# xiyichen/morphablediffusion

Hardware: AMD Instinct MI355X
Metric: multi-view denoising steps/sec (N=16 views, 256x256, CFG 2.0, DDIM-50 step) (higher is better)
Workload: dtype f16; 1 GPU; synthetic sample (FaceScape-FLAME-sized mesh, 5023 vertices before voxel de-duplication): N=16 target views, 256x256 (latent 32x32), perspective cameras, full-width UNet (916.9M params, random init), CFG 2.0, one denoise_apply per step; views_per_gpu=16, batch_view_num=16, parallelism=single GPU

## Files before the change

### include/mvd.h

```cpp
#ifndef MVD_H
#define MVD_H
#include <stddef.h>
#include <stdint.h>

#ifdef __cplusplus
extern "C" {
#endif

typedef struct mvd_ctx mvd_ctx;

typedef struct {
  int image_size;
  int in_channels;
  int out_channels;
  int model_channels;
  int num_res_blocks;
  int channel_mult[4];
  int num_heads;
  int context_dim;
  int volume_dims[4];
  int attention_levels;
} mvd_unet_config;

typedef struct {
  int time_dim;
  int view_dim;
  int num_views;
  int input_image_size;
  int frustum_volume_depth;
  int spatial_volume_size;
  float spatial_volume_length;
  float frustum_volume_length;
  int projection;
  int frustum_dims[4];
  float voxel_size;
} mvd_volume_config;

int mvd_create(const mvd_unet_config* ucfg, const mvd_volume_config* vcfg, int device, size_t workspace_bytes,
               mvd_ctx** out);
void mvd_destroy(mvd_ctx* ctx);
const char* mvd_last_error(void);
const char* mvd_compute_dtype(void);

int mvd_upload_weight(mvd_ctx* ctx, const char* name, const float* data, const int64_t* shape, int ndim, int on_device);
int mvd_set_precision_level(mvd_ctx* ctx, int level);
int mvd_set_vae_precision(mvd_ctx* ctx, int exact);
int mvd_finalize_weights(mvd_ctx* ctx);

int mvd_unet_forward(mvd_ctx* ctx, const float* x, const int64_t* timesteps, const float* context, int Bv, int n_ctx,
                     const float* src0, const float* src1, const float* src2, const float* src3, int depth0, float* out,
                     void* stream);
int mvd_unet_block(mvd_ctx* ctx, const char* path, const float* x, int B, int C, int H, int W, const int64_t* timesteps,
                   const float* context, const float* volume, int D, float* out, int out_capacity, int* out_shape, void* stream);


int mvd_embed_time(mvd_ctx* ctx, const int64_t* t, int B, float* out, void* stream);

int mvd_set_mesh(mvd_ctx* ctx, const float* vertices, const int32_t* coord, const int32_t* out_sh, const float* bounds,
                 int Nv);
int mvd_select_sample(mvd_ctx* ctx, int slot);
int mvd_set_cameras(mvd_ctx* ctx, const float* K, const float* RT, int N);
int mvd_set_mesh_async(mvd_ctx* ctx, const float* vertices, const int32_t* coord, const int32_t* out_sh, const float* bounds,
                       int Nv, void* stream);
int mvd_set_cameras_async(mvd_ctx* ctx, const float* K, const float* RT, int N, void* stream);
int mvd_set_samples_async(mvd_ctx* ctx, int B, const int* slots, const float* const* vertices, const int32_t* const* coord,
                          const int32_t* const* out_sh, const float* const* bounds, const int* Nv, const float* const* K,
                          const float* const* RT, int N, void* stream);
int mvd_rulebook_build(const int32_t* coord, const int32_t* out_sh, int Nv, int force_hash, int32_t* n_sites, int64_t* lens);
int mvd_rulebook_table(int which, int32_t* out);

int mvd_vertex_features(mvd_ctx* ctx, const float* x_noisy, const float* t_embed, const float* v_embed,
                        const int32_t* view_idx, int n_local, int add_bias, float* fused_out, void* stream);
int mvd_vertex_view_features(mvd_ctx* ctx, const float* x_noisy, const float* t_embed, const float* v_embed,
                             const int32_t* view_idx, int n_local, float* vf_out, void* stream);
int mvd_fuse_vertex_features(mvd_ctx* ctx, const float* vf_all, int n_views, float* fused_out, void* stream);
int mvd_vertex_features_stream_safe(mvd_ctx* ctx);
int mvd_stage_target_encoder(mvd_ctx* ctx, const float* x_noisy, const float* t_embed, const float* v_embed, int n_local,
                             float* feats, void* stream);
int mvd_stage_sparse_dense(mvd_ctx* ctx, const float* fused, int train_mode, float* dense_out, int32_t* shape_out, void* stream);
typedef struct { char internal[128]; } mvd_rccl_id;
int mvd_comm_unique_id(mvd_rccl_id* id_out);
int mvd_comm_init(mvd_ctx* ctx, const mvd_rccl_id* id, int rank, int world);
int mvd_comm_destroy(mvd_ctx* ctx);
int mvd_exchange_view_features(mvd_ctx* ctx, const float* local, float* all, int n_local, void* stream);
int mvd_comm_all_reduce(mvd_ctx* ctx, float* buf, size_t count, void* stream);
int mvd_set_volume_ready_event(mvd_ctx* ctx, void* event);
int mvd_volume_from_fused(mvd_ctx* ctx, const float* fused, float* volume_out, void* stream);

int mvd_volume_from_fused_train(mvd_ctx* ctx, const float* fused, float* volume_out, void* stream);
int mvd_mse_loss(mvd_ctx* ctx, const float* a, const float* b, size_t n, float* out, void* stream);
int mvd_train_enable(mvd_ctx* ctx, int on);
int mvd_train_param_count(mvd_ctx* ctx);
int mvd_train_param_info(mvd_ctx* ctx, int index, char* name, size_t name_cap, int64_t* offset, int64_t* numel, int64_t* shape,
                         int* ndim);
int64_t mvd_train_arena_size(mvd_ctx* ctx);
int mvd_train_adopt_arena(mvd_ctx* ctx, int which, float* ptr, int64_t numel);
int mvd_train_zero_grad(mvd_ctx* ctx, void* stream);
int mvd_train_unet_step(mvd_ctx* ctx, const float* x, const int64_t* timesteps, const float* context, int B, const float* src0,
                        const float* src1, const float* src2, const float* src3, int depth0, const float* target, float loss_scale,
                        int recompute, float* pred_out, float* loss_out, float* dsrc0, float* dsrc1, float* dsrc2, float* dsrc3,
                        void* stream);
int mvd_train_conditioner_backward(mvd_ctx* ctx, const float* x_noisy, int64_t timestep, const float* v_embed, int n_views,
                                   int target_index, const float* dsrc0, const float* dsrc1, const float* dsrc2, const float* dsrc3,
                                   float* dbg_dvolume, float* dbg_dfused, float* dbg_dfeats, float* dbg_dtembed, void* stream);
int mvd_train_conditioner_backward_batch(mvd_ctx* ctx, int B, const int* slots, const float* x_noisy, const int64_t* timesteps,
                                         const float* v_embed, int n_views, const int* target_index, const float* dsrc0,
                                         const float* dsrc1, const float* dsrc2, const float* dsrc3, float* dbg_dvolume,
                                         float* dbg_dfused, float* dbg_dfeats, float* dbg_dtembed, void* stream);
int mvd_train_cond_backward(mvd_ctx* ctx, int cond_index, const float* x, const float* context, const float* d_out, int B, int H,
                            int W, int depth0, float* dx, float* dcontext, void* stream);
int mvd_train_get_grad(mvd_ctx* ctx, const char* name, float* out, size_t numel, void* stream);
int mvd_train_get_tensor(mvd_ctx* ctx, const char* name, float* out, size_t numel, void* stream);
int64_t mvd_train_bn_calls(mvd_ctx* ctx);
int mvd_train_adamw_step(mvd_ctx* ctx, float lr, float lr_aux, float beta1, float beta2, float eps, float weight_decay, int step,
                         float inv_scale, int finetune_unet, int* skipped_out, void* stream);
int mvd_train_repack(mvd_ctx* ctx);
int mvd_train_repack_async(mvd_ctx* ctx, void* stream);
int mvd_train_grad_bucket_count(mvd_ctx* ctx);
int mvd_train_grad_bucket(mvd_ctx* ctx, int k, int max_ranges, int64_t* offs, int64_t* lens, int* n_ranges);
int mvd_train_grad_bucket_wait(mvd_ctx* ctx, int k, void* stream);
int mvd_train_set_bucket_snapshot(mvd_ctx* ctx, float* arena);
int mvd_train_sync_gradients(mvd_ctx* ctx, int phase, void* comm_stream, void* stream);
int mvd_set_volume(mvd_ctx* ctx, const float* volume, void* stream);

int mvd_frustum_volumes(mvd_ctx* ctx, const float* t_embed, const float* v_embed, const int32_t* view_idx, int TN,
                        float* out0, float* out1, float* out2, float* out3, void* stream);
int mvd_frustum_volumes_batch(mvd_ctx* ctx, int B, const int* slots, const float* volumes, const float* t_embed, const float* v_rows,
                              const int32_t* view_idx, float* out0, float* out1, float* out2, float* out3, void* stream);

int mvd_denoise_views(mvd_ctx* ctx, const float* x_noisy, const float* x_input, const float* clip, int64_t timestep,
                      const float* t_embed, const float* v_embed, const int32_t* view_idx, int TN, float cfg_scale,
                      const float* noise, float sqrt_one_minus_at, float sqrt_at, float sqrt_aprev, float dir_coef,
                      float sigma, float* eps_out, float* x_prev, void* stream);
int mvd_denoise_views_batch(mvd_ctx* ctx, int B, const int* slots, const float* x_noisy, const float* x_input, const float* clip,
                            const int64_t* timesteps, const float* t_embed, const float* v_embed, const int32_t* view_idx, int TN,
                            float cfg_scale, const float* noise, float sqrt_one_minus_at, float sqrt_at, float sqrt_aprev,
                            float dir_coef, float sigma, float* eps_out, float* x_prev, void* stream);

int mvd_denoise_views_ms(mvd_ctx* ctx, int B, const int* slots, const float* x_noisy, const float* x_input, const float* clip,
                         const int64_t* timesteps, const float* t_embed, const float* v_embed, const int32_t* view_idx, int TN,
                         float cfg_scale, const float* noise, float s1m, float sqrt_at, float c_x, float c_d, float c_c, float c_n,
                         float* x0_hist, int first, float* eps_out, float* x_next, void* stream);

int mvd_op_cfg_ms(const float* eps_c, const float* eps_u, float scale, const float* x, const float* noise, float s1m, float sqrt_at,
                  float c_x, float c_d, float c_c, float c_n, float* x0_hist, int first, float* eps_out, float* x_next, size_t n,
                  void* stream);
int mvd_op_conv(mvd_ctx* ctx, const float* x_nchw, int B, int Cin, int H, int W, const float* w, const float* bias,
                int Cout, int ksize, int stride, int upsample, const float* resid_nchw, float* out_nchw, int force_splitk,
                void* stream);
int mvd_op_linear(mvd_ctx* ctx, const float* a, int M, int K, const float* w, const float* bias, int N, int geglu,
                  const float* resid, int a_half, int force_splitk, float* out, void* stream);
int mvd_op_group_norm(mvd_ctx* ctx, const float* x_nchw, int B, int C, int HW, int groups, const float* gamma,
                      const float* beta, float eps, int act, float* out_nchw, void* stream);
int mvd_op_layer_norm(mvd_ctx* ctx, const float* x, int rows, int C, const float* gamma, const float* beta, float* out,
                      void* stream);
int mvd_op_attention(mvd_ctx* ctx, const float* q, const float* k, const float* v, int B, int T, int heads, int d,
                     float* out, void* stream);
int mvd_op_conv3d(mvd_ctx* ctx, const float* x_ncdhw, int B, int Cin, int D, int H, int W, const float* w,
                  const float* bias, int Cout, int stride, int transposed, const float* resid, float* out, void* stream);
int mvd_op_attention_bwd(mvd_ctx* ctx, const float* q, const float* k, const float* v, const float* d_out, int B, int T, int heads,
                         int d, float* dq, float* dk, float* dv, void* stream);
int mvd_op_group_norm_bwd(mvd_ctx* ctx, const float* x, const float* dy, int B, int rows, int C, int groups, const float* gamma,
                          const float* beta, float eps, int act, float* dx, float* dgamma, float* dbeta, void* stream);
int mvd_op_layer_norm_bwd(mvd_ctx* ctx, const float* x, const float* dy, int rows, int C, const float* gamma, float* dx,
                          float* dgamma, float* dbeta, void* stream);
int mvd_op_conv_bwd(mvd_ctx* ctx, int kind, int ksize, int B, int Cin, int H, int W, int Cout, const float* x, int x_f16,
                    const float* w, const float* dy, int xp, int accum, int need_din, int poison, float* dx, float* dw, float* db,
                    void* stream);
int mvd_op_linear_bwd(mvd_ctx* ctx, int B, int rows, int K, int N, const float* x, int x_f16, const float* w, const float* bias,
                      const float* dy, int geglu, int dx_f16, int staged, int xp, int accum, int poison, float* dx, float* dw,
                      float* db, void* stream);
int mvd_op_conv3d_bwd(mvd_ctx* ctx, int kind, int B, int Cin, int D, int H, int W, int Cout, const float* x, int x_f16,
                      const float* w, const float* dy, int accum, int poison, float* dx, float* dw, float* db, void* stream);
int mvd_op_tgemm(mvd_ctx* ctx, int M, int N, int K, const float* a, int a_f16, int a_trans, long lda, const float* b, int b_f16,
                 int b_trans, long ldb, float* out, int ldc, int accum, int xp, int poison, void* stream);
int mvd_op_st_tail(mvd_ctx* ctx, int C, int rows, int T, const float* ao, const float* xin, const float* rowbias,
                   const float* w_ao, const float* b_ao, const float* ln_g, const float* ln_b, const float* w1, const float* b1,
                   const float* w2, const float* b2, const float* w_po, const float* b_po, const float* resid, float* out,
                   int flags, int iters, float* ms_out, void* stream);
int mvd_op_st_head(mvd_ctx* ctx, int rows, int xp, const float* n0, const float* w_pi, const float* b_pi, const float* ln_g,
                   const float* ln_b, const float* w_q, const float* w_k, const float* w_v, float* t0_out, float* qkv_out,
                   int iters, float* ms_out, void* stream);
int mvd_bench_conv(mvd_ctx* ctx, int B, int C, int H, int W, int Cout, int iters, float* ms_out, void* stream);
int mvd_vae_decode(mvd_ctx* ctx, const float* z, int B, int h, int w, float* out, void* stream);
int mvd_vae_encode(mvd_ctx* ctx, const float* x, int B, int H, int W, float* moments, void* stream);
int mvd_clip_encode(mvd_ctx* ctx, const float* x, int B, int H, int W, float* out, void* stream);
int mvd_clip_embed_dim(mvd_ctx* ctx);
int mvd_probe_config(mvd_ctx* ctx, int mode, const char* family, int stride);
int mvd_probe_report(mvd_ctx* ctx, char* buf, size_t cap);
int mvd_bench_linear(mvd_ctx* ctx, int M, int K, int N, int flags, int iters, float* ms_out, void* stream);
int mvd_bench_group_norm(mvd_ctx* ctx, int B, int C, int HW, int groups, int flags, int iters, float* ms_out, void* stream);

#ifdef __cplusplus
}
#endif
#endif
```

### morphablediffusion_amd/csrc/c_api.hip

```cpp
#include <array>
#include <dlfcn.h>
#include <stdlib.h>
#include <string.h>

#include <algorithm>
#include <string>
#include <utility>
#include <vector>

#include "engine.h"
#include "rowchain.h"

int engine_set_cameras(mvd_ctx* c, const float* K, const float* RT, int N, hipStream_t s);
int engine_set_mesh(mvd_ctx* c, const float* vertices, const int32_t* coord, const int32_t* out_sh, const float* bounds,
                    int Nv, hipStream_t s);
int engine_select_sample(mvd_ctx* c, int slot);
int engine_set_samples(mvd_ctx* c, int B, const int* slots, const float* const* vertices, const int32_t* const* coord,
                       const int32_t* const* out_sh, const float* const* bounds, const int* Nv, const float* const* K,
                       const float* const* RT, int N, hipStream_t s);
int engine_rulebook_build(const int32_t* coord, const int32_t* out_sh, int Nv, int force_hash, int32_t* n_sites, int64_t* lens);
int engine_rulebook_table(int which, int32_t* out);
void mesh_free(MeshTables& m);

static thread_local std::string g_err;
// ... 899 lines not shown
  if (c->comm) {
    a->comm_destroy(c->comm);
    c->comm = nullptr;
  }
  const int rc = a->comm_init_rank(&c->comm, world, *id, rank);
  if (rc) {
    c->comm = nullptr;
    return rccl_fail(a, "ncclCommInitRank", rc);
  }
  c->comm_rank = rank;
  c->comm_world = world;
  return 0;
}

int mvd_comm_destroy(mvd_ctx* c) {
  if (!c || !c->comm) return 0;
  RcclApi* a = rccl_api();
  if (a) a->comm_destroy(c->comm);
  c->comm = nullptr;
  c->comm_world = 1;
  c->comm_rank = 0;
  return 0;
}

int mvd_exchange_view_features(mvd_ctx* c, const float* local, float* all, int n_local, void* stream) {
  if (!c || !c->comm) return mvd_fail("mvd_exchange_view_features: no communicator (mvd_comm_init)");
  if (hipSetDevice(c->device) != hipSuccess) return mvd_fail("hipSetDevice failed");
  if (!local || !all || n_local <= 0 || c->mesh.Nv <= 0) return mvd_fail("mvd_exchange_view_features: bad arguments / no mesh is set");
  RcclApi* a = rccl_api();
  if (!a) return mvd_fail("mvd_exchange_view_features: librccl.so could not be opened");
  if (c->v.num_views > 0 && (long)c->comm_world * n_local != c->v.num_views)
    return mvd_fail("mvd_exchange_view_features: comm_world * n_local does not equal the configured view count");
  const size_t count = (size_t)n_local * c->mesh.Nv * 16;
  const int rc = a->all_gather(local, all, count,  7, c->comm, S(stream));
  return rc ? rccl_fail(a, "ncclAllGather", rc) : 0;
}

int mvd_comm_all_reduce(mvd_ctx* c, float* buf, size_t count, void* stream) {
  if (!c || !c->comm) return mvd_fail("mvd_comm_all_reduce: no communicator (mvd_comm_init)");
  if (hipSetDevice(c->device) != hipSuccess) return mvd_fail("hipSetDevice failed");
  if (!buf || count == 0) return mvd_fail("mvd_comm_all_reduce: bad arguments");
  RcclApi* a = rccl_api();
  if (!a) return mvd_fail("mvd_comm_all_reduce: librccl.so could not be opened");
  const int rc = a->all_reduce(buf, buf, count,  7,  0, c->comm, S(stream));
  return rc ? rccl_fail(a, "ncclAllReduce", rc) : 0;
}

int mvd_train_sync_gradients(mvd_ctx* c, int phase, void* comm_stream, void* stream) {
  if (!c || !c->comm) return mvd_fail("mvd_train_sync_gradients: no communicator (mvd_comm_init)");
  if (hipSetDevice(c->device) != hipSuccess) return mvd_fail("hipSetDevice failed");
  if (!c->arena_g || c->arena_n == 0) return mvd_fail("mvd_train_sync_gradients: no gradient arena (mvd_train_enable)");
  if (phase != 0 && phase != 1) return mvd_fail("mvd_train_sync_gradients: phase is 0 (start) or 1 (finish)");
  RcclApi* a = rccl_api();
  if (!a) return mvd_fail("mvd_train_sync_gradients: librccl.so could not be opened");
  hipStream_t cs = S(comm_stream), ms = S(stream);
  auto reduce = [&](size_t off, size_t n) -> int {
    const int rc = a->all_reduce(c->arena_g + off, c->arena_g + off, n, 7, 0, c->comm, cs);
    return rc ? rccl_fail(a, "ncclAllReduce", rc) : 0;
  };
  if (phase == 0) {
    for (int k = 0; k < c->n_buckets; ++k) {
      const mvd_ctx::GradBucket& b = c->buckets[k];
      if (b.ev) HIP_CHECK_RET(hipStreamWaitEvent(cs, b.ev, 0));
      for (size_t r = 0; r < b.off.size(); ++r) RET_IF(reduce(b.off[r], b.len[r]));
    }
    c->grad_sync_started = true;
    return 0;
  }
  if (!c->ev_grad_sync[0]) {
    HIP_CHECK_RET(hipEventCreateWithFlags(&c->ev_grad_sync[0], hipEventDisableTiming));
    HIP_CHECK_RET(hipEventCreateWithFlags(&c->ev_grad_sync[1], hipEventDisableTiming));
  }
  HIP_CHECK_RET(hipEventRecord(c->ev_grad_sync[0], ms));
  HIP_CHECK_RET(hipStreamWaitEvent(cs, c->ev_grad_sync[0], 0));
  std::vector<std::pair<size_t, size_t>> spans;
  if (c->grad_sync_started)
    for (int k = 0; k < c->n_buckets; ++k)
      for (size_t r = 0; r < c->buckets[k].off.size(); ++r) spans.push_back({c->buckets[k].off[r], c->buckets[k].off[r] + c->buckets[k].len[r]});
  std::sort(spans.begin(), spans.end());
  size_t pos = 0;
  for (auto& sp : spans) {
    if (sp.first < pos) return mvd_fail("mvd_train_sync_gradients: gradient buckets overlap");
    if (sp.first > pos) RET_IF(reduce(pos, sp.first - pos));
    pos = sp.second;
  }
  if (pos < c->arena_n) RET_IF(reduce(pos, c->arena_n - pos));
  c->grad_sync_started = false;
  HIP_CHECK_RET(hipEventRecord(c->ev_grad_sync[1], cs));
  HIP_CHECK_RET(hipStreamWaitEvent(ms, c->ev_grad_sync[1], 0));
  return launch_scale_copy(c->arena_g, c->arena_n, 1.0f / (float)c->comm_world, c->arena_g, ms);
}

int mvd_op_conv(mvd_ctx* c, const float* x_nchw, int B, int Cin, int H, int W, const float* w, const float* bias, int Cout,
                int ksize, int stride, int upsample, const float* resid_nchw, float* out_nchw, int force_splitk,
                void* stream) {
  if (c && hipSetDevice(c->device) != hipSuccess) return mvd_fail("hipSetDevice failed");
  hipStream_t s = S(stream);
  WsScope ws_scope(c);
  const int cpad = (Cin + 7) / 8 * 8, taps = ksize * ksize;
  const int Hv = H << upsample, Wv = W << upsample;
  const int Ho = (Hv - 1) / stride + 1, Wo = (Wv - 1) / stride + 1;
  float* xn = ws_alloc<float>(c, (size_t)B * H * W * cpad);
  half_t* wp = ws_alloc<half_t>(c, (size_t)taps * Cout * cpad);
  float* on = ws_alloc<float>(c, (size_t)B * Ho * Wo * Cout);
  float* rn = resid_nchw ? ws_alloc<float>(c, (size_t)B * Ho * Wo * Cout) : nullptr;
  WS_CHECK(xn && wp && on);
  RET_IF(launch_nchw_to_nhwc(x_nchw, B, Cin, H * W, xn, cpad, cpad, s));
  RET_IF(launch_pack_weight(w, Cout, cpad, taps, 0, 0, wp, s, Cin));
  if (rn) RET_IF(launch_nchw_to_nhwc(resid_nchw, B, Cout, Ho * Wo, rn, Cout, Cout, s));
  if (force_splitk == -3) {
    if (taps != 9 || stride != 1 || upsample || rn || cpad != Cin) return mvd_fail("op_conv: the fp32 output-head form is 3x3, stride 1, no residual");
    RET_IF(launch_out_conv_f32(xn, Cin, w, bias, Cout, B, H, W, on, Cout, s));
    RET_IF(launch_nhwc_to_nchw(on, Cout, B, Cout, Ho * Wo, out_nchw, s));
    return 0;
  }
  if (force_splitk == -2) {
    if (taps != 9 || stride != 1 || upsample || rn) return mvd_fail("op_conv: the fp32 first-layer form is 3x3, stride 1, no residual");
    RET_IF(launch_conv_in_f32(xn, cpad, w, Cin, bias, Cout, B, H, W, on, Cout, s));
    RET_IF(launch_nhwc_to_nchw(on, Cout, B, Cout, Ho * Wo, out_nchw, s));
    return 0;
  }
  ConvW cw;
  cw.w = wp; cw.bias = const_cast<float*>(bias); cw.N = Cout; cw.Cin = cpad; cw.taps = taps;
  GemmArgs g;
  g.a = xn; g.a_f32 = 1; g.lda = cpad; g.w = &cw; g.out = on; g.ldc = Cout; g.resid = rn; g.ldr = Cout;
  g.use_bias = bias != nullptr; g.force_splitk = force_splitk;
  if (cpad % 64 == 0) {
    half_t* xh = ws_alloc<half_t>(c, (size_t)B * H * W * cpad);
    WS_CHECK(xh);
    RET_IF(launch_f32_to_f16(xn, xh, (size_t)B * H * W * cpad, s));
    g.a = xh;
    g.a_f32 = 0;
    const int bnx = Cout % 160 == 0 ? 160 : (Cout % 128 == 0 ? 128 : 0);
    if (taps == 9 && bnx && mvd_env_call::conv3x()) {
      cw.wx = ws_alloc<half_t>(c, conv3x_stream_halfs(Cout, cpad, bnx));
      WS_CHECK(cw.wx);
      RET_IF(conv3x_pack(wp, Cout, cpad, bnx, cw.wx, s));
      cw.wx_bn = bnx;
    }
  }
  if (upsample && taps == 9 && stride == 1 && cpad == Cin && B * H * W >= 2048) {
    cw.w_up = ws_alloc<half_t>(c, (size_t)16 * Cout * Cin);
    WS_CHECK(cw.w_up);
    RET_IF(launch_pack_upconv_weight(w, Cout, Cin, cw.w_up, s));
    g.a = xn; g.a_f32 = 1;
    RET_IF(run_upconv2d(c, g, B, H, W, s));
  } else {
    RET_IF(run_conv2d(c, g, B, H, W, stride, upsample, s));
  }
  RET_IF(launch_nhwc_to_nchw(on, Cout, B, Cout, Ho * Wo, out_nchw, s));
  return 0;
}

int mvd_op_conv3d(mvd_ctx* c, const float* x, int B, int Cin, int D, int H, int W, const float* w, const float* bias,
                  int Cout, int stride, int transposed, const float* resid, float* out, void* stream) {
  if (c && hipSetDevice(c->device) != hipSuccess) return mvd_fail("hipSetDevice failed");
  hipStream_t s = S(stream);
  WsScope ws_scope(c);
  if (Cin % 8) return mvd_fail("op_conv3d: Cin must be a multiple of 8");
  const int Do = transposed ? 2 * D : (D - 1) / stride + 1, Ho = transposed ? 2 * H : (H - 1) / stride + 1,
            Wo = transposed ? 2 * W : (W - 1) / stride + 1;
  float* xn = ws_alloc<float>(c, (size_t)B * D * H * W * Cin);
  half_t* wp = ws_alloc<half_t>(c, (size_t)27 * Cout * Cin);
  float* on = ws_alloc<float>(c, (size_t)B * Do * Ho * Wo * Cout);
  WS_CHECK(xn && wp && on);
  RET_IF(launch_nchw_to_nhwc(x, B, Cin, D * H * W, xn, Cin, Cin, s));
  RET_IF(launch_pack_weight(w, Cout, Cin, 27, transposed, 0, wp, s, Cin));
  if (resid) RET_IF(launch_nchw_to_nhwc(resid, B, Cout, Do * Ho * Wo, on, Cout, Cout, s));
  ConvW cw;
  cw.w = wp; cw.bias = const_cast<float*>(bias); cw.N = Cout; cw.Cin = Cin; cw.taps = 27;
  GemmArgs g;
  g.a = xn; g.a_f32 = 1; g.lda = Cin; g.w = &cw; g.out = on; g.ldc = Cout; g.use_bias = bias != nullptr;
  if (resid) { g.resid = on; g.ldr = Cout; }
  if (Cin % 64 == 0) {
    half_t* xh = ws_alloc<half_t>(c, (size_t)B * D * H * W * Cin);
    WS_CHECK(xh);
    RET_IF(launch_f32_to_f16(xn, xh, (size_t)B * D * H * W * Cin, s));
    g.a = xh;
    g.a_f32 = 0;
  }
  if (transposed) RET_IF(run_convT3d(c, g, B, D, H, W, s));
  else RET_IF(run_conv3d(c, g, B, D, H, W, stride, s));
  RET_IF(launch_nhwc_to_nchw(on, Cout, B, Cout, Do * Ho * Wo, out, s));
  return 0;
}

int mvd_op_linear(mvd_ctx* c, const float* a, int M, int K, const float* w, const float* bias, int N, int geglu,
                  const float* resid, int a_half, int force_splitk, float* out, void* stream) {
  if (c && hipSetDevice(c->device) != hipSuccess) return mvd_fail("hipSetDevice failed");
  hipStream_t s = S(stream);
  WsScope ws_scope(c);
  if (K % 8) return mvd_fail("op_linear: K must be a multiple of 8");
  half_t* wp = ws_alloc<half_t>(c, (size_t)N * K);
  float* bp = ws_alloc<float>(c, (size_t)N);
  WS_CHECK(wp && bp);
  RET_IF(launch_pack_weight(w, N, K, 1, 0, geglu, wp, s, K));
  if (bias) {
    if (geglu) RET_IF(launch_permute_geglu_bias(bias, N, bp, s));
    else HIP_CHECK_RET(hipMemcpyAsync(bp, bias, (size_t)N * 4, hipMemcpyDeviceToDevice, s));
  }
  ConvW cw;
  cw.w = wp; cw.bias = bias ? bp : nullptr; cw.N = N; cw.Cin = K; cw.taps = 1;
  GemmArgs g;
  g.a = a; g.a_f32 = 1; g.lda = K; g.w = &cw; g.out = out; g.ldc = geglu ? N / 2 : N; g.geglu = geglu;
  g.use_bias = bias != nullptr;
  g.force_splitk = force_splitk;
  if (resid) {
    g.resid = resid; g.resid_f32 = 1; g.ldr = N;
  }
  if (a_half) {
    half_t* ah = ws_alloc<half_t>(c, (size_t)M * K);
    WS_CHECK(ah);
    RET_IF(launch_f32_to_f16(a, ah, (size_t)M * K, s));
    g.a = ah; g.a_f32 = 0;
  }
  RET_IF(run_linear(c, g, 1, M, s));
  return 0;
}

int mvd_op_group_norm(mvd_ctx* c, const float* x_nchw, int B, int C, int HW, int groups, const float* gamma,
                      const float* beta, float eps, int act, float* out_nchw, void* stream) {
  if (c && hipSetDevice(c->device) != hipSuccess) return mvd_fail("hipSetDevice failed");
  hipStream_t s = S(stream);
  WsScope ws_scope(c);
  float* xn = ws_alloc<float>(c, (size_t)B * HW * C);
  half_t* y = ws_alloc<half_t>(c, (size_t)B * HW * C);
  float* yf = ws_alloc<float>(c, (size_t)B * HW * C);
  WS_CHECK(xn && y && yf);
  RET_IF(launch_nchw_to_nhwc(x_nchw, B, C, HW, xn, C, C, s));
  NormW n;
  n.g = const_cast<float*>(gamma); n.b = const_cast<float*>(beta); n.C = C;
  RET_IF(run_group_norm(c, xn, C, B, HW, n, groups, eps, act, nullptr, y, C, s));
  hipLaunchKernelGGL(f16_to_f32_kernel, dim3(nblk((size_t)B * HW * C)), dim3(256), 0, s, y, yf, (size_t)B * HW * C);
  RET_IF(launch_nhwc_to_nchw(yf, C, B, C, HW, out_nchw, s));
  return 0;
}

int mvd_op_layer_norm(mvd_ctx* c, const float* x, int rows, int C, const float* gamma, const float* beta, float* out,
                      void* stream) {
  if (c && hipSetDevice(c->device) != hipSuccess) return mvd_fail("hipSetDevice failed");
  hipStream_t s = S(stream);
  WsScope ws_scope(c);
  half_t* y = ws_alloc<half_t>(c, (size_t)rows * C);
  WS_CHECK(y);
  RET_IF(launch_layernorm(x, rows, C, gamma, beta, 1e-5f, y, s));
  hipLaunchKernelGGL(f16_to_f32_kernel, dim3(nblk((size_t)rows * C)), dim3(256), 0, s, y, out, (size_t)rows * C);
  HIP_CHECK_RET(hipGetLastError());
  return 0;
}

int mvd_op_attention(mvd_ctx* c, const float* q, const float* k, const float* v, int B, int T, int heads, int d, float* out,
                     void* stream) {
  if (c && hipSetDevice(c->device) != hipSuccess) return mvd_fail("hipSetDevice failed");
  hipStream_t s = S(stream);
  WsScope ws_scope(c);
  const int C = heads * d, rows = B * T;
  half_t* qkv = ws_alloc<half_t>(c, (size_t)rows * 3 * C);
  half_t* o = ws_alloc<half_t>(c, (size_t)rows * C);
  WS_CHECK(qkv && o);
  hipLaunchKernelGGL(pack_qkv_rows_kernel, dim3(nblk((size_t)rows * C)), dim3(256), 0, s, q, k, v, rows, C, qkv);
  RET_IF(launch_attention(qkv, 3 * C, qkv + 2 * C, 3 * C, o, C, B, T, heads, d, s));
  hipLaunchKernelGGL(f16_to_f32_kernel, dim3(nblk((size_t)rows * C)), dim3(256), 0, s, o, out, (size_t)rows * C);
  HIP_CHECK_RET(hipGetLastError());
  return 0;
}

int mvd_op_attention_bwd(mvd_ctx* c, const float* q, const float* k, const float* v, const float* d_out, int B, int T, int heads, int d,
                         float* dq, float* dk, float* dv, void* stream) {
  if (c && hipSetDevice(c->device) != hipSuccess) return mvd_fail("hipSetDevice failed");
  if (!c) return mvd_fail("null context");
  hipStream_t s = S(stream);
  WsScope ws_scope(c);
  const int C = heads * d, rows = B * T;
  half_t* qkv = ws_alloc<half_t>(c, (size_t)rows * 3 * C);
  half_t* o = ws_alloc<half_t>(c, (size_t)rows * C);
  half_t* do16 = ws_alloc<half_t>(c, (size_t)rows * C);
  half_t* dqkv = ws_alloc<half_t>(c, (size_t)rows * 3 * C);
  float* lse = ws_alloc<float>(c, (size_t)B * heads * T);
  float* delta = ws_alloc<float>(c, (size_t)B * heads * T);
  float* tmp = ws_alloc<float>(c, (size_t)rows * 3 * C);
  WS_CHECK(qkv && o && do16 && dqkv && lse && delta && tmp);
  hipLaunchKernelGGL(pack_qkv_rows_kernel, dim3(nblk((size_t)rows * C)), dim3(256), 0, s, q, k, v, rows, C, qkv);
  RET_IF(launch_attention(qkv, 3 * C, qkv + 2 * C, 3 * C, o, C, B, T, heads, d, s));
  RET_IF(bwd_cast_rows(d_out, C, rows, C, C, do16, s));
  RET_IF(bwd_attention(qkv, 3 * C, o, do16, C, dqkv, 3 * C, lse, delta, B, T, heads, d, s));
  hipLaunchKernelGGL(f16_to_f32_kernel, dim3(nblk((size_t)rows * 3 * C)), dim3(256), 0, s, dqkv, tmp, (size_t)rows * 3 * C);
  HIP_CHECK_RET(hipGetLastError());
  float* outs[3] = {dq, dk, dv};
  for (int i = 0; i < 3; ++i)
    HIP_CHECK_RET(hipMemcpy2DAsync(outs[i], (size_t)C * 4, tmp + (size_t)i * C, (size_t)3 * C * 4, (size_t)C * 4, rows, hipMemcpyDeviceToDevice, s));
  return 0;
}

int mvd_op_group_norm_bwd(mvd_ctx* c, const float* x, const float* dy, int B, int rows, int C, int groups, const float* gamma,
                          const float* beta, float eps, int act, float* dx, float* dgamma, float* dbeta, void* stream) {
  if (c && hipSetDevice(c->device) != hipSuccess) return mvd_fail("hipSetDevice failed");
  if (!c) return mvd_fail("null context");
  hipStream_t s = S(stream);
  WsScope ws_scope(c);
  const bool one_block = mvd_env().gn_bwd_one_block;
  const int S = one_block ? 1 : bwd_gn_slabs(B, groups, rows);
  float* dg = ws_alloc<float>(c, (size_t)B * S * C);
  float* db = ws_alloc<float>(c, (size_t)B * S * C);
  float* part = ws_alloc<float>(c, (size_t)B * groups * S * 4);
  WS_CHECK(dg && db && part);
  if (one_block)
    RET_IF(bwd_group_norm(x, C, nullptr, 0, dy, C, B, rows, C, groups, gamma, beta, eps, act, dx, C, 0, dg, db, nullptr, s));
  else
    RET_IF(bwd_group_norm_slab(x, C, nullptr, 0, dy, C, B, rows, C, groups, gamma, beta, eps, act, dx, C, 0, part,
                               part + (size_t)B * groups * S * 2, dg, db, nullptr, S, s));
  RET_IF(bwd_sum_rows_add(dg, B * S, C, C, dgamma, 0, s));
  return bwd_sum_rows_add(db, B * S, C, C, dbeta, 0, s);
}

int mvd_op_layer_norm_bwd(mvd_ctx* c, const float* x, const float* dy, int rows, int C, const float* gamma, float* dx, float* dgamma,
                          float* dbeta, void* stream) {
  if (c && hipSetDevice(c->device) != hipSuccess) return mvd_fail("hipSetDevice failed");
  if (!c) return mvd_fail("null context");
  hipStream_t s = S(stream);
  WsScope ws_scope(c);
  float* part = ws_alloc<float>(c, (size_t)bwd_ln_max_blocks() * 2 * C);
  WS_CHECK(part);
  int nb = 0;
  RET_IF(bwd_layer_norm(x, C, dy, C, rows, C, gamma, 1e-5f, dx, C, 0, part, &nb, s));
  RET_IF(bwd_sum_rows_add(part, nb, C, 2 * C, dgamma, 0, s));
  return bwd_sum_rows_add(part + C, nb, C, 2 * C, dbeta, 0, s);
}

int mvd_bench_conv(mvd_ctx* c, int B, int C, int H, int W, int Cout, int iters, float* ms_out, void* stream) {
  if (c && hipSetDevice(c->device) != hipSuccess) return mvd_fail("hipSetDevice failed");
  hipStream_t s = S(stream);
  WsScope ws_scope(c);
  const size_t na = (size_t)B * H * W * C, nw = (size_t)9 * Cout * C;
  half_t* a = ws_alloc<half_t>(c, na);
  half_t* w = ws_alloc<half_t>(c, nw);
  float* o = ws_alloc<float>(c, (size_t)B * H * W * Cout);
  WS_CHECK(a && w && o);
// ... 324 lines not shown
```

### morphablediffusion_amd/csrc/common.h

```cpp
#pragma once
#include <hip/hip_runtime.h>
#include <hip/hip_fp16.h>
#include <stdint.h>

#include "env.h"

#ifdef MVD_BF16
typedef __bf16 half_t;
#define MVD_MFMA_32x32x16 __builtin_amdgcn_mfma_f32_32x32x16_bf16
#define MVD_MFMA_16x16x32 __builtin_amdgcn_mfma_f32_16x16x32_bf16
#define MVD_DTYPE_NAME "bf16"
#else
typedef _Float16 half_t;
#define MVD_MFMA_32x32x16 __builtin_amdgcn_mfma_f32_32x32x16_f16
#define MVD_MFMA_16x16x32 __builtin_amdgcn_mfma_f32_16x16x32_f16
#define MVD_DTYPE_NAME "f16"
#endif
typedef half_t h8 __attribute__((ext_vector_type(8)));
typedef half_t h4 __attribute__((ext_vector_type(4)));
typedef half_t h2 __attribute__((ext_vector_type(2)));
typedef float f32x16 __attribute__((ext_vector_type(16)));
typedef float f32x4 __attribute__((ext_vector_type(4)));

#define MVD_MAX_TAPS 27

enum { ACT_NONE = 0, ACT_SILU = 1, ACT_RELU = 2 };

inline bool xcd_prefers_cols(int tiles_m, int groups_n, double a_bytes, double w_bytes) {
  const int nwg = tiles_m * groups_n, q = (nwg + 7) / 8;
  if (nwg < 16) return false;
  auto span = [](int q_, int inner, int outer) {
    const double n = q_ % inner == 0 ? q_ / inner : (q_ - 1) / (double)inner + 1.0;
    return n < outer ? n : (double)outer;
  };
  const double at = a_bytes / tiles_m, wt = w_bytes / groups_n;
  const double row = at * span(q, groups_n, tiles_m) + wt * (q < groups_n ? q : groups_n);
  const double col = wt * span(q, tiles_m, groups_n) + at * (q < tiles_m ? q : tiles_m);
  return col < 0.8 * row;
}

struct IGemm {
  const void* a;
  int a_f32;
  int lda;
  int Cin;
  int cin_alg;
  int B, Z, Y, X;
  int IZ, IY, IX;
  int sz, sy, sx;
  int ups;
  int PZ, PY, PX;
  int ntaps;
  int tap[MVD_MAX_TAPS];
  const half_t* w;
  int N;
  void* out;
  int out_f32;
  int ldc;
  int out_linear;
  int OZ, OY, OX, ozm, ozo, oym, oyo, oxm, oxo;
  const float* bias;
  const float* rowbias;
  int rb_ld;
  const float* rowscale;
  int rs_ld;
  float* gn_partial;
  int gn_cpg;
  const void* resid;
  int resid_f32;
  int ldr;
  int out_split;
  int geglu;
  float alpha;
  int act;
  int nch;
  int xcd_cols;
  int npar;
  int par_ntaps[8];
  int par_tap[8][8];
  int par_oz[8], par_oy[8], par_ox[8];
  int par_walk;
  const half_t* wx;
  int wx_bn;
  int bn;
  int bm;
  int splitk;
  float* partial;
};

struct MvdStream {
  hipStream_t s;
};

#define HIP_CHECK_RET(expr)                                        \
  do {                                                             \
    hipError_t _e = (expr);                                        \
    if (_e != hipSuccess) return mvd_fail(hipGetErrorString(_e));  \
  } while (0)

int mvd_fail(const char* msg);
const char* mvd_error_text();

#define MVD_MAX_DEVICES 64
static inline int mvd_current_device() {
  int d = 0;
  if (hipGetDevice(&d) != hipSuccess || d < 0 || d >= MVD_MAX_DEVICES) d = 0;
  return d;
}
static inline int cdiv(int a, int b) { return (a + b - 1) / b; }
static inline int igemm_tap(int dz, int dy, int dx, int slab) { return (dz + 1) | ((dy + 1) << 2) | ((dx + 1) << 4) | (slab << 8); }

int launch_igemm(const IGemm& g, hipStream_t s);
int igemm_pick_bn(int N, int geglu);
int launch_splitk_reduce(const IGemm& g, hipStream_t s);
bool conv3_halo_eligible(const IGemm& g);
int conv3_halo_tiles(const IGemm& g, int bn);
int launch_conv3_halo(const IGemm& g, hipStream_t s);
int igemm_pick_splitk(int M, int N, int ksteps, int bn);
bool conv3x_eligible(const IGemm& g, int bn);
size_t conv3x_stream_halfs(int N, int Cin, int bn);
int conv3x_pack(const half_t* w, int N, int Cin, int bn, half_t* stream, hipStream_t s);
int launch_conv3x(const IGemm& g, const half_t* stream, int bn, hipStream_t s);
bool gemm_dma_eligible(const IGemm& g);
bool gemm_dma_is_plain(const IGemm& g);
void gemm_dma_plan(int M, int N, int ksteps, int bn, int geglu, int* nch_out, int* splitk_out);
int launch_target_encoder(const float* x, const float* pre, int n_views, const half_t* const* w, const float* const* bias,
                          const int* cin, const float* const* gamma, const float* const* beta, float* feats, hipStream_t s);
void gemm_dma_plan_us(int M, int N, int ksteps, int geglu, int out_b, int res_b, int* bn_io, int* nch_out, int* splitk_out,
                      int* bm_out = nullptr);
int launch_gemm_dma(const IGemm& g, hipStream_t s);

int launch_gn_stats(const float* x, int ld, int B, int rows_per_sample, int C, int G, const float* preadd, int pld,
                    float* partial, int* nslabs_out, hipStream_t s);
int launch_gn_apply(const float* x, int ld, int B, int rows_per_sample, int C, int G, const float* preadd, int pld,
                    const float* partial, int nslabs, const float* gamma, const float* beta, float eps, int act,
                    half_t* out, int ldo, hipStream_t s, int split = 0);
int gn_max_slabs();
int launch_gn_finalize(const float* partial, int B, int nslabs, int rows_per_sample, int C, int G, const float* gamma,
                       const float* beta, float eps, float* scale, float* shift, int ld, hipStream_t s);
bool gn_group_eligible(int ld, int rows, int C, int G, int pld, int ldo);
int launch_gn_group(const float* x, int ld, int B, int rows, int C, int G, const float* preadd, int pld, const float* gamma,
                    const float* beta, float eps, int act, half_t* out, int ldo, hipStream_t s, int split = 0,
                    int nslab = 1, size_t slab_stride = 0, const float* bias2 = nullptr, const float* resid = nullptr, int ldr = 0,
                    float* mat = nullptr, int ldm = 0);
int launch_layernorm(const float* x, int rows, int C, const float* gamma, const float* beta, float eps,
                     half_t* out, hipStream_t s, half_t* raw = nullptr, int ld_raw = 0);
bool layernorm_slabs_takes(int C);
int launch_layernorm_slabs(const float* slabs, int nslab, size_t slab_stride, int rows, int C, const float* bias, const float* rowbias,
                           int rb_ld, int T, const float* resid, int ldr, float* mat, const float* gamma, const float* beta, float eps,
                           half_t* out, hipStream_t s, half_t* raw = nullptr, int ld_raw = 0);
int launch_layernorm_f32(const float* x, long ldx, int rows, int C, const float* gamma, const float* beta, float eps,
                         float* out, hipStream_t s);
int launch_attention(const half_t* qk, int ldqk, const half_t* v, int ldv, half_t* out, int ldo, int B, int T, int heads,
                     int d, hipStream_t s, int Tstride = 0);
int launch_clip_patches(const float* img, int B, int H, int W, int S, int P, int Kp, half_t* out, hipStream_t s);
int launch_clip_tokens(const float* pe, const float* cls, const float* pos, int B, int T, int Tp, int C, float* x,
                       hipStream_t s);
int launch_scale_copy(const float* src, size_t n, float k, float* dst, hipStream_t s);
int launch_softmax_rows(const float* s, long rows, int cols, half_t* p, hipStream_t st);
int launch_depth_attn(const float* qk, const half_t* ctxn, half_t* z, int n_cond, int HW, int D, int Cc, int heads,
                      hipStream_t s, int split = 0, int nfill = 0, const half_t* fill_row = nullptr, int ldx = 0);
int launch_small_linear(const float* a, int lda, int rows, int K, const half_t* w, const float* bias, int N,
                        int act_in, float* out, int ldo, int accumulate, hipStream_t s);
int launch_timestep_embedding(const int64_t* t, int B, int dim, float* out, hipStream_t s);
int launch_nchw_to_nhwc(const float* in, int B, int C, int HW, float* out, int ldo, int cpad, hipStream_t s);
int launch_nhwc_to_nchw(const float* in, int ld, int B, int C, int HW, float* out, hipStream_t s);
int launch_pack_weight(const float* src, int N, int Cin, int taps, int transposed, int geglu, half_t* dst,
                       hipStream_t s, int cin_src = -1, int xp = 0);
int launch_rows_f32_to_f16_split(const float* in, int lda, long rows, int C, half_t* out, hipStream_t s);
int launch_permute_geglu_bias(const float* src, int N, float* dst, hipStream_t s);
int launch_f32_to_f16(const float* in, half_t* out, size_t n, hipStream_t s);
int launch_rows_f32_to_f16(const float* in, int lda, long rows, int C, half_t* out, hipStream_t s);
int launch_pack_upconv_weight(const float* src, int N, int Cin, half_t* dst, hipStream_t s);
int launch_fill_rows_f16(half_t* out, int ld, int rows, const half_t* vec, int n, hipStream_t s);
int launch_fold_qk(const float* wq, const float* wk, int heads, int hd, int Cc, int I, float scale, half_t* out,
                   hipStream_t s, float* out32 = nullptr);
int launch_fold_ov(const float* wo, const float* wv, int heads, int hd, int Cc, int I, half_t* out, hipStream_t s,
                   float* out32 = nullptr);
int launch_fold_mm(const float* a, int lda, const float* b, int ldb, int M, int N, int K, half_t* out16, int ldc, float* out32,
                   hipStream_t s);
int launch_relu_beta_tile(const float* beta, int Cc, int heads, half_t* out, hipStream_t s, int split = 0);
int launch_cfg_ddim(const float* eps_c, const float* eps_u, float scale, const float* x, const float* noise,
                    float sqrt_one_minus_at, float sqrt_at, float sqrt_aprev, float dir_coef, float sigma,
                    float* eps_out, float* x_prev, size_t n, hipStream_t s);
struct DpmCoef {
  float s1m, sqrt_at, c_x, c_d, c_c, c_n;
};
int launch_cfg_dpm(const float* eps_c, const float* eps_u, float scale, const float* x, const float* noise, DpmCoef k,
                   float* x0_hist, int use_hist, float* eps_out, float* x_next, size_t n, hipStream_t s);
struct ViewCam {
  float P[12];
  float Pinv[12];
  float Kinv[9];
  float near_, far_;
};
int launch_vertex_gather(const float* feats, const ViewCam* cams, const int* view_idx, int n_views, const float* verts, int Nv, int V,
                         float vol_len, int fsize, int persp, float* out, hipStream_t s);
int launch_fuse_views(const float* vf, int n_views, int Nv, int total_views, const float* w, const float* b,
                      float* out, int accumulate, hipStream_t s);
int launch_sparse_conv(const float* in, const int* nbr, int n_out, int Cin, int Cout, const float* w, const float* wp,
                       const float* scale, const float* shift, float* out, hipStream_t s, int mask_nonrep = 0);
bool sparse_mfma_takes(int Cin, int Cout);
int launch_sparse_w_frag(const float* w, int Cl_in, int Cl_out, int transposed, int flip, float* dst, hipStream_t s);
int launch_sparse_w_pack(const float* src, int Cin, int Cout, int layout, float* dst, hipStream_t s);
int launch_bn_fold(const float* gamma, const float* beta, const float* mean, const float* var, float eps, int C, float* scale,
                   float* shift, hipStream_t s);
int launch_bn_rows_relu(const float* x, float* y, int n, int C, const float* gamma, const float* beta, float eps, float* stats_out,
                        hipStream_t s, float* rmean = nullptr, float* rvar = nullptr, float momentum = 0.f);
int launch_mse(const float* a, const float* b, size_t n, float* out, hipStream_t s);
int launch_latent_gather(const float* feats, const int* grid, int gd, int gh, int gw, const float* min_xyz,
                         const int* out_sh, float voxel, int V, float vol_len, float* out, hipStream_t s);
int launch_sparse_densify(const float* feats, const int* grid, long nvox, int C, float* out, hipStream_t s);
int launch_frustum_gather(const float* vol, const ViewCam* cams, const int* view_idx, int TN, int D, int S, int V,
                          float vol_len, int persp, half_t* out, hipStream_t s);
int launch_bits_checksum(const void* p, size_t bytes, unsigned long long* out, hipStream_t s);
int launch_add_rows(float* dst, const float* a, const float* b, size_t n, hipStream_t s);
int launch_add_image_rows(const float* in, int ldi, const float* img, int C, int nb, int HW, float* out, int ldo, hipStream_t s);
int launch_upsample2_f16(const float* in, int ldi, int B, int H, int W, int C, half_t* out, hipStream_t s);
int launch_conv_in_f32(const float* x, int ldx, const float* w, int cin_src, const float* bias, int N, int B, int H, int W, float* out,
                       int ldo, hipStream_t s);
int launch_out_conv_f32(const float* a, int C, const float* w, const float* bias, int N, int B, int H, int W, float* out, int ldo,
                        hipStream_t s);
int launch_probe_null(hipStream_t s);
```

### morphablediffusion_amd/csrc/engine.h

```cpp
#pragma once
#include <functional>
#include <map>
#include <string>
#include <vector>

#include "../../include/mvd.h"
#include "common.h"
#include "rowchain.h"

struct RawTensor {
  float* d = nullptr;
  std::vector<int64_t> shape;
  size_t numel = 0;
};

struct ConvW {
  int xp = 0;
  int cin_l = 0;
  half_t* w = nullptr;
  half_t* wx = nullptr;
  int wx_bn = 0;
  half_t* w_up = nullptr;
  int res_out = 0;
  float* w32 = nullptr;
  int cin_src = 0;
  float* bias = nullptr;
  int N = 0, Cin = 0, taps = 1;
  half_t* wT = nullptr;
  int Np = 0;
  std::string key;
  std::string bkey;
};
struct NormW {
  float* g = nullptr;
  float* b = nullptr;
  int C = 0;
  std::string key;
};
struct LinW {
  std::string key;
  half_t* w = nullptr;
  float* bias = nullptr;
  int N = 0, K = 0;
};

struct ResW {
  NormW n1, n2;
  ConvW c1, c2, skip;
  bool has_skip = false;
  int cin = 0, cout = 0, emb_off = 0;
  int res = 0;
  std::string key;
};
struct STW {
  NormW norm, ln1, ln3;
  ConvW proj_in, qkv, attn_out, ff1, ff2, proj_out;
  int C = 0, heads = 8, a2_off = 0;
  std::string key;
  half_t* rc_stream = nullptr;
  half_t* rh_stream = nullptr;
  int rc_po = 1, rh_xp = 0;
  ConvW ffp;
};
struct CondW {
  ConvW proj_in, proj_ctx, wqk, wov, conv1, conv2;
  NormW gn_in, gn_ctx, gn_o1, gn_o2;
  half_t* relu_beta = nullptr;
  int dim = 0, Cc = 0, I = 0;
  int res = 0;
  std::string key;
};
struct VaeResW {
  NormW n1, n2;
  ConvW c1, c2, skip;
  bool has_skip = false;
  int cin = 0, cout = 0;
};
struct VaeAttnW {
  NormW norm;
  ConvW q, k, v, proj;
};
struct VaeW {
  bool present = false;
  int ch = 0, out_ch = 0, zc = 0, embed = 0, block_in = 0, nlev = 0;
  ConvW post_quant;
  ConvW conv_in, conv_out;
  NormW norm_out;
  VaeResW mid1, mid2;
  VaeAttnW attn;
  std::vector<std::vector<VaeResW>> up;
  std::vector<ConvW> up_conv;
};
struct VaeEncW {
  bool present = false;
  int in_ch = 0, nlev = 0, mom = 0;
  ConvW conv_in, conv_out, quant;
  NormW norm_out;
  VaeResW mid1, mid2;
  VaeAttnW attn;
  std::vector<std::vector<VaeResW>> down;
  std::vector<ConvW> down_conv;
};

struct ClipLayerW {
  NormW ln1, ln2;
  ConvW qkv;
  ConvW out;
  ConvW fc;
  ConvW proj;
};
struct ClipW {
  bool present = false;
  int width = 0, layers = 0, heads = 0, patch = 0, image = 0, embed = 0;
  int T = 0, Tp = 0, Kp = 0;
  ConvW conv1;
  float* cls = nullptr;
  float* pos = nullptr;
  NormW ln_pre, ln_post;
  LinW proj;
  std::vector<ClipLayerW> blk;
};

struct UOp {
  int kind = 0;
  int idx = 0;
  int cin = 0, cout = 0;
};
enum { OP_CONV_IN = 0, OP_RES = 1, OP_ST = 2, OP_DOWN = 3, OP_UP = 4 };

struct FrustumBlockW {
  LinW t_conv, v_conv;
  NormW gn;
  ConvW conv;
  int cin = 0, cout = 0, stride = 1;
};
struct SparseLayerW {
  std::string wkey, bnkey;
  int layout = 0;
  float* w = nullptr;
  float* wp = nullptr;
  float* wd = nullptr;
  float* scale = nullptr;
  float* shift = nullptr;
  float* gamma = nullptr;
  float* beta = nullptr;
  float* rmean = nullptr;
  float* rvar = nullptr;
  int cin = 0, cout = 0;
  bool strided = false;
};
struct EncBlockW {
  LinW t, v;
  NormW n1, n2;
  ConvW c1, c2;
};

struct Workspace {
  char* base = nullptr;
  size_t size = 0, off = 0, peak = 0;
  int hold = 0;
  void* alloc(size_t bytes) {
    size_t o = (off + 255) & ~(size_t)255;
    if (o + bytes > size) return nullptr;
    off = o + bytes;
    if (off > peak) peak = off;
    return base + o;
  }
};

struct MeshTables {
  int Nv = 0;
  float* verts = nullptr;
  int n_sites[3] = {0, 0, 0};
  int shape[3][3];
// ... 415 lines not shown
```

### morphablediffusion_amd/csrc/engine_unet.hip

```cpp
#include <string.h>

#include <algorithm>

#include "engine.h"

namespace {

void igemm_init(IGemm& g) {
  memset(&g, 0, sizeof(g));
  g.alpha = 1.0f;
  g.sz = g.sy = g.sx = 1;
  g.out_linear = 1;
  g.Z = g.Y = g.X = g.B = 1;
  g.IZ = g.IY = g.IX = 1;
  g.PZ = g.PY = g.PX = 1;
  for (int i = 0; i < MVD_MAX_TAPS; ++i) g.tap[i] = igemm_tap(0, 0, 0, i);
}

void igemm_fill(IGemm& g, const GemmArgs& ga) {
  g.a = ga.a;
  g.a_f32 = ga.a_f32;
  g.lda = ga.lda;
  g.Cin = ga.w->Cin;
  g.cin_alg = ga.w->xp ? ga.w->cin_l : ga.w->Cin;
// ... 26 lines not shown
  for (int s2 = 1; s2 <= 8 && s2 <= ncc; ++s2) {
    const int rounds = cdiv(tiles * s2, 256), steps = cdiv(ncc, s2) * 9;
    double t = rounds * (steps * step_us + 8.0);
    if (s2 > 1) t += 3.0 + (s2 + 1) * (double)M * N * 4.0 / 3.5e6;
    if (t < *us) {
      *us = t;
      sk = s2;
    }
  }
  return sk;
}

bool place_partials(mvd_ctx* c, IGemm& g, int M, int sk, const GemmArgs* defer, bool form_ok) {
  g.splitk = sk;
  g.partial = nullptr;
  bool deferred = false;
  if (sk > 1) {
    if (defer && defer->slabs && defer->sk_used && sk <= mvd_env().defer_max && (size_t)sk * M * g.N <= defer->slabs_cap &&
        (!g.resid || (defer->defer_epilogue && g.resid_f32)) && form_ok) {
      g.partial = defer->slabs;
      deferred = true;
    } else {
      g.partial = ws_alloc<float>(c, (size_t)sk * M * g.N);
      if (!g.partial) g.splitk = 1;
    }
  }
  if (defer && defer->sk_used) *defer->sk_used = deferred ? sk : 1;
  return deferred;
}

int reduce_partials(mvd_ctx* c, IGemm& g, int M, hipStream_t s) {
  ProbeScope ps(c, s, "splitk_reduce_kernel", 0.0, (double)M * g.N * 4.0 * (g.splitk + 1));
  return launch_splitk_reduce(g, s);
}

int go_conv3x(mvd_ctx* c, IGemm& g, int M, int force_splitk, hipStream_t s, const GemmArgs* defer) {
  const int ncc = g.Cin / 64;
  const int tiles = (g.X == 8 ? cdiv(g.B, 4) : g.B * (g.Y / 16) * (g.X / 16)) * (g.N / g.wx_bn);
  double us;
  int sk = pick_chunk_split(tiles, ncc, g.wx_bn == 160 ? 0.75 : 0.62, M, g.N, &us);
  if (force_splitk > 0) sk = force_splitk < ncc ? force_splitk : ncc;
  if (sk > 1) sk = cdiv(ncc, cdiv(ncc, sk));
  g.bn = g.wx_bn;
  WsScope ws_scope(c, WS_TEMP);
  const bool deferred = place_partials(c, g, M, sk, defer, true);
  const double kalg = (double)(g.cin_alg ? g.cin_alg : g.Cin);
  const double flops = 2.0 * M * g.N * kalg * 9.0;
  double bytes = (double)M * kalg * 2 + 9.0 * g.N * kalg * 2 + (g.splitk > 1 ? 0.0 : (double)M * g.N * 4);
  if (g.resid && g.splitk <= 1) bytes += (double)M * g.N * 4;
  int r;
  {
    ProbeScope ps(c, s, g.wx_bn == 160 ? "conv3x_kernel<5>" : "conv3x_kernel<4>", flops, bytes);
    r = launch_conv3x(g, g.wx, g.wx_bn, s);
  }
  if (!r && g.splitk > 1 && !deferred) r = reduce_partials(c, g, M, s);
  return r;
}

int go_parity_batch(mvd_ctx* c, IGemm& g, int M, hipStream_t s) {
  if (!gemm_dma_eligible(g)) return mvd_fail("igemm_go: parity batch needs the LDS-DMA kernel");
  int kmax = 0;
  for (int p = 0; p < g.npar; ++p) kmax = g.par_ntaps[p] > kmax ? g.par_ntaps[p] : kmax;
  int nch = 1, sk2 = 1;
  gemm_dma_plan(M * g.npar, g.N, kmax * cdiv(g.Cin, 64), g.bn, 1, &nch, &sk2);
  g.nch = nch;
  g.splitk = 1;
  g.partial = nullptr;
  const int pwalk_min = mvd_env().par_walk_min;
  if (pwalk_min > 0 && cdiv(M, 256) * cdiv(g.N, g.bn) >= pwalk_min) {
    g.par_walk = 1;
    g.nch = 1;
  }
  double fl = 0.0;
  for (int p = 0; p < g.npar; ++p) fl += 2.0 * M * g.N * (double)(g.cin_alg ? g.cin_alg : g.Cin) * g.par_ntaps[p];
  const double by = (double)g.B * g.PZ * g.PY * g.PX * g.Cin * 2 + (double)g.npar * kmax * g.N * g.Cin * 2 +
                    (double)M * g.npar * g.N * (g.out_f32 ? 4 : 2) + (g.resid ? (double)M * g.npar * g.N * (g.resid_f32 ? 4 : 2) : 0.0);
  char fam[64];
  snprintf(fam, sizeof fam, "gemm_dma_kernel<%d,0>", g.bn);
  ProbeScope ps(c, s, fam, fl, by);
  return launch_gemm_dma(g, s);
}

int plan_halo(IGemm& g, int M, int force_splitk) {
  const MvdEnv& env = mvd_env();
  const int ncc = g.Cin / 64;
  double best = 1e30;
  int best_bn = 128, best_sk = 1;
  for (int bn = 128; bn <= 160; bn += 32) {
    double us;
    const int s2 = pick_chunk_split(conv3_halo_tiles(g, bn), ncc, bn == 160 ? 1.3 : 1.0, M, g.N, &us);
    if (us < best) {
      best = us;
      best_bn = bn;
      best_sk = s2;
    }
  }
  g.bn = best_bn;
  int sk = force_splitk > 0 ? (force_splitk < ncc ? force_splitk : ncc) : best_sk;
  if (env.halo_bn) g.bn = env.halo_bn;
  if (env.halo_sk) sk = env.halo_sk;
  if (sk > ncc) sk = ncc;
  if (sk > 1) sk = cdiv(ncc, cdiv(ncc, sk));
  return sk;
}

int plan_dense(IGemm& g, int M, int force_splitk) {
  const MvdEnv& env = mvd_env();
  int nch = 1, sk2 = 1;
  const int ksteps = g.ntaps * cdiv(g.Cin, 64);
  const bool plain_gemm = !g.gn_partial && !g.rowscale && g.ntaps == 1;
  if (plain_gemm && !env.old_plan) {
    int bn = 0, bm = 256;
    gemm_dma_plan_us(M, g.N, ksteps, g.geglu, g.out_f32 ? 4 : (g.out_split ? 6 : 2), g.resid ? (g.resid_f32 ? 4 : 2) : 0, &bn,
                     &nch, &sk2, gemm_dma_is_plain(g) ? &bm : nullptr);
    g.bn = bn;
    g.bm = bm;
  } else {
    gemm_dma_plan(M, g.N, ksteps, g.bn, g.geglu, &nch, &sk2);
  }
  if (g.gn_partial || g.rowscale) {
    if (g.bn == 160) g.bn = 128;
    const int tiles = cdiv(M, 256) * cdiv(g.N, g.bn);
    nch = cdiv(tiles, 256);
    if (nch > 64) nch = 64;
    force_splitk = 1;
  }
  int sk = g.geglu ? 1 : (force_splitk > 0 ? force_splitk : sk2);
  if (env.dense_bn && !g.geglu && !g.gn_partial && !g.rowscale) {
    g.bn = env.dense_bn;
    g.bm = (env.dense_bm == 128 && gemm_dma_is_plain(g)) ? 128 : 256;
    gemm_dma_plan(M, g.N, ksteps, g.bn, g.geglu, &nch, &sk2);
    if (g.bm == 128) {
      nch = 1;
      sk2 = 1;
    }
    if (force_splitk <= 0) sk = sk2;
  }
  if (env.dense_sk && !g.geglu && force_splitk <= 0) sk = env.dense_sk;
  if (sk > ksteps) sk = ksteps;
  if (sk > 1) sk = cdiv(ksteps, cdiv(ksteps, sk));
  g.nch = sk > 1 ? 1 : nch;
  if (env.plan_debug) fprintf(stderr, "[plan] M=%d N=%d ksteps=%d -> bm=%d bn=%d nch=%d sk=%d\n", M, g.N, ksteps, g.bm ? g.bm : 256, g.bn, g.nch, sk);
  return sk;
}

int plan_gather(IGemm& g, int M, int force_splitk) {
  const int ksteps = g.ntaps * cdiv(g.Cin, 64);
  int sk = force_splitk > 0 ? force_splitk : igemm_pick_splitk(M, g.N, ksteps, g.bn);
  if (sk > ksteps) sk = ksteps;
  if (sk > 1) sk = cdiv(ksteps, cdiv(ksteps, sk));
  return sk;
}

enum IGemmKernel { K_GATHER = 0, K_HALO = 1, K_DENSE = 2 };

int launch_planned(mvd_ctx* c, IGemm& g, int M, int sk, IGemmKernel kernel, hipStream_t s, const GemmArgs* defer) {
  WsScope ws_scope(c, WS_TEMP);
  const bool deferred =
      place_partials(c, g, M, sk, defer, !g.geglu && g.act == 0 && g.alpha == 1.0f && g.out_linear && g.out_f32 && !g.out_split);
  const bool timing = mvd_env().layer_timing;
  static hipEvent_t ev0 = nullptr, ev1 = nullptr;
  if (timing) {
    if (!ev0) {
      hipEventCreate(&ev0);
      hipEventCreate(&ev1);
    }
    hipEventRecord(ev0, s);
  }
  int r;
  const double flops = 2.0 * M * g.N * (double)(g.cin_alg ? g.cin_alg : g.Cin) * g.ntaps;
  const double in_rows = (double)g.B * g.PZ * g.PY * g.PX;
  const double out_cols = g.geglu ? g.N / 2 : g.N;
  const double kalg = (double)(g.cin_alg ? g.cin_alg : g.Cin);
  double bytes = in_rows * kalg * (g.a_f32 ? 4 : 2) + (double)g.ntaps * g.N * kalg * 2 +
                 (g.gn_partial ? 0.0 : (double)M * out_cols * (g.out_f32 ? 4 : 2));
  if (g.resid) bytes += (double)M * g.N * (g.resid_f32 ? 4 : 2);
  char fam[64];
  if (kernel == K_HALO) {
    snprintf(fam, sizeof fam, "conv3_dma_kernel<%d,%d,%d>", g.bn == 160 ? 160 : 128, g.X % 16 == 0 ? 16 : 8, g.X % 16 == 0 ? 16 : 8);
    ProbeScope ps(c, s, fam, flops, g.splitk > 1 ? bytes - (double)M * out_cols * (g.out_f32 ? 4 : 2) : bytes);
    r = launch_conv3_halo(g, s);
  } else if (kernel == K_DENSE) {
    if (g.bm == 128) snprintf(fam, sizeof fam, "gemm_dma_kernel<128x%d>", g.bn);
    else snprintf(fam, sizeof fam, "gemm_dma_kernel<%d,%d>", g.bn, g.gn_partial ? 1 : (g.rowscale ? 2 : 0));
    ProbeScope ps(c, s, fam, flops, bytes);
    r = launch_gemm_dma(g, s);
  } else {
    const int bn = g.bn ? g.bn : igemm_pick_bn(g.N, g.geglu);
    snprintf(fam, sizeof fam, "igemm_kernel<%d,%d>", g.a_f32, bn);
    ProbeScope ps(c, s, fam, flops, bytes);
    r = launch_igemm(g, s);
  }
  if (!r && g.splitk > 1 && !deferred) r = reduce_partials(c, g, M, s);
  if (timing) {
    hipEventRecord(ev1, s);
    hipEventSynchronize(ev1);
    float ms = 0.f;
    hipEventElapsedTime(&ms, ev0, ev1);
    const double fl = 2.0 * M * g.N * g.Cin * g.ntaps;
    fprintf(stderr, "[gemm] M=%d N=%d Cin=%d taps=%d f32=%d halo=%d bn=%d sk=%d geglu=%d  %.1f us  %.0f TF\n", M, g.N, g.Cin,
            g.ntaps, g.a_f32, (int)kernel, g.bn, g.splitk, g.geglu, ms * 1e3, fl / (ms * 1e-3) * 1e-12);
  }
  return r;
}

int igemm_go(mvd_ctx* c, IGemm& g, int force_splitk, hipStream_t s, const GemmArgs* defer = nullptr) {
  const MvdEnv& env = mvd_env();
  const int M = g.B * g.Z * g.Y * g.X;
  g.bn = igemm_pick_bn(g.N, g.geglu);
  if (g.a_f32 && g.bn == 160 && env.igemm_f32_bn128) g.bn = 128;
  if (env.conv3x && c->use_halo && g.wx && conv3x_eligible(g, g.wx_bn)) return go_conv3x(c, g, M, force_splitk, s, defer);
  if (g.npar > 0) return go_parity_batch(c, g, M, s);
  const bool halo = c->use_halo && conv3_halo_eligible(g);
  const bool dense = env.gemm_dma && !halo && M >= env.dense_min_m && (g.ntaps == 1 || M <= 16384) && gemm_dma_eligible(g);
  if (g.gn_partial && !dense) return mvd_fail("igemm_go: the statistics-only pass needs the LDS-DMA kernel");
  if (halo) return launch_planned(c, g, M, plan_halo(g, M, force_splitk), K_HALO, s, defer);
  if (dense) return launch_planned(c, g, M, plan_dense(g, M, force_splitk), K_DENSE, s, defer);
  return launch_planned(c, g, M, plan_gather(g, M, force_splitk), K_GATHER, s, defer);
}

}

int run_linear(mvd_ctx* c, const GemmArgs& ga, int B, int rows, hipStream_t s) {
  IGemm g;
  igemm_init(g);
  igemm_fill(g, ga);
  g.B = B;
  g.X = rows / B;
  g.IX = g.X;
  g.PX = g.X;
  g.ntaps = 1;
  return igemm_go(c, g, ga.force_splitk, s, &ga);
}

int run_conv2d(mvd_ctx* c, const GemmArgs& ga, int B, int H, int W, int stride, int ups, hipStream_t s) {
  IGemm g;
  igemm_init(g);
  igemm_fill(g, ga);
  g.B = B;
  g.PY = H;
  g.PX = W;
  g.ups = ups;
  g.IY = H << ups;
  g.IX = W << ups;
  g.sy = g.sx = stride;
  g.Y = (g.IY - 1) / stride + 1;
  g.X = (g.IX - 1) / stride + 1;
  if (ga.w->taps == 9) {
    g.ntaps = 9;
    for (int t = 0; t < 9; ++t) g.tap[t] = igemm_tap(0, t / 3 - 1 + ga.tap_shift, t % 3 - 1 + ga.tap_shift, t);
  } else if (ga.w->taps == 1) {
    g.ntaps = 1;
  } else {
    return mvd_fail("run_conv2d: kernel must be 1x1 or 3x3");
  }
  return igemm_go(c, g, ga.force_splitk, s, &ga);
}

int run_upconv2d(mvd_ctx* c, const GemmArgs& ga_in, int B, int H, int W, hipStream_t s) {
  if (!ga_in.w->w_up) return mvd_fail("run_upconv2d: weights were not folded");
  WsScope ws_scope(c, WS_TEMP);
  GemmArgs ga = ga_in;
  ConvW cw = *ga_in.w;
  cw.w = cw.w_up;
  cw.taps = 16;
  ga.w = &cw;
  if (ga.a_f32) {
    half_t* ah = ws_alloc<half_t>(c, (size_t)B * H * W * cw.Cin);
    WS_CHECK(ah);
    RET_IF(launch_rows_f32_to_f16((const float*)ga.a, ga.lda, (long)B * H * W, cw.Cin, ah, s));
    ga.a = ah;
    ga.a_f32 = 0;
    ga.lda = cw.Cin;
  }
  IGemm gb;
  igemm_init(gb);
  igemm_fill(gb, ga);
  gb.B = B;
  gb.Y = gb.PY = gb.IY = H;
  gb.X = gb.PX = gb.IX = W;
  gb.out_linear = 0;
  gb.OZ = 1;
  gb.OY = 2 * H;
  gb.OX = 2 * W;
  gb.ozm = 1;
  gb.oym = gb.oxm = 2;
  const bool batched = mvd_env().parity_batch && ga.force_splitk <= 1 && gemm_dma_eligible(gb);
  for (int par = 0; par < 4; ++par) {
    const int py = par >> 1, px = par & 1;
    int taps[4];
    for (int a = 0; a < 2; ++a)
      for (int b = 0; b < 2; ++b)
        taps[a * 2 + b] = igemm_tap(0, py == 0 ? a - 1 : a, px == 0 ? b - 1 : b, par * 4 + a * 2 + b);
    if (batched) {
      gb.par_ntaps[par] = 4;
      for (int i = 0; i < 4; ++i) gb.par_tap[par][i] = taps[i];
      gb.par_oz[par] = 0;
      gb.par_oy[par] = py;
      gb.par_ox[par] = px;
      continue;
    }
    IGemm g = gb;
    g.ntaps = 4;
    for (int i = 0; i < 4; ++i) g.tap[i] = taps[i];
    g.oyo = py;
    g.oxo = px;
    RET_IF(igemm_go(c, g, ga.force_splitk, s));
  }
  if (batched) {
    gb.npar = 4;
    gb.ntaps = 4;
    gb.bn = igemm_pick_bn(gb.N, 0);
    RET_IF(igemm_go(c, gb, 0, s));
  }
  return 0;
}

int run_conv3d(mvd_ctx* c, const GemmArgs& ga, int B, int D, int H, int W, int stride, hipStream_t s) {
  IGemm g;
  igemm_init(g);
  igemm_fill(g, ga);
  g.B = B;
  g.PZ = g.IZ = D;
  g.PY = g.IY = H;
  g.PX = g.IX = W;
  g.sz = g.sy = g.sx = stride;
  g.Z = (D - 1) / stride + 1;
  g.Y = (H - 1) / stride + 1;
  g.X = (W - 1) / stride + 1;
  if (ga.w->taps == 27) {
    g.ntaps = 27;
    for (int t = 0; t < 27; ++t) g.tap[t] = igemm_tap(t / 9 - 1, (t / 3) % 3 - 1, t % 3 - 1, t);
  } else if (ga.w->taps == 1) {
    g.ntaps = 1;
  } else {
    return mvd_fail("run_conv3d: kernel must be 1 or 27 taps");
  }
  return igemm_go(c, g, ga.force_splitk, s);
}

int run_convT3d(mvd_ctx* c, const GemmArgs& ga, int B, int D, int H, int W, hipStream_t s) {
  if (ga.w->taps != 27) return mvd_fail("run_convT3d: expects a 3x3x3 kernel");
  IGemm gb;
  igemm_init(gb);
  igemm_fill(gb, ga);
  gb.B = B;
  gb.Z = gb.PZ = gb.IZ = D;
  gb.Y = gb.PY = gb.IY = H;
  gb.X = gb.PX = gb.IX = W;
  gb.out_linear = 0;
  gb.OZ = 2 * D;
  gb.OY = 2 * H;
  gb.OX = 2 * W;
  gb.ozm = gb.oym = gb.oxm = 2;
  const bool batched = mvd_env().parity_batch && !ga.a_f32 && ga.force_splitk <= 1 && B * D * H * W >= 512 && gemm_dma_eligible(gb);
  for (int par = 0; par < 8; ++par) {
    const int pz = par >> 2, py = (par >> 1) & 1, px = par & 1;
    const int kz[2] = {pz ? 0 : 1, 2}, dzv[2] = {pz ? 1 : 0, 0}, nz = pz ? 2 : 1;
    const int ky[2] = {py ? 0 : 1, 2}, dyv[2] = {py ? 1 : 0, 0}, ny = py ? 2 : 1;
    const int kx[2] = {px ? 0 : 1, 2}, dxv[2] = {px ? 1 : 0, 0}, nx = px ? 2 : 1;
    int taps[8], t = 0;
    for (int a = 0; a < nz; ++a)
      for (int b = 0; b < ny; ++b)
        for (int e = 0; e < nx; ++e) taps[t++] = igemm_tap(dzv[a], dyv[b], dxv[e], (kz[a] * 3 + ky[b]) * 3 + kx[e]);
    if (batched) {
      gb.par_ntaps[par] = t;
      for (int i = 0; i < t; ++i) gb.par_tap[par][i] = taps[i];
      gb.par_oz[par] = pz;
      gb.par_oy[par] = py;
      gb.par_ox[par] = px;
      continue;
    }
    IGemm g = gb;
    for (int i = 0; i < t; ++i) g.tap[i] = taps[i];
    g.ntaps = t;
    g.ozo = pz;
    g.oyo = py;
    g.oxo = px;
    RET_IF(igemm_go(c, g, ga.force_splitk, s));
  }
  if (batched) {
    gb.npar = 8;
    gb.ntaps = 8;
    gb.bn = igemm_pick_bn(gb.N, 0);
    RET_IF(igemm_go(c, gb, 0, s));
  }
  return 0;
}

int run_group_norm(mvd_ctx* c, const float* x, int ld, int B, int rows_per_sample, const NormW& n, int groups, float eps,
                   int act, const float* preadd, half_t* out, int ldo, hipStream_t s, int preadd_ld, int split, int nslab,
                   size_t slab_stride, const float* bias2, const float* resid, int ldr, float* mat, int ldm) {
  ProbeScope ps(c, s, "group_norm", 0.0, (double)B * rows_per_sample * n.C * 6.0);
  if (!mvd_env().gn_two_pass && gn_group_eligible(ld, rows_per_sample, n.C, groups, preadd ? (preadd_ld ? preadd_ld : n.C) : 0, ldo))
    return launch_gn_group(x, ld, B, rows_per_sample, n.C, groups, preadd, preadd_ld ? preadd_ld : n.C, n.g, n.b, eps, act, out,
                           ldo, s, split, nslab, slab_stride, bias2, resid, ldr, mat, ldm);
  if (nslab > 1 || resid || mat) return mvd_fail("run_group_norm: slab input needs the single-pass form");
  WsScope ws_scope(c, WS_TEMP);
  float* partial = ws_alloc<float>(c, (size_t)B * gn_max_slabs() * groups * 2);
  WS_CHECK(partial);
  int nslabs = 0;
  RET_IF(launch_gn_stats(x, ld, B, rows_per_sample, n.C, groups, preadd, preadd_ld, partial, &nslabs, s));
  RET_IF(launch_gn_apply(x, ld, B, rows_per_sample, n.C, groups, preadd, preadd_ld, partial, nslabs, n.g, n.b, eps, act, out,
                         ldo, s, split));
  return 0;
}

namespace {

}

int unet_do_res(Fwd& f, const ResW& r, View in, View out, int H, int W, ResSaved* sv, Carry* in_carry, Carry* out_carry) {
  mvd_ctx* c = f.c;
  WsScope ws_scope(c, WS_BLOCK);
  const int rows = f.Bv * H * W;
  const int w1 = r.c1.xp ? 3 : 1, w2 = r.c2.xp ? 3 : 1;
  half_t* a1 = ws_alloc<half_t>(c, (size_t)rows * r.cin * w1);
  float* h1 = ws_alloc<float>(c, (size_t)rows * r.cout);
  half_t* a2 = ws_alloc<half_t>(c, (size_t)rows * r.cout * w2);
  WS_CHECK(a1 && h1 && a2);
  const bool skip_side = r.has_skip && mvd_env().skip_side && !f.train && !sv;
  const bool sk_in_carry = r.has_skip && out_carry && out_carry->aux && out_carry->aux_cap >= (size_t)rows * r.cout;
  float* skbuf = nullptr;
  auto launch_skip = [&](hipStream_t ss, bool no_split) -> int {
    GemmArgs gs;
    gs.a = in.p; gs.a_f32 = 1; gs.lda = in.ld; gs.w = &r.skip; gs.out = skbuf; gs.ldc = r.cout;
    if (no_split) gs.force_splitk = 1;
    if (r.skip.xp) {
      half_t* as = ws_alloc<half_t>(c, (size_t)rows * 3 * r.cin);
      WS_CHECK(as);
      RET_IF(launch_rows_f32_to_f16_split(in.p, in.ld, rows, r.cin, as, ss));
      gs.a = as; gs.a_f32 = 0; gs.lda = 3 * r.cin;
    }
    return run_linear(c, gs, f.Bv, rows, ss);
  };
  auto fork_skip = [&]() -> int {
    if (!c->side2) {
      HIP_CHECK_RET(hipStreamCreateWithFlags(&c->side2, hipStreamNonBlocking));
      HIP_CHECK_RET(hipEventCreateWithFlags(&c->ev_s2_fork, hipEventDisableTiming));
      HIP_CHECK_RET(hipEventCreateWithFlags(&c->ev_s2_join, hipEventDisableTiming));
    }
    HIP_CHECK_RET(hipEventRecord(c->ev_s2_fork, f.s));
    HIP_CHECK_RET(hipStreamWaitEvent(c->side2, c->ev_s2_fork, 0));
    RET_IF(launch_skip(c->side2, true));
    HIP_CHECK_RET(hipEventRecord(c->ev_s2_join, c->side2));
    return 0;
  };
  if (r.has_skip) {
    skbuf = sk_in_carry ? out_carry->aux : ws_alloc<float>(c, (size_t)rows * r.cout);
    WS_CHECK(skbuf);
  }
  const bool in_slabs = in_carry && in_carry->sk > 1;
  if (skip_side && !in_slabs) RET_IF(fork_skip());
  if (in_slabs)
    RET_IF(run_group_norm(c, in_carry->slabs, r.cin, f.Bv, H * W, r.n1, 32, 1e-5f, ACT_SILU, nullptr, a1, r.cin * w1, f.s, 0, r.c1.xp,
                          in_carry->sk, in_carry->stride, in_carry->bias, in_carry->resid, in_carry->ldr, in.p, in.ld));
  else
    RET_IF(run_group_norm(c, in.p, in.ld, f.Bv, H * W, r.n1, 32, 1e-5f, ACT_SILU, nullptr, a1, r.cin * w1, f.s, 0, r.c1.xp));
  if (skip_side && in_slabs) RET_IF(fork_skip());
  GemmArgs g1;
  g1.a = a1; g1.lda = r.cin * w1; g1.w = &r.c1; g1.out = h1; g1.ldc = r.cout;
  g1.rowbias = f.emb_all + r.emb_off; g1.rb_ld = c->emb_total;
  int sk1 = 1;
  const size_t slab_elems = (size_t)rows * r.cout;
  if (mvd_env().defer_reduce && !f.train && gn_group_eligible(r.cout, H * W, r.cout, 32, c->emb_total, r.cout * w2)) {
    const size_t nsl = rows > 8192 ? 4 : 16;
    g1.slabs = ws_alloc<float>(c, nsl * slab_elems);
    g1.slabs_cap = g1.slabs ? nsl * slab_elems : 0;
    g1.sk_used = &sk1;
  }
  RET_IF(run_conv2d(c, g1, f.Bv, H, W, 1, 0, f.s));
  if (sk1 > 1)
    RET_IF(run_group_norm(c, g1.slabs, r.cout, f.Bv, H * W, r.n2, 32, 1e-5f, ACT_SILU, g1.rowbias, a2, r.cout * w2, f.s, g1.rb_ld,
                          r.c2.xp, sk1, slab_elems, r.c1.bias));
  else
    RET_IF(run_group_norm(c, h1, r.cout, f.Bv, H * W, r.n2, 32, 1e-5f, ACT_SILU, nullptr, a2, r.cout * w2, f.s, 0, r.c2.xp));
  const float* resid = in.p;
  int ldr = in.ld;
  bool skip_outlives_scope = true;
  if (r.has_skip) {
    skip_outlives_scope = sk_in_carry;
    if (skip_side) HIP_CHECK_RET(hipStreamWaitEvent(f.s, c->ev_s2_join, 0));
    else RET_IF(launch_skip(f.s, false));
    resid = skbuf;
    ldr = r.cout;
  }
  GemmArgs g2;
  g2.a = a2; g2.lda = r.cout * w2; g2.w = &r.c2; g2.out = out.p; g2.ldc = out.ld; g2.resid = resid; g2.ldr = ldr;
  int sk2 = 1;
  if (out_carry && out_carry->slabs && skip_outlives_scope) {
    g2.slabs = out_carry->slabs; g2.slabs_cap = out_carry->cap; g2.sk_used = &sk2; g2.defer_epilogue = true;
  }
  RET_IF(run_conv2d(c, g2, f.Bv, H, W, 1, 0, f.s));
  if (out_carry) {
    out_carry->sk = sk2;
    out_carry->stride = (size_t)rows * r.cout;
    out_carry->bias = r.c2.bias;
    out_carry->resid = resid;
    out_carry->ldr = ldr;
  }
  if (sv) {
    sv->a1 = a1; sv->ld1 = r.cin * w1; sv->h1 = h1; sv->a2 = a2; sv->ld2 = r.cout * w2;
  }
  return 0;
}

int unet_do_st(Fwd& f, const STW& t, View in, View out, int H, int W, STSaved* sv, Carry* in_carry, Carry* out_carry) {
// ... 829 lines not shown
```

### morphablediffusion_amd/csrc/engine_weights.hip

```cpp
#include <algorithm>
#include <math.h>
#include <string.h>

#include "engine.h"

int engine_dmalloc(mvd_ctx* c, void** p, size_t bytes) {
  if (bytes == 0) bytes = 16;
  if (c->repacking) {
    if (c->repack_cursor >= c->sec_end || c->owned_bytes[c->repack_cursor] != bytes)
      return mvd_fail("engine_repack: allocation sequence differs from the first build");
    *p = c->owned[c->repack_cursor++];
    return 0;
  }
  HIP_CHECK_RET(hipMalloc(p, bytes));
  c->owned.push_back(*p);
  c->owned_bytes.push_back(bytes);
  return 0;
}

void engine_build_rotate(mvd_ctx* c) {
  if (c->bs_multi) c->bs = c->bstreams[(c->bs_rr++) & 3];
}
int engine_build_join(mvd_ctx* c) {
  if (!c->bs_multi) return 0;
// ... 374 lines not shown
  RET_IF(pack_conv(c, V + "quant_conv.weight", V + "quant_conv.bias", false, false, &v.quant, 0, c->vae_exact));
  v.present = true;
  return 0;
}

int build_vae(mvd_ctx* c) {
  const std::string V = "first_stage_model.", D = V + "decoder.";
  VaeW& v = c->vae;
  RawTensor *co, *ci, *pq;
  RET_IF(get_raw(c, D + "conv_out.weight", &co));
  RET_IF(get_raw(c, D + "conv_in.weight", &ci));
  RET_IF(get_raw(c, V + "post_quant_conv.weight", &pq));
  v.out_ch = (int)co->shape[0];
  v.ch = (int)co->shape[1];
  v.block_in = (int)ci->shape[0];
  v.zc = (int)ci->shape[1];
  v.embed = (int)pq->shape[1];
  if (v.out_ch > 4 || v.zc > 8 || (v.zc & 3) || v.embed > 8)
    return mvd_fail("VAE decoder: out_ch <= 4, z_channels in {4, 8} and embed_dim <= 8 expected");
  RET_IF(pack_conv(c, V + "post_quant_conv.weight", V + "post_quant_conv.bias", false, false, &v.post_quant, 8, c->vae_exact));
  RET_IF(pack_conv(c, D + "conv_in.weight", D + "conv_in.bias", false, false, &v.conv_in, 8, c->vae_exact));
  RET_IF(build_vae_res(c, D + "mid.block_1", &v.mid1));
  RET_IF(build_vae_res(c, D + "mid.block_2", &v.mid2));
  RET_IF(build_vae_attn(c, D + "mid.attn_1", &v.attn));
  v.nlev = 0;
  while (c->raw.count(D + "up." + std::to_string(v.nlev) + ".block.0.conv1.weight")) ++v.nlev;
  if (v.nlev < 1) return mvd_fail("VAE decoder: no up blocks uploaded");
  v.up.assign(v.nlev, {});
  v.up_conv.assign(v.nlev, ConvW());
  for (int l = 0; l < v.nlev; ++l) {
    const std::string L = D + "up." + std::to_string(l);
    for (int i = 0; c->raw.count(L + ".block." + std::to_string(i) + ".conv1.weight"); ++i) {
      VaeResW r;
      RET_IF(build_vae_res(c, L + ".block." + std::to_string(i), &r));
      v.up[l].push_back(r);
    }
    if (l > 0) {
      ConvW& uc = v.up_conv[l];
      RET_IF(pack_conv(c, L + ".upsample.conv.weight", L + ".upsample.conv.bias", false, false, &uc, 0, c->vae_exact));
      RawTensor* r;
      RET_IF(get_raw(c, L + ".upsample.conv.weight", &r));
      if (!c->vae_exact) {
        RET_IF(dmalloc(c, (void**)&uc.w_up, (size_t)16 * uc.N * uc.Cin * sizeof(half_t)));
        RET_IF(launch_pack_upconv_weight(r->d, uc.N, uc.Cin, uc.w_up, c->bs));
      }
    }
  }
  RET_IF(load_norm(c, D + "norm_out", &v.norm_out));
  {
    RawTensor pad, padb, *b;
    RET_IF(get_raw(c, D + "conv_out.bias", &b));
    const size_t per = co->numel / co->shape[0];
    pad.shape = {4, co->shape[1], co->shape[2], co->shape[3]};
    pad.numel = 4 * per;
    HIP_CHECK_RET(hipMalloc((void**)&pad.d, pad.numel * sizeof(float)));
    HIP_CHECK_RET(hipMemset(pad.d, 0, pad.numel * sizeof(float)));
    HIP_CHECK_RET(hipMemcpyAsync(pad.d, co->d, co->numel * sizeof(float), hipMemcpyDeviceToDevice, 0));
    padb.shape = {4};
    padb.numel = 4;
    HIP_CHECK_RET(hipMalloc((void**)&padb.d, 4 * sizeof(float)));
    HIP_CHECK_RET(hipMemset(padb.d, 0, 4 * sizeof(float)));
    HIP_CHECK_RET(hipMemcpyAsync(padb.d, b->d, b->numel * sizeof(float), hipMemcpyDeviceToDevice, 0));
    c->raw[D + "conv_out.weight.pad4"] = pad;
    c->raw[D + "conv_out.bias.pad4"] = padb;
    RET_IF(pack_conv(c, D + "conv_out.weight.pad4", D + "conv_out.bias.pad4", false, false, &v.conv_out, 0, c->vae_exact));
  }
  v.present = true;
  return 0;
}

int repack_xp(mvd_ctx* c, const std::string& wkey, ConvW* o, int cin_pad = 0) {
  if (o->xp) return 0;
  ConvW n;
  RET_IF(pack_conv(c, wkey, "", false, false, &n, cin_pad, true));
  n.bias = o->bias;
  n.bkey = o->bkey;
  n.w_up = nullptr;
  *o = n;
  return 0;
}

int xp_cond(mvd_ctx* c, CondW& d) {
  if (d.wqk.xp) return 0;
  const int heads = 4, hd = d.Cc / 2;
  RET_IF(repack_xp(c, d.key + ".proj_out.2.weight", &d.conv1));
  RET_IF(repack_xp(c, d.key + ".proj_out.5.weight", &d.conv2));
  RawTensor *wq, *wk, *wv, *wo;
  RET_IF(get_raw(c, d.key + ".depth_attn.to_q.weight", &wq));
  RET_IF(get_raw(c, d.key + ".depth_attn.to_k.weight", &wk));
  RET_IF(get_raw(c, d.key + ".depth_attn.to_v.weight", &wv));
  RET_IF(get_raw(c, d.key + ".depth_attn.to_out.weight", &wo));
  const size_t nf = (size_t)heads * d.Cc * d.I;
  float* tmp = nullptr;
  RET_IF(dmalloc(c, (void**)&tmp, nf * sizeof(float)));
  auto fold = [&](ConvW& w, int N, int Cl, bool qk) -> int {
    if (qk) RET_IF(launch_fold_qk(wq->d, wk->d, heads, hd, d.Cc, d.I, 1.0f / sqrtf((float)hd), nullptr, c->bs, tmp));
    else RET_IF(launch_fold_ov(wo->d, wv->d, heads, hd, d.Cc, d.I, nullptr, c->bs, tmp));
    w.N = N;
    w.cin_l = Cl;
    w.Cin = 3 * Cl;
    w.xp = 1;
    w.taps = 1;
    RET_IF(dmalloc(c, (void**)&w.w, (size_t)N * 3 * Cl * sizeof(half_t)));
    return launch_pack_weight(tmp, N, 3 * Cl, 1, 0, 0, w.w, c->bs, Cl, 1);
  };
  RET_IF(fold(d.wqk, heads * d.Cc, d.I, true));
  RET_IF(fold(d.wov, d.I, heads * d.Cc, false));
  RET_IF(dmalloc(c, (void**)&d.relu_beta, (size_t)3 * heads * d.Cc * sizeof(half_t)));
  return launch_relu_beta_tile(d.gn_ctx.b, d.Cc, heads, d.relu_beta, c->bs, 1);
}

int xp_ops(mvd_ctx* c, const std::vector<UOp>& ops, bool convs3) {
  for (const UOp& op : ops) {
    if (op.kind == OP_RES) {
      ResW& r = c->res[op.idx];
      if (r.has_skip) RET_IF(repack_xp(c, r.key + ".skip_connection.weight", &r.skip));
      if (convs3) {
        RET_IF(repack_xp(c, r.key + ".in_layers.2.weight", &r.c1));
        RET_IF(repack_xp(c, r.key + ".out_layers.3.weight", &r.c2));
      }
    } else if (op.kind == OP_ST) {
      STW& t = c->st[op.idx];
      RET_IF(repack_xp(c, t.key + ".proj_in.weight", &t.proj_in));
      RET_IF(repack_xp(c, t.key + ".proj_out.weight", &t.proj_out));
    }
  }
  return 0;
}

int build_conv3x_streams(mvd_ctx* c) {
  if (!mvd_env().conv3x || !c->has_unet) return 0;
  auto takes = [](int res) { return (res % 16 == 0 && res >= 16) || res == 8; };
  std::vector<ConvW*> cs;
  for (ResW& r : c->res) {
    if (!takes(r.res)) continue;
    cs.push_back(&r.c1);
    cs.push_back(&r.c2);
  }
  for (CondW& d : c->conds) {
    if (!takes(d.res)) continue;
    cs.push_back(&d.conv1);
    cs.push_back(&d.conv2);
  }
  for (ConvW& w : c->convs)
    if (w.res_out == 8 && !w.xp) cs.push_back(&w);
  for (ConvW* w : cs) {
    if (w->taps != 9 || w->Cin % 64) continue;
    const int bn = w->N % 160 == 0 ? 160 : (w->N % 128 == 0 ? 128 : 0);
    if (!bn) continue;
    engine_build_rotate(c);
    RET_IF(dmalloc(c, (void**)&w->wx, conv3x_stream_halfs(w->N, w->Cin, bn) * sizeof(half_t)));
    RET_IF(conv3x_pack(w->w, w->N, w->Cin, bn, w->wx, c->bs));
    w->wx_bn = bn;
  }
  return engine_build_join(c);
}

int build_rowchain_streams(mvd_ctx* c) {
  if (!c->has_unet || c->train_mode) return 0;
  for (STW& st : c->st) {
    const int C = st.C;
    if (!rc_supported_c(C)) continue;
    const std::string& p = st.key;
    const std::string t = p + ".transformer_blocks.0";
    engine_build_rotate(c);
    RawTensor *wao, *g3, *b3, *w1, *b1, *w2, *b2, *wpo;
    RET_IF(get_raw(c, t + ".attn1.to_out.0.weight", &wao));
    RET_IF(get_raw(c, t + ".norm3.weight", &g3));
    RET_IF(get_raw(c, t + ".norm3.bias", &b3));
    RET_IF(get_raw(c, t + ".ff.net.0.proj.weight", &w1));
    RET_IF(get_raw(c, t + ".ff.net.0.proj.bias", &b1));
    RET_IF(get_raw(c, t + ".ff.net.2.weight", &w2));
    RET_IF(get_raw(c, t + ".ff.net.2.bias", &b2));
    RET_IF(get_raw(c, p + ".proj_out.weight", &wpo));
    if (wao->numel != (size_t)C * C || w1->numel != (size_t)8 * C * C || w2->numel != (size_t)4 * C * C || wpo->numel != (size_t)C * C)
      return mvd_fail("build_rowchain_streams: transformer block weights do not have the row-chain kernel's shapes");
    st.rc_po = st.proj_out.xp ? 2 : 1;
    if (!rowchain_form_instantiated(C, 1, st.rc_po)) st.rc_po = 0;
    float* tmp = nullptr;
    RET_IF(dmalloc(c, (void**)&tmp, (size_t)8 * C * sizeof(float)));
    RET_IF(dmalloc(c, (void**)&st.rc_stream, rowchain_stream_halfs(C, 1, st.rc_po) * sizeof(half_t)));
    RcWeights rw;
    rw.w_ao = wao->d; rw.ln_g = g3->d; rw.ln_b = b3->d; rw.w1 = w1->d; rw.b1 = b1->d; rw.w2 = w2->d; rw.b2 = b2->d; rw.w_po = wpo->d;
    RET_IF(rowchain_pack(rw, C, 1, st.rc_po, tmp, st.rc_stream, c->bs));
    if (C == RH_C) {
      RawTensor *wpi, *g1, *b1n, *q, *k, *v;
      RET_IF(get_raw(c, p + ".proj_in.weight", &wpi));
      RET_IF(get_raw(c, t + ".norm1.weight", &g1));
      RET_IF(get_raw(c, t + ".norm1.bias", &b1n));
      RET_IF(get_raw(c, t + ".attn1.to_q.weight", &q));
      RET_IF(get_raw(c, t + ".attn1.to_k.weight", &k));
      RET_IF(get_raw(c, t + ".attn1.to_v.weight", &v));
      if (wpi->numel != (size_t)C * C || q->numel != (size_t)C * C) return mvd_fail("build_rowchain_streams: unexpected proj_in / to_q shape");
      st.rh_xp = st.proj_in.xp ? 1 : 0;
      RET_IF(dmalloc(c, (void**)&st.rh_stream, rowhead_stream_halfs(st.rh_xp) * sizeof(half_t)));
      RhWeights hw;
      hw.w_pi = wpi->d; hw.ln_g = g1->d; hw.ln_b = b1n->d; hw.w_q = q->d; hw.w_k = k->d; hw.w_v = v->d;
      RET_IF(rowhead_pack(hw, st.rh_xp, tmp, st.rh_stream, c->bs));
    }
  }
  return engine_build_join(c);
}

int build_ffp(mvd_ctx* c) {
  if (!mvd_env().ffp || !c->has_unet || c->train_mode) return 0;
  for (STW& st : c->st) {
    if (st.proj_out.xp || (st.C & 7)) continue;
    const int C = st.C;
    const std::string t = st.key + ".transformer_blocks.0";
    RawTensor *w2, *b2, *wpo, *bpo;
    RET_IF(get_raw(c, t + ".ff.net.2.weight", &w2));
    RET_IF(get_raw(c, t + ".ff.net.2.bias", &b2));
    RET_IF(get_raw(c, st.key + ".proj_out.weight", &wpo));
    RET_IF(get_raw(c, st.key + ".proj_out.bias", &bpo));
    if (w2->numel != (size_t)4 * C * C || wpo->numel != (size_t)C * C || b2->numel != (size_t)C || bpo->numel != (size_t)C) continue;
    engine_build_rotate(c);
    ConvW& f = st.ffp;
    f.N = C; f.Cin = 5 * C; f.cin_l = 5 * C; f.taps = 1;
    half_t* tmp16 = nullptr;
    float* tmp32 = nullptr;
    RET_IF(dmalloc(c, (void**)&f.w, (size_t)C * 5 * C * sizeof(half_t)));
    RET_IF(dmalloc(c, (void**)&f.bias, (size_t)C * sizeof(float)));
    RET_IF(dmalloc(c, (void**)&tmp16, (size_t)C * C * sizeof(half_t)));
    RET_IF(dmalloc(c, (void**)&tmp32, (size_t)C * sizeof(float)));
    RET_IF(launch_fold_mm(wpo->d, C, w2->d, 4 * C, C, 4 * C, C, f.w, 5 * C, nullptr, c->bs));
    RET_IF(launch_f32_to_f16(wpo->d, tmp16, (size_t)C * C, c->bs));
    HIP_CHECK_RET(hipMemcpy2DAsync(f.w + 4 * C, (size_t)5 * C * sizeof(half_t), tmp16, (size_t)C * sizeof(half_t), (size_t)C * sizeof(half_t), C,
                                   hipMemcpyDeviceToDevice, c->bs));
    RET_IF(launch_fold_mm(wpo->d, C, b2->d, 1, C, 1, C, nullptr, 1, tmp32, c->bs));
    RET_IF(launch_add_rows(f.bias, tmp32, bpo->d, (size_t)C, c->bs));
  }
  return engine_build_join(c);
}

int apply_xp_policy(mvd_ctx* c) {
  const int lvl = mvd_env_call::xp(c->precision_level);
  if (lvl <= 0 || !c->has_unet) return 0;
  const std::string U = "model.diffusion_model.";
  RET_IF(repack_xp(c, U + "out.2.weight", &c->out_conv));
  RET_IF(repack_xp(c, U + "input_blocks.0.0.weight", &c->convs[c->in_blocks[0][0].idx], 8));
  if (lvl < 2) return 0;
  const int nb = (int)c->out_blocks.size();
  const int nblk = lvl >= 5 ? 3 : (lvl >= 3 ? 2 : 1);
  for (int k = 0; k < nblk && k < nb; ++k) {
    const int bi = nb - 1 - k;
    RET_IF(xp_ops(c, c->out_blocks[bi], lvl >= 5 || (lvl >= 4 && k == 0)));
    if (bi >= 3 && 1 + (bi - 3) < (int)c->conds.size()) RET_IF(xp_cond(c, c->conds[1 + (bi - 3)]));
  }
  if (lvl >= 6)
    for (int j = 1; j <= 2 && j < (int)c->in_blocks.size(); ++j) RET_IF(xp_ops(c, c->in_blocks[j], true));
  return 0;
}

namespace {

int build_unet_section(mvd_ctx* c) {
  const std::string U = "model.diffusion_model.";
  const mvd_unet_config& u = c->u;
  const int mc = u.model_channels;
  const int temb = 4 * mc;
  c->res.clear();
  c->st.clear();
  c->convs.clear();
  c->conds.clear();
  c->in_blocks.clear();
  c->out_blocks.clear();
  c->mid_block.clear();
  c->emb_total = 0;
  c->a2_total = 0;
  RET_IF(pack_lin(c, U + "time_embed.0.weight", U + "time_embed.0.bias", &c->te0));
  RET_IF(pack_lin(c, U + "time_embed.2.weight", U + "time_embed.2.bias", &c->te2));
  struct EmbPiece {
    std::string key;
    int cout;
  };
  std::vector<EmbPiece> emb_pieces;
  auto add_res = [&](const std::string& name, int cin, int cout, std::vector<UOp>& ops) -> int {
    ResW r;
    RET_IF(build_res(c, U + name, cin, cout, &r));
    r.emb_off = c->emb_total;
    c->emb_total += cout;
    emb_pieces.push_back({U + name + ".emb_layers.1", cout});
    c->res.push_back(r);
    ops.push_back({OP_RES, (int)c->res.size() - 1, cin, cout});
    return 0;
  };
  std::vector<std::string> a2v_keys;
  auto add_st = [&](const std::string& name, int C, std::vector<UOp>& ops) -> int {
    STW s;
    RET_IF(build_st(c, U + name, C, &s));
    s.a2_off = c->a2_total;
    c->a2_total += C;
    a2v_keys.push_back(U + name + ".transformer_blocks.0.attn2");
    c->st.push_back(s);
    ops.push_back({OP_ST, (int)c->st.size() - 1, C, C});
    return 0;
  };
  auto add_conv = [&](const std::string& wkey, int kind, int cin, int cout, std::vector<UOp>& ops) -> int {
    ConvW w;
    RET_IF(pack_conv(c, U + wkey + ".weight", U + wkey + ".bias", false, false, &w));
    if (kind == OP_UP && w.taps == 9) {
      RawTensor* r;
      RET_IF(get_raw(c, U + wkey + ".weight", &r));
      RET_IF(dmalloc(c, (void**)&w.w_up, (size_t)16 * w.N * w.Cin * sizeof(half_t)));
      RET_IF(launch_pack_upconv_weight(r->d, w.N, w.Cin, w.w_up, c->bs));
    }
// ... 86 lines not shown
    }
  }
  c->a2_all.N = c->a2_total;
  c->a2_all.Cin = u.context_dim;
  c->a2_all.taps = 1;
  RET_IF(dmalloc(c, (void**)&c->a2_all.w, (size_t)c->a2_total * u.context_dim * sizeof(half_t)));
  RET_IF(dmalloc(c, (void**)&c->a2_all.bias, (size_t)c->a2_total * sizeof(float)));
  {
    size_t off = 0;
    for (auto& k : a2v_keys) {
      RawTensor *wv, *wo, *bo;
      RET_IF(get_raw(c, k + ".to_v.weight", &wv));
      RET_IF(get_raw(c, k + ".to_out.0.weight", &wo));
      RET_IF(get_raw(c, k + ".to_out.0.bias", &bo));
      const int C = (int)bo->numel;
      RET_IF(launch_fold_ov(wo->d, wv->d, 1, C, u.context_dim, C, c->a2_all.w + off * u.context_dim, c->bs));
      HIP_CHECK_RET(hipMemcpyAsync(c->a2_all.bias + off, bo->d, C * sizeof(float), hipMemcpyDeviceToDevice, c->bs));
      off += C;
    }
  }
  {
    const int c2 = mc * u.channel_mult[2], c1 = mc * u.channel_mult[1], c0 = mc * u.channel_mult[0];
    const int* d = u.volume_dims;
    const int dims[10] = {c2, c2, c2, c2, c1, c1, c1, c0, c0, c0};
    const int ccs[10] = {d[3], d[2], d[2], d[1], d[1], d[1], d[0], d[0], d[0], d[0]};
    const int lvl[10] = {3, 2, 2, 1, 1, 1, 0, 0, 0, 0};
    c->conds.resize(10);
    RET_IF(build_cond(c, U + "middle_conditions", dims[0], ccs[0], &c->conds[0]));
    for (int k = 0; k < 9; ++k)
      RET_IF(build_cond(c, U + "output_conditions." + std::to_string(k), dims[k + 1], ccs[k + 1], &c->conds[k + 1]));
    for (int k = 0; k < 10; ++k) c->conds[k].res = u.image_size >> lvl[k];
    c->ctx_groups.clear();
    for (int L = 0; L < 4; ++L) {
      mvd_ctx::CtxGroup gp;
      gp.level = L;
      for (int k = 0; k < 10; ++k)
        if (lvl[k] == L && gp.nblk < 4 && !c->conds[k].proj_ctx.xp && (gp.nblk == 0 || c->conds[k].Cc == gp.Cc)) {
          gp.Cc = c->conds[k].Cc;
          gp.cond[gp.nblk++] = k;
        }
      if (gp.nblk < 2) continue;
      const int Cc = gp.Cc, N = gp.nblk * Cc;
      gp.w.N = N; gp.w.Cin = Cc; gp.w.taps = 1;
      gp.gn.C = N;
      RET_IF(dmalloc(c, (void**)&gp.w.w, (size_t)N * Cc * sizeof(half_t)));
      RET_IF(dmalloc(c, (void**)&gp.gn.g, (size_t)N * sizeof(float)));
      RET_IF(dmalloc(c, (void**)&gp.gn.b, (size_t)N * sizeof(float)));
      for (int j = 0; j < gp.nblk; ++j) {
        const CondW& d = c->conds[gp.cond[j]];
        if (d.proj_ctx.N != Cc || d.proj_ctx.Cin != Cc) return mvd_fail("build_unet_section: unexpected proj_context shape");
        HIP_CHECK_RET(hipMemcpyAsync(gp.w.w + (size_t)j * Cc * Cc, d.proj_ctx.w, (size_t)Cc * Cc * sizeof(half_t), hipMemcpyDeviceToDevice, c->bs));
        HIP_CHECK_RET(hipMemcpyAsync(gp.gn.g + (size_t)j * Cc, d.gn_ctx.g, (size_t)Cc * sizeof(float), hipMemcpyDeviceToDevice, c->bs));
        HIP_CHECK_RET(hipMemcpyAsync(gp.gn.b + (size_t)j * Cc, d.gn_ctx.b, (size_t)Cc * sizeof(float), hipMemcpyDeviceToDevice, c->bs));
      }
      c->ctx_groups.push_back(gp);
    }
  }
  return 0;
}

int build_step_section(mvd_ctx* c) {
  RET_IF(pack_lin(c, "time_embed.0.weight", "time_embed.0.bias", &c->step_te0));
  RET_IF(pack_lin(c, "time_embed.2.weight", "time_embed.2.bias", &c->step_te2));
  return 0;
}

int build_condnet_section(mvd_ctx* c) {
  const std::string S = "spatial_volume.";
  RET_IF(pack_conv(c, S + "target_encoder.init_conv.weight", S + "target_encoder.init_conv.bias", false, false,
                   &c->enc_init, 8));
  for (int i = 0; i < 3; ++i) {
    const std::string p = S + "target_encoder.out_conv" + std::to_string(i) + ".";
    EncBlockW& e = c->enc_blocks[i];
    RET_IF(pack_lin(c, p + "time_embed.weight", p + "time_embed.bias", &e.t));
    RET_IF(pack_lin(c, p + "view_embed.weight", p + "view_embed.bias", &e.v));
    RET_IF(load_norm(c, p + "conv.0", &e.n1));
    RET_IF(pack_conv(c, p + "conv.2.weight", p + "conv.2.bias", false, false, &e.c1));
    RET_IF(load_norm(c, p + "conv.3", &e.n2));
    RET_IF(pack_conv(c, p + "conv.5.weight", p + "conv.5.bias", false, false, &e.c2));
  }
  RET_IF(load_norm(c, S + "target_encoder.final_out.0", &c->enc_final_norm));
  RET_IF(pack_conv(c, S + "target_encoder.final_out.2.weight", S + "target_encoder.final_out.2.bias", false, false,
                   &c->enc_final));
  RET_IF(copy_f32(c, S + "smpl_feature_extractor.conv0.weight", &c->fuse_w));
  RET_IF(copy_f32(c, S + "smpl_feature_extractor.conv0.bias", &c->fuse_b));
  {
    const char* blk[9] = {"conv0", "conv0", "down0", "conv1", "conv1", "down1", "conv2", "conv2", "conv2"};
    const int slot[9] = {0, 3, 0, 0, 3, 0, 0, 3, 6};
    for (int i = 0; i < 9; ++i)
      RET_IF(build_sparse_layer(c, S + "xyzc_net.", blk[i], slot[i], blk[i][0] == 'd', &c->sparse[i]));
  }
  const std::string F = S + "frustum_volume_feats.";
  RET_IF(pack_conv(c, F + "conv0.weight", F + "conv0.bias", false, false, &c->fr_conv0));
  for (int i = 0; i < 6; ++i)
    RET_IF(build_frustum_block(c, F + "conv" + std::to_string(i + 1) + ".", "bn", false, (i % 2 == 0) ? 2 : 1,
                               &c->fr_blocks[i]));
  for (int i = 0; i < 3; ++i)
    RET_IF(build_frustum_block(c, F + "up" + std::to_string(i) + ".", "norm", true, 2, &c->fr_up[i]));
  {
    auto stack = [&](const std::vector<std::string>& prefixes, const char* wn, LinW* out, int K) -> int {
      int total = 0;
      std::vector<RawTensor*> ws, bs;
      for (auto& p : prefixes) {
        RawTensor *wt, *bt;
        RET_IF(get_raw(c, p + wn + ".weight", &wt));
        RET_IF(get_raw(c, p + wn + ".bias", &bt));
        ws.push_back(wt);
        bs.push_back(bt);
        total += (int)wt->shape[0];
      }
      out->N = total;
      out->K = K;
      RET_IF(dmalloc(c, (void**)&out->w, (size_t)total * K * sizeof(half_t)));
      RET_IF(dmalloc(c, (void**)&out->bias, (size_t)total * sizeof(float)));
      size_t off = 0;
      for (size_t i = 0; i < ws.size(); ++i) {
        RET_IF(launch_f32_to_f16(ws[i]->d, out->w + off * K, ws[i]->numel, c->bs));
        HIP_CHECK_RET(hipMemcpyAsync(out->bias + off, bs[i]->d, bs[i]->numel * sizeof(float), hipMemcpyDeviceToDevice, c->bs));
        off += ws[i]->shape[0];
      }
      return 0;
    };
    std::vector<std::string> fp, ep;
    int off = 0;
    for (int i = 0; i < 9; ++i) {
      fp.push_back(i < 6 ? F + "conv" + std::to_string(i + 1) + "." : F + "up" + std::to_string(i - 6) + ".");
      c->film_off[i] = off;
      off += i < 6 ? c->fr_blocks[i].cin : c->fr_up[i - 6].cin;
    }
    c->film_total = off;
    RET_IF(stack(fp, "t_conv", &c->film_t, c->v.time_dim));
    RET_IF(stack(fp, "v_conv", &c->film_v, c->v.view_dim));
    for (int i = 0; i < 3; ++i) ep.push_back(S + "target_encoder.out_conv" + std::to_string(i) + ".");
    RET_IF(stack(ep, "time_embed", &c->enc_t, c->v.time_dim));
    RET_IF(stack(ep, "view_embed", &c->enc_v, c->v.view_dim));
  }
  return 0;
}

int build_hot_sections(mvd_ctx* c) {
  if (c->has_unet) {
    RET_IF(build_unet_section(c));
    RET_IF(apply_xp_policy(c));
    RET_IF(engine_build_join(c));
    RET_IF(build_conv3x_streams(c));
    RET_IF(build_rowchain_streams(c));
    RET_IF(build_ffp(c));
    if (c->train_mode) RET_IF(engine_build_dgrad(c));
  }
  if (c->has_step) RET_IF(build_step_section(c));
  if (c->has_cond) {
    RET_IF(build_condnet_section(c));
    RET_IF(engine_build_join(c));
    if (c->train_mode) RET_IF(engine_build_dgrad_cond(c));
  }
  return 0;
}

}

int engine_finalize(mvd_ctx* c) {
  const std::string U = "model.diffusion_model.";
  HIP_CHECK_RET(hipSetDevice(c->device));
  const bool has_unet = c->raw.count(U + "time_embed.0.weight") > 0;
  const bool has_cond = c->raw.count("spatial_volume.target_encoder.init_conv.weight") > 0;
  const bool has_step = c->raw.count("time_embed.0.weight") > 0;
  const bool has_vae = c->raw.count("first_stage_model.decoder.conv_in.weight") > 0;
  const bool has_vae_enc = c->raw.count("first_stage_model.encoder.conv_in.weight") > 0;
  const bool has_clip = c->raw.count("clip_image_encoder.model.visual.conv1.weight") > 0;
  if (!has_unet && !has_cond && !has_vae && !has_vae_enc && !has_clip)
    return mvd_fail("finalize: no UNet, spatial_volume, first-stage or CLIP weights were uploaded");
  if (has_clip) RET_IF(build_clip(c));
  if (has_vae) RET_IF(build_vae(c));
  if (has_vae_enc) RET_IF(build_vae_encoder(c));
  c->has_unet = has_unet;
  c->has_step = has_step;
  c->has_cond = has_cond;
  if (c->train_mode) RET_IF(engine_train_setup(c));
  for (auto& cc : c->cond_const) cc.valid = false;
  c->sec_begin = c->owned.size();
  RET_IF(build_hot_sections(c));
  c->sec_end = c->owned.size();
  HIP_CHECK_RET(hipDeviceSynchronize());
  for (auto it = c->raw.begin(); it != c->raw.end();) {
    if (c->train_mode && engine_hot_key(it->first)) {
      ++it;
      continue;
    }
    hipFree(it->second.d);
    it = c->raw.erase(it);
  }
  if (c->has_unet) RET_IF(engine_side_init(c));
  c->finalized = true;
  return 0;
}

int engine_repack(mvd_ctx* c, hipStream_t after, bool have_stream) {
  if (!c->finalized || !c->train_mode) return mvd_fail("engine_repack: the context was not finalized in training mode");
  HIP_CHECK_RET(hipSetDevice(c->device));
  const bool one_stream = mvd_env().repack_one_stream;
  if (!c->bstreams[0])
    for (int i = 0; i < 4; ++i) {
      HIP_CHECK_RET(hipStreamCreateWithFlags(&c->bstreams[i], hipStreamNonBlocking));
      HIP_CHECK_RET(hipEventCreateWithFlags(&c->bevents[i], hipEventDisableTiming));
    }
  if (!c->bev_after) HIP_CHECK_RET(hipEventCreateWithFlags(&c->bev_after, hipEventDisableTiming));
  if (have_stream) {
    HIP_CHECK_RET(hipEventRecord(c->bev_after, after));
    for (int i = 0; i < 4; ++i) HIP_CHECK_RET(hipStreamWaitEvent(c->bstreams[i], c->bev_after, 0));
  } else {
    HIP_CHECK_RET(hipDeviceSynchronize());
  }
  c->bs_multi = !one_stream;
  c->bs_rr = 0;
  c->bs = c->bstreams[0];
  c->repacking = true;
  c->repack_cursor = c->sec_begin;
  const int r = build_hot_sections(c);
  const bool complete = c->repack_cursor == c->sec_end;
  c->repacking = false;
  c->bs_multi = false;
  c->bs = 0;
  if (have_stream) {
    for (int i = 0; i < 4; ++i) {
      hipEventRecord(c->bevents[i], c->bstreams[i]);
      hipStreamWaitEvent(after, c->bevents[i], 0);
    }
  } else {
    hipDeviceSynchronize();
  }
  RET_IF(r);
  if (!complete) return mvd_fail("engine_repack: allocation sequence shorter than the first build");
  return 0;
}
```

### morphablediffusion_amd/csrc/env.h

```cpp
#pragma once

#define MVD_ENV_TABLE(PROCESS, ENGINE, CALL, PROCESS_CALL) \
   \
  ENGINE(off, halo, "MVD_NO_HALO", true, "3x3 convs on the gather kernel instead of the LDS-halo / conv3x kernels") \
  PROCESS_CALL(off, conv3x, "MVD_NO_CONV3X", true, "no conv3x fragment streams: 3x3 ResBlock convs on the LDS-halo kernel") \
  PROCESS(off, up_conv3x, "MVD_NO_UP_CONV3X", true, "the 4x4 -> 8x8 upsample conv as the 9-tap GEMM on the fp32 source, not upsample + conv3x") \
  PROCESS(off, gemm_dma, "MVD_NO_GEMM_DMA", true, "GEMMs / 1x1 convs on the older register-staged igemm kernel, not the LDS-DMA kernel") \
  PROCESS(num, dense_min_m, "MVD_DENSE_MIN_M", 64, "fewest rows routed to the LDS-DMA kernel (2 views per rank: 7.08 ms at 512, 6.97 ms at 64)") \
  PROCESS(off, plain, "MVD_NO_PLAIN", true, "general row mapping for plain GEMMs instead of the PLAIN instantiations") \
  PROCESS(on, old_plan, "MVD_OLD_PLAN", false, "k-step cost model (gemm_dma_plan) instead of gemm_dma_plan_us for plain GEMMs") \
  PROCESS(on, igemm_f32_bn128, "MVD_IGEMM_F32_BN128", false, "fp32 sources on 128-column tiles where 160 is picked (32768 x 960 x 320: 48 vs 37 us)") \
  PROCESS(on, bm128, "MVD_BM128", false, "offer the planner the four-wave 128-row tiles: measured, lost (profiles/r06_b_bm_sweep.txt)") \
  PROCESS(on, bm128_off, "MVD_NO_BM128", false, "overrides MVD_BM128: the 128-row tiles stay off") \
  PROCESS(num, dense_bn, "MVD_DENSE_BN", 0, "sweep (tools/gemm_plan_sweep.py): column-tile width of the dense launches, 0 = planner's") \
  PROCESS(num, dense_sk, "MVD_DENSE_SK", 0, "sweep: split-K of the dense launches, 0 = planner's") \
  PROCESS(num, dense_bm, "MVD_DENSE_BM", 0, "sweep: 128 = four-wave row tiles with MVD_DENSE_BN, else 256") \
  PROCESS(num, halo_bn, "MVD_HALO_BN", 0, "sweep (tools/conv_bench3.py): column width of the LDS-halo kernel, 0 = planner's") \
  PROCESS(num, halo_sk, "MVD_HALO_SK", 0, "sweep: split over 64-channel chunks of the LDS-halo kernel, 0 = planner's") \
  PROCESS(off, parity_batch, "MVD_NO_PARITY_BATCH", true, "one launch per output-parity class of the transposed / upsample convs, not one for all") \
  PROCESS(num, par_walk_min, "MVD_PAR_WALK_MIN", 0, "tiles from which a workgroup walks the parity classes, 0 = never (profiles/r06_y_ab_pwalk.txt: nothing)") \
  PROCESS(off, xcd_cols, "MVD_NO_XCD_COLS", true, "row-tile-major XCD walk always, never the column-major one (common.h: xcd_prefers_cols)") \
  PROCESS(off, attn_xcd, "MVD_ATTN_NO_XCD", true, "attention with the pre-remap workgroup order") \
   \
  PROCESS(num, defer_max, "MVD_DEFER_MAX", 16, "largest split a consumer takes as slabs (4 = the round-3 limit)") \
  PROCESS(off, defer_reduce, "MVD_NO_DEFER_REDUCE", true, "ResBlock conv1 with its own reduce pass; also turns off ln_defer and cond_defer") \
  PROCESS(off, cond_defer, "MVD_NO_COND_DEFER", true, "the DepthTransformer's GEMMs in front of a GroupNorm with their reduce passes") \
  PROCESS(on, ln_defer, "MVD_LN_DEFER", false, "LayerNorm sums the split-K slabs of proj_in / to_out (profiles/r06_g_ab_ln_defer.txt: no time gained)") \
  PROCESS(off, carry, "MVD_NO_CARRY", true, "a block's last GEMM reduces its own slabs instead of leaving them to the next block's GroupNorm") \
   \
  PROCESS(on, gn_two_pass, "MVD_GN_TWO_PASS", false, "two-pass GroupNorm everywhere; also turns off defer_reduce, cond_defer and out_conv_f32") \
  PROCESS(on, skip_side, "MVD_SKIP_SIDE", false, "the ResBlock's 1x1 skip conv on a helper stream (profiles/r06_z_ab_skip_side.txt: nothing)") \
  PROCESS(off, rowchain, "MVD_NO_ROWCHAIN", true, "the transformer block behind the attention as layered GEMMs, not the row-chain kernel") \
  PROCESS(num, rowchain_min_rows, "MVD_ROWCHAIN_MIN_ROWS", 16384, "fewest rows that take the row-chain kernel") \
  PROCESS(off, rowhead, "MVD_NO_ROWHEAD", true, "proj_in, LayerNorm1 and q | k | v as separate launches, not the row-head kernel") \
  PROCESS(off, xp_fuse, "MVD_NO_XP_FUSE", true, "extended-precision proj_in / proj_out as separate GEMMs beside the row kernels") \
  PROCESS(off, ffp, "MVD_NO_FFP", true, "FF2 and proj_out as two GEMMs, not one over [gg | t2]") \
  PROCESS(on, ln_scalar, "MVD_LN_SCALAR", false, "element-per-thread LayerNorm (also keeps FF2 and proj_out apart)") \
  PROCESS(off, ctx_fold, "MVD_NO_CTX_FOLD", true, "GroupNorm(proj_context(volume)) materialised, not folded into two GEMM passes") \
  PROCESS(off, ctx_group, "MVD_NO_CTX_GROUP", true, "context fold block by block, not once per level") \
  PROCESS(off, cond_const, "MVD_NO_COND_CONST", true, "DepthTransformer over all samples, context-free ones included (profiles/r06_i_ab_cond_const.txt)") \
  PROCESS(off, conv_in_f32, "MVD_NO_CONV_IN_F32", true, "the input conv on the MFMA forms, not in exact fp32 on the vector ALU") \
  PROCESS(off, out_conv_f32, "MVD_NO_OUT_CONV_F32", true, "the output head on the MFMA forms, not GroupNorm + conv in exact fp32") \
  PROCESS(off, side_stream, "MVD_NO_SIDE_STREAM", true, "context volumes and folds on the caller's stream") \
  PROCESS(off, side_emb, "MVD_NO_SIDE_EMB", true, "the timestep-embedding GEMMs on the caller's stream") \
  PROCESS(on, one_way_fork, "MVD_ONE_WAY_FORK", false, "side-stream fork without the acknowledgement: the round-1 race on demand (DESIGN.md section 4, tools/det_fork.sh)") \
   \
  PROCESS(off, fused_enc, "MVD_NO_FUSED_ENC", true, "the 2-D target encoder layer by layer, not as one launch") \
  CALL(one, bn_loop, "MVD_BN_LOOP", false, "the looped BatchNorm + ReLU kernel; tests/test_gpu_train.py flips it for its bit-identity check") \
  CALL(one, sparse_valu, "MVD_SPARSE_VALU", false, "read when sparse-conv weights are built: one-site-per-workgroup kernels and the scatter-form data gradient") \
  CALL(num, xp, "MVD_XP", precision_level, "overrides the engine's extended-precision level when the policy is applied") \
  PROCESS(on, stage_scalar, "MVD_STAGE_SCALAR", false, "element-per-thread staging kernels of the backward pass (profiles/r04_m_*)") \
  PROCESS(on, gn_bwd_one_block, "MVD_GN_BWD_ONE_BLOCK", false, "mvd_op_group_norm_bwd: one workgroup per (sample, group), not the slabbed form") \
  PROCESS(one, repack_one_stream, "MVD_REPACK_STREAMS", false, "=1: the training re-pack on one stream, not four") \
   \
  PROCESS(on, plan_debug, "MVD_PLAN_DEBUG", false, "print every dense plan as a [plan] line") \
  PROCESS(on, layer_timing, "MVD_LAYER_TIMING", false, "per-GEMM event time (tools/layer_step.py); synchronises every launch") \
  PROCESS(on, debug_sum, "MVD_DEBUG_SUM", false, "bit checksums of the step's buffers: which differ between repeats?") \
  PROCESS(on, mesh_timing, "MVD_MESH_TIMING", false, "host phases of set_mesh / set_samples") \
  PROCESS(on, cond_bwd_timing, "MVD_COND_BWD_TIMING", false, "host-side enqueue time of each conditioner-backward phase")

#include <stdlib.h>

inline bool mvd_env_on(const char* name, bool) { return getenv(name) != nullptr; }
inline bool mvd_env_off(const char* name, bool) { return getenv(name) == nullptr; }
inline bool mvd_env_one(const char* name, bool) { const char* v = getenv(name); return v && v[0] == '1'; }
inline int mvd_env_num(const char* name, int unset) { const char* v = getenv(name); return v ? atoi(v) : unset; }

#define MVD_ENV_SKIP(...)
#define MVD_ENV_FIELD(kind, field, name, def, doc) decltype(mvd_env_##kind(name, 0)) field = def;
#define MVD_ENV_PARSE(kind, field, name, def, doc) e.field = mvd_env_##kind(name, def);

struct MvdEnv {
  MVD_ENV_TABLE(MVD_ENV_FIELD, MVD_ENV_SKIP, MVD_ENV_SKIP, MVD_ENV_FIELD)
};
inline const MvdEnv& mvd_env() {
  static const MvdEnv env = [] {
    MvdEnv e;
    MVD_ENV_TABLE(MVD_ENV_PARSE, MVD_ENV_SKIP, MVD_ENV_SKIP, MVD_ENV_PARSE)
    e.ln_defer = e.ln_defer && e.defer_reduce;
    e.defer_reduce = e.defer_reduce && !e.gn_two_pass;
    e.cond_defer = e.cond_defer && e.defer_reduce;
    e.out_conv_f32 = e.out_conv_f32 && !e.gn_two_pass;
    e.bm128 = e.bm128 && !e.bm128_off;
    return e;
  }();
  return env;
}

struct MvdEnvEngine {
  MVD_ENV_TABLE(MVD_ENV_SKIP, MVD_ENV_FIELD, MVD_ENV_SKIP, MVD_ENV_SKIP)
};
inline MvdEnvEngine mvd_env_engine() {
  MvdEnvEngine e;
  MVD_ENV_TABLE(MVD_ENV_SKIP, MVD_ENV_PARSE, MVD_ENV_SKIP, MVD_ENV_SKIP)
  return e;
}

namespace mvd_env_call {
#define MVD_ENV_CALL_BOOL(kind, field, name, def) inline bool field() { return mvd_env_##kind(name, def); }
#define MVD_ENV_CALL_on MVD_ENV_CALL_BOOL
#define MVD_ENV_CALL_off MVD_ENV_CALL_BOOL
#define MVD_ENV_CALL_one MVD_ENV_CALL_BOOL
#define MVD_ENV_CALL_num(kind, field, name, def) inline int field(int unset) { return mvd_env_num(name, unset); }
#define MVD_ENV_CALL_FN(kind, field, name, def, doc) MVD_ENV_CALL_##kind(kind, field, name, def)
MVD_ENV_TABLE(MVD_ENV_SKIP, MVD_ENV_SKIP, MVD_ENV_CALL_FN, MVD_ENV_CALL_FN)
}
```

### morphablediffusion_amd/csrc/k_misc.hip

```cpp
#include "common.h"

namespace {

__global__ __launch_bounds__(256) void small_linear_kernel(const float* __restrict__ a, int lda, int rows, int K,
                                                           const half_t* __restrict__ w, const float* __restrict__ bias,
                                                           int N, int act_in, float* __restrict__ out, int ldo,
                                                           int accumulate) {
  const int lane = threadIdx.x & 63;
  const int n = blockIdx.x * 4 + (threadIdx.x >> 6);
  if (n >= N) return;
  const half_t* wr = w + (long)n * K;
  const int out_rows = rows < 0 ? -rows : rows;
  const int in_rows = rows < 0 ? 1 : rows;
  for (int r0 = 0; r0 < in_rows; r0 += 8) {
    float acc[8];
#pragma unroll
    for (int j = 0; j < 8; ++j) acc[j] = 0.f;
    if ((K & 7) == 0 && (lda & 3) == 0) {
      for (int k = lane * 8; k < K; k += 512) {
        const h8 wv = *(const h8*)(wr + k);
#pragma unroll
        for (int j = 0; j < 8; ++j) {
          if (r0 + j < in_rows) {
            const float4 a0 = *(const float4*)(a + (long)(r0 + j) * lda + k);
// ... 69 lines not shown
                                    int cpad) {
  const long total = (long)B * HW * cpad;
  for (long idx = (long)blockIdx.x * blockDim.x + threadIdx.x; idx < total; idx += (long)gridDim.x * blockDim.x) {
    const int c = (int)(idx % cpad);
    const long bp = idx / cpad;
    const int p = (int)(bp % HW), b = (int)(bp / HW);
    out[bp * ldo + c] = c < C ? in[((long)b * C + c) * HW + p] : 0.f;
  }
}

__global__ void nhwc_to_nchw_kernel(const float* __restrict__ in, int ld, int B, int C, int HW, float* __restrict__ out) {
  const long total = (long)B * C * HW;
  for (long idx = (long)blockIdx.x * blockDim.x + threadIdx.x; idx < total; idx += (long)gridDim.x * blockDim.x) {
    const int p = (int)(idx % HW);
    const long bc = idx / HW;
    const int c = (int)(bc % C), b = (int)(bc / C);
    out[idx] = in[((long)b * HW + p) * ld + c];
  }
}

__global__ __launch_bounds__(256) void nchw_to_nhwc_tiled_kernel(const float* __restrict__ in, int C, int HW, float* __restrict__ out, int ldo,
                                                                 int cpad) {
  __shared__ float tile[32][33];
  const int b = blockIdx.z, p0 = blockIdx.x * 32, c0 = blockIdx.y * 32, tx = threadIdx.x & 31, ty = threadIdx.x >> 5;
#pragma unroll
  for (int i = 0; i < 4; ++i) {
    const int c = c0 + ty + 8 * i, p = p0 + tx;
    tile[ty + 8 * i][tx] = (c < C && p < HW) ? in[((long)b * C + c) * HW + p] : 0.f;
  }
  __syncthreads();
#pragma unroll
  for (int i = 0; i < 4; ++i) {
    const int p = p0 + ty + 8 * i, c = c0 + tx;
    if (p < HW && c < cpad) out[((long)b * HW + p) * ldo + c] = tile[tx][ty + 8 * i];
  }
}
__global__ __launch_bounds__(256) void nhwc_to_nchw_tiled_kernel(const float* __restrict__ in, int ld, int C, int HW, float* __restrict__ out) {
  __shared__ float tile[32][33];
  const int b = blockIdx.z, p0 = blockIdx.x * 32, c0 = blockIdx.y * 32, tx = threadIdx.x & 31, ty = threadIdx.x >> 5;
#pragma unroll
  for (int i = 0; i < 4; ++i) {
    const int p = p0 + ty + 8 * i, c = c0 + tx;
    tile[ty + 8 * i][tx] = (p < HW && c < C) ? in[((long)b * HW + p) * ld + c] : 0.f;
  }
  __syncthreads();
#pragma unroll
  for (int i = 0; i < 4; ++i) {
    const int c = c0 + ty + 8 * i, p = p0 + tx;
    if (c < C && p < HW) out[((long)b * C + c) * HW + p] = tile[tx][ty + 8 * i];
  }
}

__global__ void pack_weight_kernel(const float* __restrict__ src, int N, int Cin, int taps, int transposed, int geglu,
                                   int cin_src, half_t* __restrict__ dst, int xp) {
  const long total = (long)taps * N * Cin;
  const int Cl = xp ? Cin / 3 : Cin;
  for (long idx = (long)blockIdx.x * blockDim.x + threadIdx.x; idx < total; idx += (long)gridDim.x * blockDim.x) {
    const int cp = (int)(idx % Cin), seg = cp / Cl, c = cp - seg * Cl;
    const long tn = idx / Cin;
    const int nd = (int)(tn % N), t = (int)(tn / N);
    int n = nd;
    if (geglu) {
      const int j = nd >> 6, wi = nd & 63;
      n = wi < 32 ? 32 * j + wi : N / 2 + 32 * j + (wi - 32);
    }
    if (c >= cin_src) {
      dst[idx] = (half_t)0;
      continue;
    }
    const long s = transposed ? ((long)c * N + n) * taps + t : ((long)n * cin_src + c) * taps + t;
    const float w = src[s];
    const half_t hi = (half_t)w;
    dst[idx] = seg < 2 ? hi : (half_t)(w - (float)hi);
  }
}

__global__ __launch_bounds__(256) void pack_weight_taps_kernel(const float* __restrict__ src, int N, int Cin, int taps, int geglu, int cin_src,
                                                               half_t* __restrict__ dst, int xp) {
  __shared__ float sw[64 * 27];
  const int Cl = xp ? Cin / 3 : Cin;
  const int nd = blockIdx.y, c0 = blockIdx.x * 64;
  int n = nd;
  if (geglu) {
    const int j = nd >> 6, wi = nd & 63;
    n = wi < 32 ? 32 * j + wi : N / 2 + 32 * j + (wi - 32);
  }
  const int nc = min(64, cin_src - c0);
  const float* p = src + ((long)n * cin_src + c0) * taps;
  for (int i = threadIdx.x; i < nc * taps; i += 256) sw[i] = p[i];
  __syncthreads();
  for (int i = threadIdx.x; i < 64 * taps; i += 256) {
    const int t = i >> 6, cl = i & 63, c = c0 + cl;
    if (c >= Cl) continue;
    const float w = cl < nc ? sw[cl * taps + t] : 0.f;
    const half_t hi = (half_t)w;
    half_t* d = dst + ((long)t * N + nd) * Cin + c;
    d[0] = hi;
    if (xp) {
      d[Cl] = hi;
      d[2 * Cl] = (half_t)(w - (float)hi);
    }
  }
}

__global__ __launch_bounds__(256) void pack_weight_taps_vec_kernel(const float* __restrict__ src, int N, int Cin, int taps, int geglu,
                                                                   int cin_src, half_t* __restrict__ dst, int xp) {
  __shared__ float sw[4][64 * 27];
  const int Cl = xp ? Cin / 3 : Cin;
  const int nd0 = blockIdx.y * 4, c0 = blockIdx.x * 64;
  const int nc = min(64, cin_src - c0);
#pragma unroll
  for (int rw = 0; rw < 4; ++rw) {
    const int nd = nd0 + rw;
    if (nd >= N) break;
    int n = nd;
    if (geglu) {
      const int j = nd >> 6, wi = nd & 63;
      n = wi < 32 ? 32 * j + wi : N / 2 + 32 * j + (wi - 32);
    }
    const float* p = src + ((long)n * cin_src + c0) * taps;
    for (int i = threadIdx.x; i < nc * taps; i += 256) sw[rw][i] = p[i];
  }
  __syncthreads();
  const int per_row = taps * 8;
  for (int i = threadIdx.x; i < 4 * per_row; i += 256) {
    const int rw = i / per_row, rem = i - rw * per_row, t = rem >> 3, cl = (rem & 7) * 8, c = c0 + cl, nd = nd0 + rw;
    if (nd >= N || c >= Cl) continue;
    h8 hi, lo;
#pragma unroll
    for (int k = 0; k < 8; ++k) {
      const float w = cl + k < nc ? sw[rw][(cl + k) * taps + t] : 0.f;
      hi[k] = (half_t)w;
      lo[k] = (half_t)(w - (float)hi[k]);
    }
    half_t* d = dst + ((long)t * N + nd) * Cin + c;
    *(h8*)d = hi;
    if (xp) {
      *(h8*)(d + Cl) = hi;
      *(h8*)(d + 2 * Cl) = lo;
    }
  }
}

__global__ void permute_geglu_bias_kernel(const float* __restrict__ src, int N, float* __restrict__ dst) {
  const int nd = blockIdx.x * blockDim.x + threadIdx.x;
  if (nd >= N) return;
  const int j = nd >> 6, wi = nd & 63;
  dst[nd] = src[wi < 32 ? 32 * j + wi : N / 2 + 32 * j + (wi - 32)];
}

__global__ void f32_to_f16_kernel(const float* __restrict__ in, half_t* __restrict__ out, size_t n) {
  for (size_t i = (size_t)blockIdx.x * blockDim.x + threadIdx.x; i < n; i += (size_t)gridDim.x * blockDim.x)
    out[i] = (half_t)in[i];
}

__global__ void rows_f32_to_f16_split_kernel(const float* __restrict__ in, int lda, long rows, int C, half_t* __restrict__ out) {
  const int q = C >> 2;
  const long total = rows * q;
  for (long i = (long)blockIdx.x * blockDim.x + threadIdx.x; i < total; i += (long)gridDim.x * blockDim.x) {
    const long r = i / q;
    const int c = (int)(i - r * q) * 4;
    const float4 v = *(const float4*)(in + r * lda + c);
    h4 hi, lo;
    hi[0] = (half_t)v.x; hi[1] = (half_t)v.y; hi[2] = (half_t)v.z; hi[3] = (half_t)v.w;
    lo[0] = (half_t)(v.x - (float)hi[0]); lo[1] = (half_t)(v.y - (float)hi[1]);
    lo[2] = (half_t)(v.z - (float)hi[2]); lo[3] = (half_t)(v.w - (float)hi[3]);
    half_t* o = out + r * 3 * C + c;
    *(h4*)o = hi;
    *(h4*)(o + C) = lo;
    *(h4*)(o + 2 * C) = hi;
  }
}

__global__ void rows_f32_to_f16_kernel(const float* __restrict__ in, int lda, long rows, int C, half_t* __restrict__ out) {
  const int q = C >> 2;
  const long total = rows * q;
  for (long i = (long)blockIdx.x * blockDim.x + threadIdx.x; i < total; i += (long)gridDim.x * blockDim.x) {
    const long r = i / q;
    const int c = (int)(i - r * q) * 4;
    const float4 v = *(const float4*)(in + r * lda + c);
    h4 o;
    o[0] = (half_t)v.x; o[1] = (half_t)v.y; o[2] = (half_t)v.z; o[3] = (half_t)v.w;
    *(h4*)(out + r * C + c) = o;
  }
}

__global__ void pack_upconv_weight_kernel(const float* __restrict__ src, int N, int Cin, half_t* __restrict__ dst) {
  const long total = (long)16 * N * Cin;
  for (long idx = (long)blockIdx.x * blockDim.x + threadIdx.x; idx < total; idx += (long)gridDim.x * blockDim.x) {
    const int c = (int)(idx % Cin);
    const int n = (int)((idx / Cin) % N);
    const int slab = (int)(idx / ((long)Cin * N));
    const int b = slab & 1, a = (slab >> 1) & 1, px = (slab >> 2) & 1, py = slab >> 3;
    const int ky0 = py == 0 ? (a == 0 ? 0 : 1) : (a == 0 ? 0 : 2), ky1 = py == 0 ? (a == 0 ? 0 : 2) : (a == 0 ? 1 : 2);
    const int kx0 = px == 0 ? (b == 0 ? 0 : 1) : (b == 0 ? 0 : 2), kx1 = px == 0 ? (b == 0 ? 0 : 2) : (b == 0 ? 1 : 2);
    const float* w = src + ((long)n * Cin + c) * 9;
    float acc = 0.f;
    for (int ky = ky0; ky <= ky1; ++ky)
      for (int kx = kx0; kx <= kx1; ++kx) acc += w[ky * 3 + kx];
    dst[idx] = (half_t)acc;
  }
}

__global__ void fill_rows_f16_kernel(half_t* __restrict__ out, int ld, int rows, const half_t* __restrict__ vec, int n) {
  const long total = (long)rows * n;
  for (long idx = (long)blockIdx.x * blockDim.x + threadIdx.x; idx < total; idx += (long)gridDim.x * blockDim.x) {
    const int c = (int)(idx % n);
    out[(idx / n) * ld + c] = vec[c];
  }
}

__global__ __launch_bounds__(256) void fold_gemm_kernel(const float* __restrict__ a, long a_zs, long a_rs, long a_cs,
                                                        const float* __restrict__ b, long b_zs, long b_rs, long b_cs, int M, int N, int K,
                                                        float scale, long c_zs, long c_rs, long c_cs, half_t* __restrict__ out,
                                                        float* __restrict__ out32) {
  __shared__ float sA[16][68], sB[16][68];
  const int tx = threadIdx.x & 15, ty = threadIdx.x >> 4, z = blockIdx.z;
  const int m0 = blockIdx.y * 64, n0 = blockIdx.x * 64;
  const float* az = a + z * a_zs;
  const float* bz = b + z * b_zs;
  double acc[4][4];
#pragma unroll
  for (int i = 0; i < 4; ++i)
#pragma unroll
    for (int j = 0; j < 4; ++j) acc[i][j] = 0.0;
  for (int k0 = 0; k0 < K; k0 += 16) {
#pragma unroll
    for (int e = 0; e < 4; ++e) {
      const int ml = ty + 16 * e, ka = k0 + tx;
      sA[tx][ml] = (m0 + ml < M && ka < K) ? az[(long)(m0 + ml) * a_rs + (long)ka * a_cs] : 0.f;
      const int nl = tx + 16 * e, kb = k0 + ty;
      sB[ty][nl] = (kb < K && n0 + nl < N) ? bz[(long)kb * b_rs + (long)(n0 + nl) * b_cs] : 0.f;
    }
    __syncthreads();
#pragma unroll
    for (int kk = 0; kk < 16; ++kk) {
      double av[4], bv[4];
#pragma unroll
      for (int i = 0; i < 4; ++i) av[i] = (double)sA[kk][ty + 16 * i];
#pragma unroll
      for (int j = 0; j < 4; ++j) bv[j] = (double)sB[kk][tx + 16 * j];
#pragma unroll
      for (int i = 0; i < 4; ++i)
#pragma unroll
        for (int j = 0; j < 4; ++j) acc[i][j] += av[i] * bv[j];
    }
    __syncthreads();
  }
#pragma unroll
  for (int i = 0; i < 4; ++i)
#pragma unroll
    for (int j = 0; j < 4; ++j) {
      const int m = m0 + ty + 16 * i, n = n0 + tx + 16 * j;
      if (m < M && n < N) {
        const long o = z * c_zs + (long)m * c_rs + (long)n * c_cs;
        const float v = (float)(acc[i][j] * (double)scale);
        if (out32) out32[o] = v;
        else out[o] = (half_t)v;
      }
    }
}

__global__ void relu_beta_tile_kernel(const float* __restrict__ beta, int Cc, int heads, half_t* __restrict__ out, int split) {
  const int idx = blockIdx.x * blockDim.x + threadIdx.x;
  const int W4 = heads * Cc;
  if (idx >= W4) return;
  const float v = fmaxf(beta[idx % Cc], 0.f);
  const half_t hi = (half_t)v;
  out[idx] = hi;
  if (split) {
    out[W4 + idx] = (half_t)(v - (float)hi);
    out[2 * W4 + idx] = hi;
  }
}

__global__ void cfg_ddim_kernel(const float* __restrict__ ec, const float* __restrict__ eu, float scale,
                                const float* __restrict__ x, const float* __restrict__ noise, float s1m, float sqrt_at,
                                float sqrt_aprev, float dir_coef, float sigma, float* __restrict__ eps_out,
                                float* __restrict__ x_prev, size_t n) {
  for (size_t i = (size_t)blockIdx.x * blockDim.x + threadIdx.x; i < n; i += (size_t)gridDim.x * blockDim.x) {
    float e = ec[i];
    if (eu) e = eu[i] + scale * (e - eu[i]);
    if (eps_out) eps_out[i] = e;
    if (x_prev) {
      const float pred_x0 = (x[i] - s1m * e) / sqrt_at;
      float xp = sqrt_aprev * pred_x0 + dir_coef * e;
      if (noise) xp += sigma * noise[i];
      x_prev[i] = xp;
    }
  }
}

__device__ __forceinline__ void dpm_elem(float ec, const float eu, bool has_eu, float scale, float x, float z, bool has_z, float h,
                                         bool use_hist, const DpmCoef& k, float& e, float& pred_x0, float& xn) {
  e = ec;
  if (has_eu) e = eu + scale * (e - eu);
  pred_x0 = (x - k.s1m * e) / k.sqrt_at;
  xn = k.c_x * x + k.c_d * pred_x0;
  if (use_hist) xn += k.c_c * (pred_x0 - h);
  if (has_z) xn += k.c_n * z;
}

__global__ void cfg_dpm_kernel(const float* __restrict__ ec, const float* __restrict__ eu, float scale, const float* __restrict__ x,
                               const float* __restrict__ noise, DpmCoef k, float* x0_hist, int use_hist,
                               float* __restrict__ eps_out, float* __restrict__ x_next, size_t n, int vec) {
  const size_t stride = (size_t)gridDim.x * blockDim.x, tid = (size_t)blockIdx.x * blockDim.x + threadIdx.x;
  const size_t n4 = vec ? n / 4 : 0;
  const float4 zero4 = make_float4(0.f, 0.f, 0.f, 0.f);
  for (size_t q = tid; q < n4; q += stride) {
    const float4 c4 = reinterpret_cast<const float4*>(ec)[q];
    const float4 u4 = eu ? reinterpret_cast<const float4*>(eu)[q] : zero4;
    const float4 x4 = reinterpret_cast<const float4*>(x)[q];
    const float4 z4 = noise ? reinterpret_cast<const float4*>(noise)[q] : zero4;
    const float4 h4 = use_hist ? reinterpret_cast<const float4*>(x0_hist)[q] : zero4;
    float4 e4, p4, n4v;
    dpm_elem(c4.x, u4.x, eu, scale, x4.x, z4.x, noise, h4.x, use_hist, k, e4.x, p4.x, n4v.x);
    dpm_elem(c4.y, u4.y, eu, scale, x4.y, z4.y, noise, h4.y, use_hist, k, e4.y, p4.y, n4v.y);
    dpm_elem(c4.z, u4.z, eu, scale, x4.z, z4.z, noise, h4.z, use_hist, k, e4.z, p4.z, n4v.z);
    dpm_elem(c4.w, u4.w, eu, scale, x4.w, z4.w, noise, h4.w, use_hist, k, e4.w, p4.w, n4v.w);
    if (eps_out) reinterpret_cast<float4*>(eps_out)[q] = e4;
    reinterpret_cast<float4*>(x0_hist)[q] = p4;
    reinterpret_cast<float4*>(x_next)[q] = n4v;
  }
  for (size_t i = n4 * 4 + tid; i < n; i += stride) {
    float e, p, xn;
    dpm_elem(ec[i], eu ? eu[i] : 0.f, eu, scale, x[i], noise ? noise[i] : 0.f, noise, use_hist ? x0_hist[i] : 0.f, use_hist, k, e, p,
             xn);
    if (eps_out) eps_out[i] = e;
    x0_hist[i] = p;
    x_next[i] = xn;
  }
}

__global__ void add_rows_kernel(float* __restrict__ dst, const float* __restrict__ a, const float* __restrict__ b, size_t n) {
  for (size_t i = (size_t)blockIdx.x * blockDim.x + threadIdx.x; i < n; i += (size_t)gridDim.x * blockDim.x)
    dst[i] = a[i] + (b ? b[i] : 0.f);
}

inline int grid_for(size_t n, int block = 256, int cap = 4096) {
  size_t g = (n + block - 1) / block;
  if (g > (size_t)cap) g = cap;
  if (g < 1) g = 1;
  return (int)g;
}

}

int launch_small_linear(const float* a, int lda, int rows, int K, const half_t* w, const float* bias, int N,
                        int act_in, float* out, int ldo, int accumulate, hipStream_t s) {
  hipLaunchKernelGGL(small_linear_kernel, dim3(cdiv(N, 4)), dim3(256), 0, s, a, lda, rows, K, w, bias, N, act_in, out,
                     ldo, accumulate);
  HIP_CHECK_RET(hipGetLastError());
  return 0;
}

int launch_timestep_embedding(const int64_t* t, int B, int dim, float* out, hipStream_t s) {
  hipLaunchKernelGGL(timestep_embedding_kernel, dim3(cdiv(B * dim, 256)), dim3(256), 0, s, t, B, dim, out);
  HIP_CHECK_RET(hipGetLastError());
  return 0;
}

int launch_nchw_to_nhwc(const float* in, int B, int C, int HW, float* out, int ldo, int cpad, hipStream_t s) {
  if (C >= 16 && HW >= 32 && B <= 65535 && cdiv(cpad, 32) <= 65535)
    hipLaunchKernelGGL(nchw_to_nhwc_tiled_kernel, dim3(cdiv(HW, 32), cdiv(cpad, 32), B), dim3(256), 0, s, in, C, HW, out, ldo, cpad);
  else
    hipLaunchKernelGGL(nchw_to_nhwc_kernel, dim3(grid_for((size_t)B * HW * cpad)), dim3(256), 0, s, in, B, C, HW, out,
                       ldo, cpad);
  HIP_CHECK_RET(hipGetLastError());
  return 0;
}

int launch_nhwc_to_nchw(const float* in, int ld, int B, int C, int HW, float* out, hipStream_t s) {
  if (C >= 16 && HW >= 32 && B <= 65535 && cdiv(C, 32) <= 65535)
    hipLaunchKernelGGL(nhwc_to_nchw_tiled_kernel, dim3(cdiv(HW, 32), cdiv(C, 32), B), dim3(256), 0, s, in, ld, C, HW, out);
  else
    hipLaunchKernelGGL(nhwc_to_nchw_kernel, dim3(grid_for((size_t)B * HW * C)), dim3(256), 0, s, in, ld, B, C, HW, out);
  HIP_CHECK_RET(hipGetLastError());
  return 0;
}

int launch_pack_weight(const float* src, int N, int Cin, int taps, int transposed, int geglu, half_t* dst,
                       hipStream_t s, int cin_src, int xp) {
  if (xp && Cin % 3) return mvd_fail("pack_weight: the extended-precision layout needs Cin = 3 * Cl");
  if (cin_src <= 0) cin_src = xp ? Cin / 3 : Cin;
  if (taps > 1 && taps <= 27 && !transposed && N <= 65535) {
    const int Cl = xp ? Cin / 3 : Cin;
    if (!(Cl & 7) && !((uintptr_t)dst & 15))
      hipLaunchKernelGGL(pack_weight_taps_vec_kernel, dim3(cdiv(Cl, 64), cdiv(N, 4)), dim3(256), 0, s, src, N, Cin, taps, geglu, cin_src,
                         dst, xp);
    else
      hipLaunchKernelGGL(pack_weight_taps_kernel, dim3(cdiv(Cl, 64), N), dim3(256), 0, s, src, N, Cin, taps, geglu, cin_src, dst, xp);
    HIP_CHECK_RET(hipGetLastError());
    return 0;
  }
  hipLaunchKernelGGL(pack_weight_kernel, dim3(grid_for((size_t)N * Cin * taps)), dim3(256), 0, s, src, N, Cin, taps,
                     transposed, geglu, cin_src, dst, xp);
  HIP_CHECK_RET(hipGetLastError());
  return 0;
}

int launch_permute_geglu_bias(const float* src, int N, float* dst, hipStream_t s) {
  hipLaunchKernelGGL(permute_geglu_bias_kernel, dim3(cdiv(N, 256)), dim3(256), 0, s, src, N, dst);
  HIP_CHECK_RET(hipGetLastError());
  return 0;
}

int launch_f32_to_f16(const float* in, half_t* out, size_t n, hipStream_t s) {
  hipLaunchKernelGGL(f32_to_f16_kernel, dim3(grid_for(n)), dim3(256), 0, s, in, out, n);
  HIP_CHECK_RET(hipGetLastError());
  return 0;
}

int launch_rows_f32_to_f16(const float* in, int lda, long rows, int C, half_t* out, hipStream_t s) {
  if ((C & 3) || (lda & 3)) return mvd_fail("rows_f32_to_f16: C and lda must be multiples of 4");
  hipLaunchKernelGGL(rows_f32_to_f16_kernel, dim3(grid_for((size_t)rows * C / 4)), dim3(256), 0, s, in, lda, rows, C, out);
  HIP_CHECK_RET(hipGetLastError());
  return 0;
}

int launch_rows_f32_to_f16_split(const float* in, int lda, long rows, int C, half_t* out, hipStream_t s) {
  if ((C & 3) || (lda & 3)) return mvd_fail("rows_f32_to_f16_split: C and lda must be multiples of 4");
  hipLaunchKernelGGL(rows_f32_to_f16_split_kernel, dim3(grid_for((size_t)rows * C / 4)), dim3(256), 0, s, in, lda, rows, C, out);
  HIP_CHECK_RET(hipGetLastError());
  return 0;
}

int launch_pack_upconv_weight(const float* src, int N, int Cin, half_t* dst, hipStream_t s) {
  hipLaunchKernelGGL(pack_upconv_weight_kernel, dim3(grid_for((size_t)16 * N * Cin)), dim3(256), 0, s, src, N, Cin, dst);
  HIP_CHECK_RET(hipGetLastError());
  return 0;
}

int launch_fill_rows_f16(half_t* out, int ld, int rows, const half_t* vec, int n, hipStream_t s) {
  hipLaunchKernelGGL(fill_rows_f16_kernel, dim3(grid_for((size_t)rows * n)), dim3(256), 0, s, out, ld, rows, vec, n);
  HIP_CHECK_RET(hipGetLastError());
  return 0;
}

int launch_fold_qk(const float* wq, const float* wk, int heads, int hd, int Cc, int I, float scale, half_t* out,
                   hipStream_t s, float* out32) {
  hipLaunchKernelGGL(fold_gemm_kernel, dim3(cdiv(I, 64), cdiv(Cc, 64), heads), dim3(256), 0, s, wk, (long)hd * Cc, 1L, (long)Cc, wq,
                     (long)hd * I, (long)I, 1L, Cc, I, hd, scale, (long)Cc * I, (long)I, 1L, out, out32);
  HIP_CHECK_RET(hipGetLastError());
  return 0;
}

int launch_fold_ov(const float* wo, const float* wv, int heads, int hd, int Cc, int I, half_t* out, hipStream_t s,
                   float* out32) {
  hipLaunchKernelGGL(fold_gemm_kernel, dim3(cdiv(Cc, 64), cdiv(I, 64), heads), dim3(256), 0, s, wo, (long)hd, (long)I, 1L, wv,
                     (long)hd * Cc, (long)Cc, 1L, I, Cc, hd, 1.0f, (long)Cc, (long)heads * Cc, 1L, out, out32);
  HIP_CHECK_RET(hipGetLastError());
  return 0;
}

int launch_fold_mm(const float* a, int lda, const float* b, int ldb, int M, int N, int K, half_t* out16, int ldc, float* out32,
                   hipStream_t s) {
  hipLaunchKernelGGL(fold_gemm_kernel, dim3(cdiv(N, 64), cdiv(M, 64), 1), dim3(256), 0, s, a, 0L, (long)lda, 1L, b, 0L, (long)ldb, 1L, M, N, K,
                     1.0f, 0L, (long)ldc, 1L, out16, out32);
  HIP_CHECK_RET(hipGetLastError());
  return 0;
}

int launch_relu_beta_tile(const float* beta, int Cc, int heads, half_t* out, hipStream_t s, int split) {
  hipLaunchKernelGGL(relu_beta_tile_kernel, dim3(cdiv(heads * Cc, 256)), dim3(256), 0, s, beta, Cc, heads, out, split);
  HIP_CHECK_RET(hipGetLastError());
  return 0;
}

int launch_cfg_ddim(const float* eps_c, const float* eps_u, float scale, const float* x, const float* noise,
                    float sqrt_one_minus_at, float sqrt_at, float sqrt_aprev, float dir_coef, float sigma,
                    float* eps_out, float* x_prev, size_t n, hipStream_t s) {
  hipLaunchKernelGGL(cfg_ddim_kernel, dim3(grid_for(n)), dim3(256), 0, s, eps_c, eps_u, scale, x, noise,
                     sqrt_one_minus_at, sqrt_at, sqrt_aprev, dir_coef, sigma, eps_out, x_prev, n);
  HIP_CHECK_RET(hipGetLastError());
  return 0;
}

int launch_cfg_dpm(const float* eps_c, const float* eps_u, float scale, const float* x, const float* noise, DpmCoef k,
                   float* x0_hist, int use_hist, float* eps_out, float* x_next, size_t n, hipStream_t s) {
  if (n == 0) return 0;
  if (!eps_c || !x || !x0_hist || !x_next) return mvd_fail("launch_cfg_dpm: null argument");
  const auto al = [](const void* p) { return ((uintptr_t)p & 15) == 0; };
  const int vec = al(eps_c) && al(eps_u) && al(x) && al(noise) && al(x0_hist) && al(eps_out) && al(x_next);
  const size_t work = vec ? n / 4 + (n & 3) : n;
  hipLaunchKernelGGL(cfg_dpm_kernel, dim3(grid_for(work)), dim3(256), 0, s, eps_c, eps_u, scale, x, noise, k, x0_hist, use_hist ? 1 : 0,
                     eps_out, x_next, n, vec);
  HIP_CHECK_RET(hipGetLastError());
  return 0;
}

__global__ void bits_checksum_kernel(const unsigned* __restrict__ p, size_t nwords, unsigned long long* __restrict__ out) {
  unsigned long long a = 0;
  for (size_t i = (size_t)blockIdx.x * blockDim.x + threadIdx.x; i < nwords; i += (size_t)gridDim.x * blockDim.x)
    a += (unsigned long long)p[i] * 0x9E3779B97F4A7C15ull + (i & 0xFFFF);
  atomicAdd(out, a);
}
int launch_bits_checksum(const void* p, size_t bytes, unsigned long long* out, hipStream_t s) {
  hipMemsetAsync(out, 0, 8, s);
  hipLaunchKernelGGL(bits_checksum_kernel, dim3(512), dim3(256), 0, s, (const unsigned*)p, bytes / 4, out);
  HIP_CHECK_RET(hipGetLastError());
  return 0;
}

int launch_add_rows(float* dst, const float* a, const float* b, size_t n, hipStream_t s) {
  hipLaunchKernelGGL(add_rows_kernel, dim3(grid_for(n)), dim3(256), 0, s, dst, a, b, n);
  HIP_CHECK_RET(hipGetLastError());
  return 0;
}

namespace {
__global__ void probe_null_kernel() {}
}
int launch_probe_null(hipStream_t s) {
  hipLaunchKernelGGL(probe_null_kernel, dim3(1), dim3(64), 0, s);
  return hipGetLastError() == hipSuccess ? 0 : mvd_fail("probe_null launch failed");
}

namespace {
__global__ __launch_bounds__(256) void add_image_rows_kernel(const float* __restrict__ in, int ldi, const float* __restrict__ img, int C4,
                                                             long total4, int HW, float* __restrict__ out, int ldo) {
  for (long i = (long)blockIdx.x * blockDim.x + threadIdx.x; i < total4; i += (long)gridDim.x * blockDim.x) {
    const long row = i / C4;
    const int q = (int)(i - row * C4), p = (int)(row % HW);
    const float4 a = *(const float4*)(in + row * ldi + q * 4), k = *(const float4*)(img + ((long)p * C4 + q) * 4);
    *(float4*)(out + row * ldo + q * 4) = make_float4(a.x + k.x, a.y + k.y, a.z + k.z, a.w + k.w);
  }
}
}
int launch_add_image_rows(const float* in, int ldi, const float* img, int C, int nb, int HW, float* out, int ldo, hipStream_t s) {
  if ((C & 3) || (ldi & 3) || (ldo & 3) || (((uintptr_t)in | (uintptr_t)img | (uintptr_t)out) & 15))
    return mvd_fail("add_image_rows: 16-byte aligned rows");
  const long total4 = (long)nb * HW * (C / 4);
  if (total4 <= 0) return 0;
  long blocks = (total4 + 255) / 256;
  if (blocks > 4096) blocks = 4096;
  hipLaunchKernelGGL(add_image_rows_kernel, dim3((unsigned)blocks), dim3(256), 0, s, in, ldi, img, C / 4, total4, HW, out, ldo);
  HIP_CHECK_RET(hipGetLastError());
  return 0;
}

namespace {
__global__ __launch_bounds__(256) void upsample2_f16_kernel(const float* __restrict__ in, int ldi, int B, int H, int W, int C4,
                                                            half_t* __restrict__ out) {
  const long total = (long)B * 4 * H * W * C4;
  for (long i = (long)blockIdx.x * blockDim.x + threadIdx.x; i < total; i += (long)gridDim.x * blockDim.x) {
    const int q = (int)(i % C4);
    long p = i / C4;
    const int x = (int)(p % (2 * W));
    p /= 2 * W;
    const int y = (int)(p % (2 * H)), b = (int)(p / (2 * H));
    const float4 v = *(const float4*)(in + (((long)b * H + (y >> 1)) * W + (x >> 1)) * ldi + q * 4);
    h4 o;
    o[0] = (half_t)v.x; o[1] = (half_t)v.y; o[2] = (half_t)v.z; o[3] = (half_t)v.w;
    *(h4*)(out + i * 4) = o;
  }
}
}
int launch_upsample2_f16(const float* in, int ldi, int B, int H, int W, int C, half_t* out, hipStream_t s) {
  if ((C & 3) || (ldi & 3) || (((uintptr_t)in | (uintptr_t)out) & 15)) return mvd_fail("upsample2_f16: 16-byte aligned rows");
  const long total = (long)B * 4 * H * W * (C / 4);
  if (total <= 0) return 0;
  long blocks = (total + 255) / 256;
  if (blocks > 4096) blocks = 4096;
  hipLaunchKernelGGL(upsample2_f16_kernel, dim3((unsigned)blocks), dim3(256), 0, s, in, ldi, B, H, W, C / 4, out);
  HIP_CHECK_RET(hipGetLastError());
// ... 155 lines not shown
```

### morphablediffusion_amd/engine.py

```python
import collections
import ctypes as C
import os
from typing import Dict, Optional

import torch

from . import lib as L
from .spec import UNetConfig, VolumeConfig


def _stream():
    return C.c_void_p(torch.cuda.current_stream().cuda_stream)


def _f32(t, device):
    return t.detach().to(device=device, dtype=torch.float32).contiguous()


IncompatibleKeys = collections.namedtuple("IncompatibleKeys", ["missing_keys", "unexpected_keys"])
MAX_SAMPLE_SLOTS = 64


def _level_dims(d, s):
    out = []
# ... 433 lines not shown
        v = _f32(volume, self.device)
        L.check(self.lib.mvd_set_volume(self._ctx, L.ptr(v), _stream()))

    def mse_loss(self, a, b):
        a, b = _f32(a, self.device), _f32(b, self.device)
        out = torch.empty(1, device=self.device, dtype=torch.float32)
        L.check(self.lib.mvd_mse_loss(self._ctx, L.ptr(a), L.ptr(b), C.c_size_t(a.numel()), L.ptr(out), _stream()))
        return out[0]

    def frustum_volumes_batch(self, slots, volumes, t_embed, v_rows, view_idx):
        dev = self.device
        vol, te, vr = _f32(volumes, dev), _f32(t_embed, dev), _f32(v_rows, dev)
        vi = view_idx.to(device=dev, dtype=torch.int32).contiguous()
        B = vol.shape[0]
        outs, ptrs = {}, []
        for lvl, (Dl, Sl) in enumerate(_level_dims(self.vcfg.frustum_volume_depth, self.vcfg.frustum_volume_size)):
            o = torch.empty(B, self.vcfg.frustum_dims[lvl], Dl, Sl, Sl, device=dev, dtype=torch.float32)
            outs[Sl] = o
            ptrs.append(L.ptr(o))
        L.check(self.lib.mvd_frustum_volumes_batch(self._ctx, B, (C.c_int * B)(*[int(v) for v in slots]), L.ptr(vol), L.ptr(te), L.ptr(vr),
                                                   L.ptr(vi), *ptrs, _stream()))
        return outs

    def frustum_volumes(self, t_embed, v_embed, view_idx):
        dev = self.device
        vi = view_idx.to(device=dev, dtype=torch.int32).contiguous()
        TN = vi.shape[0]
        outs = {}
        ptrs = []
        for lvl, (Dl, Sl) in enumerate(_level_dims(self.vcfg.frustum_volume_depth, self.vcfg.frustum_volume_size)):
            o = torch.empty(TN, self.vcfg.frustum_dims[lvl], Dl, Sl, Sl, device=dev, dtype=torch.float32)
            outs[Sl] = o
            ptrs.append(L.ptr(o))
        te, ve = _f32(t_embed, dev), _f32(v_embed, dev)
        L.check(self.lib.mvd_frustum_volumes(self._ctx, L.ptr(te), L.ptr(ve), L.ptr(vi), TN, *ptrs, _stream()))
        return outs

    def denoise_views(self, x_noisy, x_input, clip, timestep, t_embed, v_embed, view_idx, cfg_scale, noise, coef,
                      want_eps=False, out=None, eps_out=None):
        dev = self.device
        x = _f32(x_noisy, dev)
        vi = view_idx.to(device=dev, dtype=torch.int32).contiguous()
        TN = vi.shape[0]

        def direct(t):
            return t is not None and t.is_contiguous() and t.dtype == torch.float32 and t.device == x.device and t.shape == x.shape

        x_prev = out if direct(out) else torch.empty_like(x)
        eps = (eps_out if direct(eps_out) else torch.empty_like(x)) if want_eps else None
        nz = None if noise is None else _f32(noise, dev)
        xi, cl, te, ve = _f32(x_input, dev), _f32(clip, dev), _f32(t_embed, dev), _f32(v_embed, dev)
        L.check(self.lib.mvd_denoise_views(
            self._ctx, L.ptr(x), L.ptr(xi), L.ptr(cl), C.c_int64(int(timestep)),
            L.ptr(te), L.ptr(ve), L.ptr(vi), TN, C.c_float(cfg_scale), L.ptr(nz),
            C.c_float(coef[0]), C.c_float(coef[1]), C.c_float(coef[2]), C.c_float(coef[3]), C.c_float(coef[4]),
            L.ptr(eps), L.ptr(x_prev), _stream()))
        if out is not None and x_prev is not out:
            out.copy_(x_prev)
        if want_eps and eps_out is not None and eps is not eps_out:
            eps_out.copy_(eps)
        return (x_prev, eps) if want_eps else x_prev

    def denoise_views_batch(self, slots, x_noisy, x_input, clip, timesteps, t_embed, v_embed, view_idx, cfg_scale, noise, coef,
                            want_eps=False):
        dev = self.device
        x = _f32(x_noisy, dev)
        B, TN = x.shape[:2]
        vi = view_idx.to(device=dev, dtype=torch.int32).contiguous()
        assert vi.shape[0] == TN and len(slots) == B and len(timesteps) == B
        x_prev = torch.empty_like(x)
        eps = torch.empty_like(x) if want_eps else None
        nz = None if noise is None else _f32(noise, dev)
        xi, cl, te, ve = _f32(x_input, dev), _f32(clip, dev), _f32(t_embed, dev), _f32(v_embed, dev)
        sl = (C.c_int * B)(*[int(v) for v in slots])
        ts = (C.c_int64 * B)(*[int(v) for v in timesteps])
        L.check(self.lib.mvd_denoise_views_batch(
            self._ctx, B, sl, L.ptr(x), L.ptr(xi), L.ptr(cl), ts, L.ptr(te), L.ptr(ve), L.ptr(vi), TN, C.c_float(cfg_scale),
            L.ptr(nz), C.c_float(coef[0]), C.c_float(coef[1]), C.c_float(coef[2]), C.c_float(coef[3]), C.c_float(coef[4]),
            L.ptr(eps), L.ptr(x_prev), _stream()))
        return (x_prev, eps) if want_eps else x_prev

    def denoise_views_ms(self, slots, x_noisy, x_input, clip, timesteps, t_embed, v_embed, view_idx, cfg_scale, noise, coef,
                         x0_hist, first, want_eps=False, out=None, eps_out=None):
        dev = self.device
        x = _f32(x_noisy, dev)
        single = slots is None
        B, TN = (1, x.shape[0]) if single else x.shape[:2]
        vi = view_idx.to(device=dev, dtype=torch.int32).contiguous()
        steps = [timesteps] if single else list(timesteps)
        assert vi.shape[0] == TN and len(steps) == B and (single or len(slots) == B)
        if not (x0_hist.is_contiguous() and x0_hist.dtype == torch.float32 and x0_hist.device == x.device and x0_hist.shape == x.shape):
            raise ValueError("x0_hist must be a contiguous float32 tensor on the engine's device shaped like x_noisy")

        def direct(t):
            return t is not None and t.is_contiguous() and t.dtype == torch.float32 and t.device == x.device and t.shape == x.shape

        x_next = out if direct(out) else torch.empty_like(x)
        eps = (eps_out if direct(eps_out) else torch.empty_like(x)) if want_eps else None
        nz = None if noise is None else _f32(noise, dev)
        xi, cl, te, ve = _f32(x_input, dev), _f32(clip, dev), _f32(t_embed, dev), _f32(v_embed, dev)
        sl = None if single else (C.c_int * B)(*[int(v) for v in slots])
        ts = (C.c_int64 * B)(*[int(v) for v in steps])
        L.check(self.lib.mvd_denoise_views_ms(
            self._ctx, B, sl, L.ptr(x), L.ptr(xi), L.ptr(cl), ts, L.ptr(te), L.ptr(ve), L.ptr(vi), TN, C.c_float(cfg_scale),
            L.ptr(nz), *[C.c_float(v) for v in coef], L.ptr(x0_hist), 1 if first else 0, L.ptr(eps), L.ptr(x_next), _stream()))
        if out is not None and x_next is not out:
            out.copy_(x_next)
        if want_eps and eps_out is not None and eps is not eps_out:
            eps_out.copy_(eps)
        return (x_next, eps) if want_eps else x_next

    def op_cfg_ms(self, eps_c, eps_u, scale, x, noise, coef, x0_hist, first, want_eps=False):
        dev = self.device
        ec, x = _f32(eps_c, dev), _f32(x, dev)
        eu = None if eps_u is None else _f32(eps_u, dev)
        nz = None if noise is None else _f32(noise, dev)
        assert x0_hist.is_contiguous() and x0_hist.dtype == torch.float32 and x0_hist.numel() == x.numel()
        x_next = torch.empty_like(x)
        eps = torch.empty_like(x) if want_eps else None
        L.check(self.lib.mvd_op_cfg_ms(L.ptr(ec), L.ptr(eu), C.c_float(scale), L.ptr(x), L.ptr(nz), *[C.c_float(v) for v in coef],
                                       L.ptr(x0_hist), 1 if first else 0, L.ptr(eps), L.ptr(x_next), C.c_size_t(x.numel()),
                                       _stream()))
        return (x_next, eps) if want_eps else x_next

    def op_conv(self, x, w, bias=None, stride=1, upsample=0, resid=None, force_splitk=0):
        dev = self.device
        x, w = _f32(x, dev), _f32(w, dev)
        B, Cin, H, W = x.shape
        Cout, k = w.shape[0], w.shape[2]
        Ho, Wo = ((H << upsample) - 1) // stride + 1, ((W << upsample) - 1) // stride + 1
        out = torch.empty(B, Cout, Ho, Wo, device=dev)
        b = None if bias is None else _f32(bias, dev)
        r = None if resid is None else _f32(resid, dev)
        L.check(self.lib.mvd_op_conv(self._ctx, L.ptr(x), B, Cin, H, W, L.ptr(w), L.ptr(b), Cout, k, stride, upsample,
                                     L.ptr(r), L.ptr(out), force_splitk, _stream()))
        return out

    def op_conv3d(self, x, w, bias=None, stride=1, transposed=False, resid=None):
        dev = self.device
        x, w = _f32(x, dev), _f32(w, dev)
        B, Cin, D, H, W = x.shape
        Cout = w.shape[1] if transposed else w.shape[0]
        if transposed:
            od = (2 * D, 2 * H, 2 * W)
        else:
            od = ((D - 1) // stride + 1, (H - 1) // stride + 1, (W - 1) // stride + 1)
        out = torch.empty(B, Cout, *od, device=dev)
        b = None if bias is None else _f32(bias, dev)
        r = None if resid is None else _f32(resid, dev)
        L.check(self.lib.mvd_op_conv3d(self._ctx, L.ptr(x), B, Cin, D, H, W, L.ptr(w), L.ptr(b), Cout, stride,
                                       1 if transposed else 0, L.ptr(r), L.ptr(out), _stream()))
        return out

    def op_linear(self, a, w, bias=None, geglu=False, resid=None, a_half=False, force_splitk=0):
        dev = self.device
        a, w = _f32(a, dev), _f32(w, dev)
        M, K = a.shape
        N = w.shape[0]
        out = torch.empty(M, N // 2 if geglu else N, device=dev)
        b = None if bias is None else _f32(bias, dev)
        r = None if resid is None else _f32(resid, dev)
        L.check(self.lib.mvd_op_linear(self._ctx, L.ptr(a), M, K, L.ptr(w), L.ptr(b), N, 1 if geglu else 0, L.ptr(r),
                                       1 if a_half else 0, int(force_splitk), L.ptr(out), _stream()))
        return out

    def op_group_norm(self, x, groups, gamma, beta, eps, act=0):
        dev = self.device
        x = _f32(x, dev)
        B, Cc = x.shape[:2]
        HW = x[0, 0].numel()
        out = torch.empty_like(x)
        g, b = _f32(gamma, dev), _f32(beta, dev)
        L.check(self.lib.mvd_op_group_norm(self._ctx, L.ptr(x), B, Cc, HW, groups, L.ptr(g), L.ptr(b), C.c_float(eps),
                                           act, L.ptr(out), _stream()))
        return out

    def op_layer_norm(self, x, gamma, beta):
        dev = self.device
        x = _f32(x, dev)
        out = torch.empty_like(x)
        g, b = _f32(gamma, dev), _f32(beta, dev)
        L.check(self.lib.mvd_op_layer_norm(self._ctx, L.ptr(x), x.shape[0], x.shape[1], L.ptr(g), L.ptr(b), L.ptr(out),
                                           _stream()))
        return out

    def op_st_tail(self, xin, ln_g, ln_b, w1, b1, w2, b2, ao=None, w_ao=None, b_ao=None, rowbias=None, T=None, w_po=None, b_po=None,
                   resid=None, split=False, iters=0, xp_out=False):
        dev = self.device
        xin = _f32(xin, dev)
        rows, Cc = xin.shape
        keep = [_f32(t, dev) if t is not None else None for t in (ao, rowbias, w_ao, b_ao, ln_g, ln_b, w1, b1, w2, b2, w_po, b_po, resid)]
        ao_, rb_, wao_, bao_, g_, b_, w1_, b1_, w2_, b2_, wpo_, bpo_, res_ = keep
        flags = (1 if ao is not None else 0) | (2 if w_po is not None else 0) | (4 if split else 0) | (8 if xp_out else 0)
        out = torch.empty_like(xin)
        ms = C.c_float(0)
        L.check(self.lib.mvd_op_st_tail(self._ctx, Cc, rows, int(T or rows), L.ptr(ao_), L.ptr(xin), L.ptr(rb_), L.ptr(wao_), L.ptr(bao_),
                                        L.ptr(g_), L.ptr(b_), L.ptr(w1_), L.ptr(b1_), L.ptr(w2_), L.ptr(b2_), L.ptr(wpo_), L.ptr(bpo_),
                                        L.ptr(res_), L.ptr(out), flags, int(iters), C.byref(ms), _stream()))
        return (out, ms.value) if iters > 0 else out

    def op_st_head(self, n0, w_pi, b_pi, ln_g, ln_b, w_q, w_k, w_v, iters=0, xp=False):
        dev = self.device
        n0 = _f32(n0, dev)
        rows, Cc = n0.shape
        keep = [_f32(t, dev) for t in (w_pi, b_pi, ln_g, ln_b, w_q, w_k, w_v)]
        t0 = torch.empty(rows, Cc, device=dev)
        qkv = torch.empty(rows, 3 * Cc, device=dev)
        ms = C.c_float(0)
        L.check(self.lib.mvd_op_st_head(self._ctx, rows, 1 if xp else 0, L.ptr(n0), *[L.ptr(t) for t in keep], L.ptr(t0), L.ptr(qkv), int(iters),
                                        C.byref(ms), _stream()))
        return (t0, qkv, ms.value) if iters > 0 else (t0, qkv)

    def op_attention(self, q, k, v, heads):
        dev = self.device
        q, k, v = _f32(q, dev), _f32(k, dev), _f32(v, dev)
        B, T, Cc = q.shape
        out = torch.empty_like(q)
        L.check(self.lib.mvd_op_attention(self._ctx, L.ptr(q), L.ptr(k), L.ptr(v), B, T, heads, Cc // heads, L.ptr(out),
                                          _stream()))
        return out

    def op_attention_bwd(self, q, k, v, d_out, heads):
        dev = self.device
        q, k, v, d_out = _f32(q, dev), _f32(k, dev), _f32(v, dev), _f32(d_out, dev)
        B, T, Cc = q.shape
        dq, dk, dv = torch.empty_like(q), torch.empty_like(q), torch.empty_like(q)
        L.check(self.lib.mvd_op_attention_bwd(self._ctx, L.ptr(q), L.ptr(k), L.ptr(v), L.ptr(d_out), B, T, heads, Cc // heads,
                                              L.ptr(dq), L.ptr(dk), L.ptr(dv), _stream()))
        return dq, dk, dv

    def op_group_norm_bwd(self, x, dy, groups, gamma, beta, eps, act=0):
        dev = self.device
        x, dy, g, b = _f32(x, dev), _f32(dy, dev), _f32(gamma, dev), _f32(beta, dev)
        B, rows, Cc = x.shape
        dx, dg, db = torch.empty_like(x), torch.empty_like(g), torch.empty_like(g)
        L.check(self.lib.mvd_op_group_norm_bwd(self._ctx, L.ptr(x), L.ptr(dy), B, rows, Cc, groups, L.ptr(g), L.ptr(b), C.c_float(eps),
                                               act, L.ptr(dx), L.ptr(dg), L.ptr(db), _stream()))
        return dx, dg, db

    def op_layer_norm_bwd(self, x, dy, gamma):
        dev = self.device
        x, dy, g = _f32(x, dev), _f32(dy, dev), _f32(gamma, dev)
        dx, dg, db = torch.empty_like(x), torch.empty_like(g), torch.empty_like(g)
        L.check(self.lib.mvd_op_layer_norm_bwd(self._ctx, L.ptr(x), L.ptr(dy), x.shape[0], x.shape[1], L.ptr(g), L.ptr(dx), L.ptr(dg),
                                               L.ptr(db), _stream()))
        return dx, dg, db

    def _pad_last(self, t, n):
        t = _f32(t, self.device)
        return t if t.shape[-1] == n else torch.nn.functional.pad(t, (0, n - t.shape[-1])).contiguous()

    def op_conv_bwd(self, x, w, dy, kind=0, x_half=False, xp=False, accum=None, need_din=True, poison=False):
        dev = self.device
        B, Cin, H, W = x.shape
        Cout, k = w.shape[0], w.shape[2]
        cp = (Cin + 7) // 8 * 8
        xn = self._pad_last(x.permute(0, 2, 3, 1), cp)
        dyn = _f32(dy.permute(0, 2, 3, 1), dev)
        ww = _f32(w, dev)
        dx = torch.zeros(B, H, W, cp, device=dev)
        dW = torch.zeros(Cout, Cin * k * k, device=dev)
        db = torch.zeros(Cout, device=dev)
        if accum is not None:
            dx.copy_(self._pad_last(accum[0].permute(0, 2, 3, 1), cp))
            dW.copy_(accum[1].reshape(Cout, -1))
            db.copy_(accum[2])
        L.check(self.lib.mvd_op_conv_bwd(self._ctx, int(kind), int(k), B, Cin, H, W, Cout, L.ptr(xn), 1 if x_half else 0, L.ptr(ww), L.ptr(dyn),
                                         1 if xp else 0, 1 if accum is not None else 0, 1 if need_din else 0, 1 if poison else 0,
                                         L.ptr(dx), L.ptr(dW), L.ptr(db), _stream()))
        dxo = dx[..., :Cin].permute(0, 3, 1, 2).contiguous() if need_din else None
        return dxo, dW.view_as(w), db

    def op_linear_bwd(self, x, w, dy, B=1, bias=None, x_half=False, geglu=False, dx_half=False, staged=True, xp=False, accum=None,
                      poison=False):
        dev = self.device
        rows, K = x.shape
        N = w.shape[0]
        kp = (K + 7) // 8 * 8
        xn, dyn, ww = self._pad_last(x, kp), _f32(dy, dev), _f32(w, dev)
        bb = None if bias is None else _f32(bias, dev)
        dx = torch.zeros(rows, kp, device=dev)
        dW = torch.zeros(N, K, device=dev)
        db = torch.zeros(N, device=dev)
        if accum is not None:
            dx.copy_(self._pad_last(accum[0], kp))
            dW.copy_(accum[1])
            db.copy_(accum[2])
        L.check(self.lib.mvd_op_linear_bwd(self._ctx, int(B), rows, K, N, L.ptr(xn), 1 if x_half else 0, L.ptr(ww), L.ptr(bb), L.ptr(dyn),
                                           1 if geglu else 0, 1 if dx_half else 0, 1 if staged else 0, 1 if xp else 0,
                                           1 if accum is not None else 0, 1 if poison else 0, L.ptr(dx), L.ptr(dW), L.ptr(db), _stream()))
        return dx[:, :K].contiguous(), dW, db

    def op_conv3d_bwd(self, x, w, dy, kind=0, x_half=False, accum=None, poison=False):
        dev = self.device
        B, Cin, D, H, W = x.shape
        Cout = w.shape[1] if kind == 2 else w.shape[0]
        xn = _f32(x.permute(0, 2, 3, 4, 1), dev)
        dyn = _f32(dy.permute(0, 2, 3, 4, 1), dev)
        ww = _f32(w, dev)
        dx = torch.zeros(B, D, H, W, Cin, device=dev)
        dW = torch.zeros(w.shape, device=dev)
        db = torch.zeros(Cout, device=dev)
        if accum is not None:
            dx.copy_(accum[0].permute(0, 2, 3, 4, 1))
            dW.copy_(accum[1])
            db.copy_(accum[2])
# ... 75 lines not shown
```

### morphablediffusion_amd/lib.py

```python
import ctypes as C
import os

_HERE = os.path.dirname(os.path.abspath(__file__))
DTYPE = os.environ.get("MVD_DTYPE", "f16")
if DTYPE not in ("f16", "bf16"):
    raise ValueError(f"MVD_DTYPE must be f16 or bf16, not {DTYPE!r}")
LIB_PATH = os.environ.get("MVD_LIB_PATH", os.path.join(_HERE, "libmvd_hip.so" if DTYPE == "f16" else "libmvd_hip_bf16.so"))

SYMBOLS = [
    "mvd_create", "mvd_destroy", "mvd_last_error", "mvd_compute_dtype", "mvd_upload_weight", "mvd_set_precision_level", "mvd_set_vae_precision", "mvd_finalize_weights", "mvd_unet_forward", "mvd_unet_block",
    "mvd_embed_time", "mvd_select_sample", "mvd_set_mesh", "mvd_set_cameras", "mvd_set_mesh_async", "mvd_set_cameras_async", "mvd_set_samples_async", "mvd_rulebook_build", "mvd_rulebook_table", "mvd_vertex_features", "mvd_vertex_view_features", "mvd_vertex_features_stream_safe", "mvd_fuse_vertex_features",
    "mvd_comm_unique_id", "mvd_comm_init", "mvd_comm_destroy", "mvd_exchange_view_features", "mvd_comm_all_reduce", "mvd_train_sync_gradients",
    "mvd_stage_target_encoder", "mvd_stage_sparse_dense", "mvd_set_volume_ready_event", "mvd_volume_from_fused", "mvd_volume_from_fused_train", "mvd_mse_loss", "mvd_set_volume", "mvd_train_enable", "mvd_train_param_count", "mvd_train_param_info", "mvd_train_arena_size", "mvd_train_adopt_arena", "mvd_train_zero_grad", "mvd_train_unet_step", "mvd_train_get_grad", "mvd_train_get_tensor", "mvd_train_bn_calls", "mvd_train_cond_backward", "mvd_train_conditioner_backward", "mvd_train_conditioner_backward_batch", "mvd_train_adamw_step", "mvd_train_repack", "mvd_train_repack_async", "mvd_train_grad_bucket_count", "mvd_train_grad_bucket", "mvd_train_grad_bucket_wait", "mvd_train_set_bucket_snapshot",
    "mvd_frustum_volumes", "mvd_frustum_volumes_batch", "mvd_denoise_views", "mvd_denoise_views_batch", "mvd_denoise_views_ms", "mvd_op_cfg_ms", "mvd_op_conv", "mvd_op_linear", "mvd_op_group_norm",
    "mvd_op_layer_norm", "mvd_op_attention", "mvd_op_attention_bwd", "mvd_op_group_norm_bwd", "mvd_op_layer_norm_bwd", "mvd_op_conv3d", "mvd_op_conv_bwd", "mvd_op_linear_bwd", "mvd_op_conv3d_bwd", "mvd_op_tgemm", "mvd_op_st_tail", "mvd_op_st_head", "mvd_bench_conv", "mvd_bench_linear", "mvd_bench_group_norm", "mvd_probe_config", "mvd_probe_report", "mvd_vae_decode", "mvd_vae_encode",
    "mvd_clip_encode", "mvd_clip_embed_dim",
]


def csrc_sha16():
    import glob
    import hashlib
    h = hashlib.sha256()
    files = sorted(glob.glob(os.path.join(_HERE, "csrc", "*.hip")) + glob.glob(os.path.join(_HERE, "csrc", "*.h")) +
                   [os.path.join(_HERE, "csrc", "Makefile"), os.path.join(_HERE, "..", "include", "mvd.h")])
    for f in files:
        h.update(os.path.basename(f).encode())
        with open(f, "rb") as fh:
            h.update(fh.read())
    return h.hexdigest()[:16]


class UNetConfigC(C.Structure):
    _fields_ = [("image_size", C.c_int), ("in_channels", C.c_int), ("out_channels", C.c_int),
                ("model_channels", C.c_int), ("num_res_blocks", C.c_int), ("channel_mult", C.c_int * 4),
                ("num_heads", C.c_int), ("context_dim", C.c_int), ("volume_dims", C.c_int * 4),
                ("attention_levels", C.c_int)]


class VolumeConfigC(C.Structure):
    _fields_ = [("time_dim", C.c_int), ("view_dim", C.c_int), ("num_views", C.c_int), ("input_image_size", C.c_int),
                ("frustum_volume_depth", C.c_int), ("spatial_volume_size", C.c_int),
                ("spatial_volume_length", C.c_float), ("frustum_volume_length", C.c_float), ("projection", C.c_int),
                ("frustum_dims", C.c_int * 4), ("voxel_size", C.c_float)]


class MvdError(RuntimeError):
    pass


_lib = None


def load():
    global _lib
    if _lib is not None:
        return _lib
    if not os.path.exists(LIB_PATH):
        raise MvdError(f"{LIB_PATH} not found: build it with `python -c 'import __graft_entry__ as g; g.build()'` "
                       f"(hipcc --offload-arch=gfx950). There is no CPU fallback.")
    lib = C.CDLL(LIB_PATH)
    lib.mvd_last_error.restype = C.c_char_p
    lib.mvd_compute_dtype.restype = C.c_char_p
    lib.mvd_destroy.restype = None
    for name in SYMBOLS:
        if not hasattr(lib, name):
            raise MvdError(f"libmvd_hip.so does not export {name}")
    for name in SYMBOLS:
        if name not in ("mvd_last_error", "mvd_destroy", "mvd_compute_dtype"):
            getattr(lib, name).restype = C.c_int
    lib.mvd_train_arena_size.restype = C.c_int64
    lib.mvd_train_bn_calls.restype = C.c_int64
    if "MVD_LIB_PATH" not in os.environ and lib.mvd_compute_dtype().decode() != DTYPE:
        raise MvdError(f"{LIB_PATH} computes in {lib.mvd_compute_dtype().decode()}, MVD_DTYPE asks for {DTYPE}")
    _lib = lib
    return lib


def check(rc):
    if rc != 0:
        raise MvdError(load().mvd_last_error().decode())


def ptr(t):
    if t is None:
        return C.c_void_p(0)
    assert t.is_contiguous(), "tensor must be contiguous at the C boundary"
    return C.c_void_p(t.data_ptr())
```

Measured before the change: 78.80 steps/s.

## Add 3-D halo-tile MFMA kernels for frustum network level-0 27-tap convs

Adds a dedicated conv3d kernel that loads a 3-D halo tile of the input into LDS once and streams prepacked weight fragments through a 4-stage LDS ring, replacing the implicit-GEMM path for the frustum network's first conv and last transposed conv. The goal is to reuse input voxels across all 27 taps instead of re-gathering them, and to handle all eight transposed parity classes in a single launch. Weight streams are prepacked at build time; an env flag disables the path. It adds a sizeable new kernel with complex indexing, and these convs may be a small share of each denoise step.

```diff
diff --git a/include/mvd.h b/include/mvd.h
--- a/include/mvd.h
+++ b/include/mvd.h
@@ -158,6 +158,9 @@
                      float* out, void* stream);
 int mvd_op_conv3d(mvd_ctx* ctx, const float* x_ncdhw, int B, int Cin, int D, int H, int W, const float* w,
                   const float* bias, int Cout, int stride, int transposed, const float* resid, float* out, void* stream);
+int mvd_op_conv3d_form(mvd_ctx* ctx, const float* x_ncdhw, int B, int Cin, int D, int H, int W, const float* w,
+                       const float* bias, int Cout, int stride, int transposed, const float* resid, int out_half, int poison,
+                       float* out, void* stream);
 int mvd_op_attention_bwd(mvd_ctx* ctx, const float* q, const float* k, const float* v, const float* d_out, int B, int T, int heads,
                          int d, float* dq, float* dk, float* dv, void* stream);
 int mvd_op_group_norm_bwd(mvd_ctx* ctx, const float* x, const float* dy, int B, int rows, int C, int groups, const float* gamma,
diff --git a/morphablediffusion_amd/csrc/c_api.hip b/morphablediffusion_amd/csrc/c_api.hip
--- a/morphablediffusion_amd/csrc/c_api.hip
+++ b/morphablediffusion_amd/csrc/c_api.hip
@@ -1075,12 +1075,13 @@
   return 0;
 }
 
-int mvd_op_conv3d(mvd_ctx* c, const float* x, int B, int Cin, int D, int H, int W, const float* w, const float* bias,
-                  int Cout, int stride, int transposed, const float* resid, float* out, void* stream) {
+static int op_conv3d(mvd_ctx* c, const float* x, int B, int Cin, int D, int H, int W, const float* w, const float* bias, int Cout,
+                     int stride, int transposed, const float* resid, int out_half, int poison, float* out, void* stream) {
   if (c && hipSetDevice(c->device) != hipSuccess) return mvd_fail("hipSetDevice failed");
   hipStream_t s = S(stream);
   WsScope ws_scope(c);
   if (Cin % 8) return mvd_fail("op_conv3d: Cin must be a multiple of 8");
+  if (out_half && Cout % 4) return mvd_fail("op_conv3d: the fp16-output form needs Cout % 4 == 0");
   const int Do = transposed ? 2 * D : (D - 1) / stride + 1, Ho = transposed ? 2 * H : (H - 1) / stride + 1,
             Wo = transposed ? 2 * W : (W - 1) / stride + 1;
   float* xn = ws_alloc<float>(c, (size_t)B * D * H * W * Cin);
@@ -1095,17 +1096,45 @@
   GemmArgs g;
   g.a = xn; g.a_f32 = 1; g.lda = Cin; g.w = &cw; g.out = on; g.ldc = Cout; g.use_bias = bias != nullptr;
   if (resid) { g.resid = on; g.ldr = Cout; }
+  half_t* oh = nullptr;
+  if (out_half) {
+    oh = ws_alloc<half_t>(c, (size_t)B * Do * Ho * Wo * Cout);
+    WS_CHECK(oh);
+    g.out = oh;
+    g.out_f32 = 0;
+  }
   if (Cin % 64 == 0) {
     half_t* xh = ws_alloc<half_t>(c, (size_t)B * D * H * W * Cin);
     WS_CHECK(xh);
     RET_IF(launch_f32_to_f16(xn, xh, (size_t)B * D * H * W * Cin, s));
     g.a = xh;
     g.a_f32 = 0;
+    if (!mvd_env().no_conv3d_tile && (transposed || stride == 1) && conv3d_tile_shape(Cout, Cin, transposed)) {
+      cw.wt3 = ws_alloc<half_t>(c, conv3d_tile_stream_halfs(Cout, Cin));
+      WS_CHECK(cw.wt3);
+      RET_IF(conv3d_tile_pack(wp, Cout, Cin, transposed, cw.wt3, s));
+      cw.wt3_tr = transposed ? 1 : 0;
+    }
+  }
+  if (poison) {
+    const size_t o = (c->ws.off + 255) & ~(size_t)255;
+    if (o < c->ws.size) HIP_CHECK_RET(hipMemsetAsync(c->ws.base + o, 0xFF, c->ws.size - o, s));
   }
   if (transposed) RET_IF(run_convT3d(c, g, B, D, H, W, s));
   else RET_IF(run_conv3d(c, g, B, D, H, W, stride, s));
+  if (oh) RET_IF(launch_f16_to_f32(oh, on, (size_t)B * Do * Ho * Wo * Cout, s));
   RET_IF(launch_nhwc_to_nchw(on, Cout, B, Cout, Do * Ho * Wo, out, s));
   return 0;
+}
+
+int mvd_op_conv3d(mvd_ctx* c, const float* x, int B, int Cin, int D, int H, int W, const float* w, const float* bias,
+                  int Cout, int stride, int transposed, const float* resid, float* out, void* stream) {
+  return op_conv3d(c, x, B, Cin, D, H, W, w, bias, Cout, stride, transposed, resid, 0, 0, out, stream);
+}
+
+int mvd_op_conv3d_form(mvd_ctx* c, const float* x, int B, int Cin, int D, int H, int W, const float* w, const float* bias,
+                       int Cout, int stride, int transposed, const float* resid, int out_half, int poison, float* out, void* stream) {
+  return op_conv3d(c, x, B, Cin, D, H, W, w, bias, Cout, stride, transposed, resid, out_half, poison, out, stream);
 }
 
 int mvd_op_linear(mvd_ctx* c, const float* a, int M, int K, const float* w, const float* bias, int N, int geglu,
diff --git a/morphablediffusion_amd/csrc/common.h b/morphablediffusion_amd/csrc/common.h
--- a/morphablediffusion_amd/csrc/common.h
+++ b/morphablediffusion_amd/csrc/common.h
@@ -121,6 +121,11 @@
 size_t conv3x_stream_halfs(int N, int Cin, int bn);
 int conv3x_pack(const half_t* w, int N, int Cin, int bn, half_t* stream, hipStream_t s);
 int launch_conv3x(const IGemm& g, const half_t* stream, int bn, hipStream_t s);
+bool conv3d_tile_shape(int N, int Cin, int transposed);
+bool conv3d_tile_eligible(const IGemm& g, int transposed);
+size_t conv3d_tile_stream_halfs(int N, int Cin);
+int conv3d_tile_pack(const half_t* w, int N, int Cin, int transposed, half_t* stream, hipStream_t s);
+int launch_conv3d_tile(const IGemm& g, const half_t* stream, int transposed, hipStream_t s);
 bool gemm_dma_eligible(const IGemm& g);
 bool gemm_dma_is_plain(const IGemm& g);
 void gemm_dma_plan(int M, int N, int ksteps, int bn, int geglu, int* nch_out, int* splitk_out);
@@ -170,6 +175,7 @@
 int launch_rows_f32_to_f16_split(const float* in, int lda, long rows, int C, half_t* out, hipStream_t s);
 int launch_permute_geglu_bias(const float* src, int N, float* dst, hipStream_t s);
 int launch_f32_to_f16(const float* in, half_t* out, size_t n, hipStream_t s);
+int launch_f16_to_f32(const half_t* in, float* out, size_t n, hipStream_t s);
 int launch_rows_f32_to_f16(const float* in, int lda, long rows, int C, half_t* out, hipStream_t s);
 int launch_pack_upconv_weight(const float* src, int N, int Cin, half_t* dst, hipStream_t s);
 int launch_fill_rows_f16(half_t* out, int ld, int rows, const half_t* vec, int n, hipStream_t s);
diff --git a/morphablediffusion_amd/csrc/engine.h b/morphablediffusion_amd/csrc/engine.h
--- a/morphablediffusion_amd/csrc/engine.h
+++ b/morphablediffusion_amd/csrc/engine.h
@@ -20,6 +20,8 @@
   half_t* w = nullptr;
   half_t* wx = nullptr;
   int wx_bn = 0;
+  half_t* wt3 = nullptr;
+  int wt3_tr = 0;
   half_t* w_up = nullptr;
   int res_out = 0;
   float* w32 = nullptr;
diff --git a/morphablediffusion_amd/csrc/engine_unet.hip b/morphablediffusion_amd/csrc/engine_unet.hip
--- a/morphablediffusion_amd/csrc/engine_unet.hip
+++ b/morphablediffusion_amd/csrc/engine_unet.hip
@@ -202,6 +202,17 @@
   return sk;
 }
 
+bool tile3d_takes(mvd_ctx* c, const IGemm& g, const GemmArgs& ga, int transposed) {
+  return !mvd_env().no_conv3d_tile && !c->train_mode && ga.force_splitk <= 1 && conv3d_tile_eligible(g, transposed);
+}
+int go_conv3d_tile(mvd_ctx* c, IGemm& g, const half_t* stream, int transposed, hipStream_t s) {
+  const double vin = (double)g.B * g.PZ * g.PY * g.PX, vout = vin * (transposed ? 8 : 1);
+  const double flops = 2.0 * vin * g.N * g.Cin * 27.0;
+  const double bytes = vin * g.Cin * 2 + 27.0 * g.N * g.Cin * 2 + vout * g.N * (g.out_f32 ? 4 : 2) + (g.resid ? vout * g.N * 4 : 0.0);
+  ProbeScope ps(c, s, transposed ? "convT3d_tile_kernel" : "conv3d_tile_kernel", flops, bytes);
+  return launch_conv3d_tile(g, stream, transposed, s);
+}
+
 enum IGemmKernel { K_GATHER = 0, K_HALO = 1, K_DENSE = 2 };
 
 int launch_planned(mvd_ctx* c, IGemm& g, int M, int sk, IGemmKernel kernel, hipStream_t s, const GemmArgs* defer) {
@@ -386,6 +397,7 @@
   } else {
     return mvd_fail("run_conv3d: kernel must be 1 or 27 taps");
   }
+  if (stride == 1 && g.ntaps == 27 && ga.w->wt3 && !ga.w->wt3_tr && tile3d_takes(c, g, ga, 0)) return go_conv3d_tile(c, g, ga.w->wt3, 0, s);
   return igemm_go(c, g, ga.force_splitk, s);
 }
 
@@ -403,6 +415,7 @@
   gb.OY = 2 * H;
   gb.OX = 2 * W;
   gb.ozm = gb.oym = gb.oxm = 2;
+  if (ga.w->wt3 && ga.w->wt3_tr && tile3d_takes(c, gb, ga, 1)) return go_conv3d_tile(c, gb, ga.w->wt3, 1, s);
   const bool batched = mvd_env().parity_batch && !ga.a_f32 && ga.force_splitk <= 1 && B * D * H * W >= 512 && gemm_dma_eligible(gb);
   for (int par = 0; par < 8; ++par) {
     const int pz = par >> 2, py = (par >> 1) & 1, px = par & 1;
diff --git a/morphablediffusion_amd/csrc/engine_weights.hip b/morphablediffusion_amd/csrc/engine_weights.hip
--- a/morphablediffusion_amd/csrc/engine_weights.hip
+++ b/morphablediffusion_amd/csrc/engine_weights.hip
@@ -550,6 +550,20 @@
     RET_IF(dmalloc(c, (void**)&w->wx, conv3x_stream_halfs(w->N, w->Cin, bn) * sizeof(half_t)));
     RET_IF(conv3x_pack(w->w, w->N, w->Cin, bn, w->wx, c->bs));
     w->wx_bn = bn;
+  }
+  return engine_build_join(c);
+}
+
+int build_conv3d_tile_streams(mvd_ctx* c) {
+  if (mvd_env().no_conv3d_tile || !c->has_cond || c->train_mode) return 0;
+  struct { ConvW* w; int tr; } cs[2] = {{&c->fr_conv0, 0}, {&c->fr_up[2].conv, 1}};
+  for (auto& e : cs) {
+    ConvW* w = e.w;
+    if (w->taps != 27 || w->xp || !conv3d_tile_shape(w->N, w->Cin, e.tr)) continue;
+    engine_build_rotate(c);
+    RET_IF(dmalloc(c, (void**)&w->wt3, conv3d_tile_stream_halfs(w->N, w->Cin) * sizeof(half_t)));
+    RET_IF(conv3d_tile_pack(w->w, w->N, w->Cin, e.tr, w->wt3, c->bs));
+    w->wt3_tr = e.tr;
   }
   return engine_build_join(c);
 }
@@ -942,6 +956,7 @@
   if (c->has_cond) {
     RET_IF(build_condnet_section(c));
     RET_IF(engine_build_join(c));
+    RET_IF(build_conv3d_tile_streams(c));
     if (c->train_mode) RET_IF(engine_build_dgrad_cond(c));
   }
   return 0;
diff --git a/morphablediffusion_amd/csrc/env.h b/morphablediffusion_amd/csrc/env.h
--- a/morphablediffusion_amd/csrc/env.h
+++ b/morphablediffusion_amd/csrc/env.h
@@ -17,6 +17,7 @@
   PROCESS(num, dense_bm, "MVD_DENSE_BM", 0, "sweep: 128 = four-wave row tiles with MVD_DENSE_BN, else 256") \
   PROCESS(num, halo_bn, "MVD_HALO_BN", 0, "sweep (tools/conv_bench3.py): column width of the LDS-halo kernel, 0 = planner's") \
   PROCESS(num, halo_sk, "MVD_HALO_SK", 0, "sweep: split over 64-channel chunks of the LDS-halo kernel, 0 = planner's") \
+  PROCESS(on, no_conv3d_tile, "MVD_NO_CONV3D_TILE", false, "the frustum network's level-0 27-tap convs on the implicit GEMMs, not the 3-D halo-tile kernels") \
   PROCESS(off, parity_batch, "MVD_NO_PARITY_BATCH", true, "one launch per output-parity class of the transposed / upsample convs, not one for all") \
   PROCESS(num, par_walk_min, "MVD_PAR_WALK_MIN", 0, "tiles from which a workgroup walks the parity classes, 0 = never (profiles/r06_y_ab_pwalk.txt: nothing)") \
   PROCESS(off, xcd_cols, "MVD_NO_XCD_COLS", true, "row-tile-major XCD walk always, never the column-major one (common.h: xcd_prefers_cols)") \
diff --git a/morphablediffusion_amd/csrc/k_conv3d_tile.hip b/morphablediffusion_amd/csrc/k_conv3d_tile.hip
--- /dev/null
+++ b/morphablediffusion_amd/csrc/k_conv3d_tile.hip
@@ -0,0 +1,281 @@
+#include "common.h"
+#include "igemm_epilogue.h"
+
+namespace {
+
+constexpr int C3_RING = 4;
+constexpr int C3_STAGE_BYTES = 8 * 1024;
+
+__device__ __forceinline__ int c3_class_taps(int tr, int cls) { return tr ? (1 + (cls >> 2)) * (1 + ((cls >> 1) & 1)) * (1 + (cls & 1)) : 27; }
+__device__ __forceinline__ void c3_tap(int tr, int cls, int ti, int& a, int& b, int& e, int& slab) {
+  if (!tr) {
+    a = ti / 9;
+    b = (ti / 3) % 3;
+    e = ti % 3;
+    slab = ti;
+    return;
+  }
+  const int pz = cls >> 2, py = (cls >> 1) & 1, px = cls & 1;
+  const int ia = ti >> (py + px), ib = (ti >> px) & py, ie = ti & px;
+  a = pz ? 1 - ia : 0;
+  b = py ? 1 - ib : 0;
+  e = px ? 1 - ie : 0;
+  slab = ((pz ? 2 * ia : 1) * 3 + (py ? 2 * ib : 1)) * 3 + (px ? 2 * ie : 1);
+}
+__device__ inline void c3_stage(int tr, int kc, int j, int& cls, int& ti, int& cc) {
+  cls = 0;
+  while (j >= c3_class_taps(tr, cls) * kc) j -= c3_class_taps(tr, cls++) * kc;
+  ti = j / kc;
+  cc = j - ti * kc;
+}
+
+template <bool TR, int KC>
+struct C3Geo {
+  static constexpr int O = TR ? 0 : 1;
+  static constexpr int HD = 4 + 1 + O, HH = 8 + 1 + O, HW = 8 + 1 + O;
+  static constexpr int ROWS = HD * HH * HW;
+  static constexpr int RB = 128 * KC;
+  static constexpr int RPP = 8 / KC;
+  static constexpr int PIECES = (ROWS + RPP - 1) / RPP;
+  static constexpr int HALO_BYTES = PIECES * 1024;
+  static constexpr int LDS = HALO_BYTES + C3_RING * C3_STAGE_BYTES + 4 * EPI_WAVE_BYTES;
+};
+
+template <int KC>
+__device__ __forceinline__ int c3_key(int hy, int hx) {
+  if constexpr (KC == 1) return ((hx >> 1) + 4 * (hy & 1)) & 7;
+  else return ((hx & 7) + 8 * (hy & 1)) & 15;
+}
+
+template <bool TR, int KC>
+__global__ __launch_bounds__(256) void conv3d_tile_kernel(const IGemm g, const half_t* __restrict__ wstream) {
+#if defined(__HIP_DEVICE_COMPILE__)
+  using Geo = C3Geo<TR, KC>;
+  constexpr int O = Geo::O, HH = Geo::HH, HW = Geo::HW;
+  extern __shared__ __attribute__((aligned(16))) char smem[];
+  char* sHalo = smem;
+  char* sRing = smem + Geo::HALO_BYTES;
+  char* sEpi = sRing + C3_RING * C3_STAGE_BYTES;
+  typedef __attribute__((address_space(3))) void* lds_ptr;
+
+  const int tid = threadIdx.x, lane = tid & 63, h = lane >> 5, pl = lane & 31;
+  const int wave = __builtin_amdgcn_readfirstlane(tid >> 6);
+  const int D = g.PZ, H = g.PY, W = g.PX, N = g.N;
+  const int td = (D + 3) >> 2, th = (H + 7) >> 3, tw = (W + 7) >> 3;
+  const int tiles_n = N >> 6;
+  const int tm = blockIdx.x / tiles_n, tn = blockIdx.x - tm * tiles_n;
+  const int bs = tm / (td * th * tw);
+  int r0 = tm - bs * (td * th * tw);
+  const int d0 = (r0 / (th * tw)) * 4;
+  r0 -= (r0 / (th * tw)) * (th * tw);
+  const int y0 = (r0 / tw) * 8, x0 = (r0 - (r0 / tw) * tw) * 8;
+  const int n0 = tn * 64;
+  const int nst = 27 * KC;
+
+  const auto rsrcA = __builtin_amdgcn_make_buffer_rsrc(const_cast<void*>(g.a), (short)0, 0xFFFFFFFEu, 0x00020000);
+  const auto rsrcW = __builtin_amdgcn_make_buffer_rsrc(const_cast<half_t*>(wstream), (short)0, 0xFFFFFFFEu, 0x00020000);
+
+#pragma unroll 1
+  for (int i = wave; i < Geo::PIECES; i += 4) {
+    const int hr = i * Geo::RPP + lane / (8 * KC), cphys = lane & (8 * KC - 1);
+    const int hd = hr / (HH * HW), rem = hr - hd * (HH * HW);
+    const int hy = rem / HW, hx = rem - hy * HW;
+    const int d = d0 + hd - O, y = y0 + hy - O, x = x0 + hx - O;
+    const bool ok = hr < Geo::ROWS && d >= 0 && d < D && y >= 0 && y < H && x >= 0 && x < W;
+    const unsigned vox = (unsigned)(((bs * D + d) * H + y) * W + x);
+    const unsigned off = ok ? (vox * (unsigned)g.lda + (unsigned)((cphys ^ c3_key<KC>(hy, hx)) * 8)) * 2 : 0xFFFFFFFFu;
+    __builtin_amdgcn_raw_ptr_buffer_load_lds(rsrcA, (lds_ptr)(sHalo + i * 1024), 16, off, 0, 0, 0);
+  }
+  const unsigned wvoff = (unsigned)(lane * 16);
+  auto dma_stage = [&](int j) {
+    const int jc = j < nst ? j : nst - 1;
+#pragma unroll
+    for (int i = 0; i < 2; ++i) {
+      const int fr = wave + 4 * i;
+      __builtin_amdgcn_raw_ptr_buffer_load_lds(rsrcW, (lds_ptr)(sRing + (((j & (C3_RING - 1)) * 8 + fr) << 10)), 16, wvoff + (fr << 10),
+                                               (tn * nst + jc) * C3_STAGE_BYTES, 0, 0);
+    }
+  };
+#pragma unroll
+  for (int j = 0; j < C3_RING - 1; ++j) dma_stage(j);
+  asm volatile("s_waitcnt vmcnt(0)" ::: "memory");
+  __builtin_amdgcn_s_barrier();
+
+  const int vy = pl >> 3, vx = pl & 7;
+  int centre[2];
+#pragma unroll
+  for (int p = 0; p < 2; ++p) centre[p] = (wave * HH + 4 * p + vy) * HW + vx;
+
+  float* sc = (float*)(sEpi + wave * EPI_WAVE_BYTES);
+  const int cq = (lane & 7) * 4;
+  const int ed = d0 + wave, ex = x0 + (lane >> 3);
+  const bool has_res = g.resid != nullptr;
+  float4 bias4[2];
+#pragma unroll
+  for (int f = 0; f < 2; ++f) bias4[f] = g.bias ? *(const float4*)(g.bias + n0 + 32 * f + cq) : make_float4(0.f, 0.f, 0.f, 0.f);
+
+  f32x16 acc[2][2];
+#pragma unroll
+  for (int p = 0; p < 2; ++p)
+#pragma unroll
+    for (int f = 0; f < 2; ++f)
+#pragma unroll
+      for (int r = 0; r < 16; ++r) acc[p][f][r] = 0.f;
+
+  int cls = 0, ti = 0, cc = 0;
+#pragma unroll 1
+  for (int j = 0; j < nst; ++j) {
+    int ta, tb, te, slab_unused;
+    c3_tap(TR, cls, ti, ta, tb, te, slab_unused);
+    h8 xa[2][4];
+    {
+      const int shift = (ta * HH + tb) * HW + te;
+      const int key = c3_key<KC>(vy + tb, vx + te);
+#pragma unroll
+      for (int p = 0; p < 2; ++p)
+#pragma unroll
+        for (int kk = 0; kk < 4; ++kk)
+          xa[p][kk] = *(const h8*)(sHalo + (centre[p] + shift) * Geo::RB + (((cc * 8 + 2 * kk + h) ^ key) << 4));
+    }
+    asm volatile("s_waitcnt vmcnt(4)" ::: "memory");
+    __builtin_amdgcn_s_barrier();
+    dma_stage(j + C3_RING - 1);
+    const char* rs = sRing + (j & (C3_RING - 1)) * C3_STAGE_BYTES + lane * 16;
+#pragma unroll
+    for (int kk = 0; kk < 4; ++kk) {
+      const h8 w0 = *(const h8*)(rs + ((2 * kk) << 10)), w1 = *(const h8*)(rs + ((2 * kk + 1) << 10));
+#pragma unroll
+      for (int p = 0; p < 2; ++p) {
+        acc[p][0] = MVD_MFMA_32x32x16(w0, xa[p][kk], acc[p][0], 0, 0, 0);
+        acc[p][1] = MVD_MFMA_32x32x16(w1, xa[p][kk], acc[p][1], 0, 0, 0);
+      }
+    }
+    const int ecls = cls;
+    bool class_done = false;
+    if (++cc == KC) {
+      cc = 0;
+      if (++ti == c3_class_taps(TR, cls)) {
+        ti = 0;
+        ++cls;
+        class_done = true;
+      }
+    }
+    if (!class_done) continue;
+
+    const int pz = ecls >> 2, py = (ecls >> 1) & 1, px = ecls & 1;
+    long row[2][4];
+    bool live[2][4];
+#pragma unroll
+    for (int p = 0; p < 2; ++p)
+#pragma unroll
+      for (int i = 0; i < 4; ++i) {
+        const int ey = y0 + 4 * p + i;
+        live[p][i] = ed < D && ey < H && ex < W;
+        if constexpr (TR) row[p][i] = ((long)((bs * 2 * D + 2 * ed + pz) * 2 * H + 2 * ey + py)) * (2 * W) + 2 * ex + px;
+        else row[p][i] = ((long)((bs * D + ed) * H + ey)) * W + ex;
+      }
+    float4 rpre[2][2][4];
+    if (has_res) {
+#pragma unroll
+      for (int p = 0; p < 2; ++p)
+#pragma unroll
+        for (int f = 0; f < 2; ++f)
+#pragma unroll
+          for (int i = 0; i < 4; ++i)
+            rpre[p][f][i] = live[p][i] ? *(const float4*)((const float*)g.resid + row[p][i] * g.ldr + n0 + 32 * f + cq) : make_float4(0.f, 0.f, 0.f, 0.f);
+    }
+#pragma unroll
+    for (int p = 0; p < 2; ++p) {
+#pragma unroll
+      for (int f = 0; f < 2; ++f) {
+#pragma unroll
+        for (int q = 0; q < 4; ++q)
+          *(float4*)(sc + pl * EPI_LD + 8 * q + 4 * h) =
+              make_float4(acc[p][f][4 * q], acc[p][f][4 * q + 1], acc[p][f][4 * q + 2], acc[p][f][4 * q + 3]);
+        asm volatile("s_waitcnt lgkmcnt(0)" ::: "memory");
+        const int n = n0 + 32 * f + cq;
+        const float4 bsum = bias4[f];
+#pragma unroll
+        for (int i = 0; i < 4; ++i) {
+          const int fr = (lane >> 3) + 8 * i;
+          float4 v = *(const float4*)(sc + fr * EPI_LD + cq);
+          if (!live[p][i]) continue;
+          v.x += bsum.x; v.y += bsum.y; v.z += bsum.z; v.w += bsum.w;
+          if (has_res) {
+            const float4 r = rpre[p][f][i];
+            v.x += r.x; v.y += r.y; v.z += r.z; v.w += r.w;
+          }
+          if (g.out_f32) {
+            *(float4*)((float*)g.out + row[p][i] * g.ldc + n) = v;
+          } else {
+            h4 hv;
+            hv[0] = (half_t)v.x; hv[1] = (half_t)v.y; hv[2] = (half_t)v.z; hv[3] = (half_t)v.w;
+            *(h4*)((half_t*)g.out + row[p][i] * g.ldc + n) = hv;
+          }
+        }
+        asm volatile("s_waitcnt lgkmcnt(0)" ::: "memory");
+#pragma unroll
+        for (int r = 0; r < 16; ++r) acc[p][f][r] = 0.f;
+      }
+    }
+  }
+  asm volatile("s_waitcnt vmcnt(0)" ::: "memory");
+#endif
+}
+
+__global__ void conv3d_tile_pack_kernel(const half_t* __restrict__ w, int N, int Cin, int tr, half_t* __restrict__ out, long nfrag) {
+  const long gid = (long)blockIdx.x * blockDim.x + threadIdx.x;
+  const int kc = Cin / 64, nst = 27 * kc;
+  if (gid >= nfrag * 64) return;
+  const long q = gid >> 6;
+  const int l = (int)(gid & 63);
+  const int tn = (int)(q / (nst * 8));
+  const int r = (int)(q - (long)tn * nst * 8);
+  const int j = r >> 3, kk = (r >> 1) & 3, f = r & 1;
+  int cls, ti, cc, a, b, e, slab;
+  c3_stage(tr, kc, j, cls, ti, cc);
+  c3_tap(tr, cls, ti, a, b, e, slab);
+  const int n = tn * 64 + 32 * f + (l & 31);
+  *(h8*)(out + gid * 8) = *(const h8*)(w + ((long)slab * N + n) * Cin + 64 * cc + 16 * kk + 8 * (l >> 5));
+}
+
+template <bool TR, int KC>
+int launch_c3(const IGemm& g, const half_t* stream, hipStream_t s) {
+  constexpr int LDS = C3Geo<TR, KC>::LDS;
+  static_assert(LDS <= 160 * 1024, "LDS budget");
+  static bool attr_done[MVD_MAX_DEVICES] = {false};
+  bool& attr_set = attr_done[mvd_current_device()];
+  if (!attr_set) {
+    HIP_CHECK_RET(hipFuncSetAttribute((const void*)conv3d_tile_kernel<TR, KC>, hipFuncAttributeMaxDynamicSharedMemorySize, LDS));
+    attr_set = true;
+  }
+  const long tiles = (long)g.B * cdiv(g.PZ, 4) * cdiv(g.PY, 8) * cdiv(g.PX, 8) * (g.N / 64);
+  hipLaunchKernelGGL((conv3d_tile_kernel<TR, KC>), dim3((unsigned)tiles), dim3(256), LDS, s, g, stream);
+  HIP_CHECK_RET(hipGetLastError());
+  return 0;
+}
+
+}
+
+bool conv3d_tile_shape(int N, int Cin, int transposed) { return N > 0 && N % 64 == 0 && Cin == (transposed ? 128 : 64); }
+bool conv3d_tile_eligible(const IGemm& g, int transposed) {
+  if (g.a_f32 || g.ups || g.geglu || g.act != ACT_NONE || g.alpha != 1.0f || g.out_split || g.rowscale || g.gn_partial || g.rowbias) return false;
+  if (!conv3d_tile_shape(g.N, g.Cin, transposed)) return false;
+  if ((g.lda & 7) || g.lda < g.Cin || (g.ldc & 3) || (g.resid && (!g.resid_f32 || (g.ldr & 3)))) return false;
+  const long vox = (long)g.B * g.PZ * g.PY * g.PX;
+  if (vox * g.lda * 2 >= 0xFFFFFF00L || vox * (transposed ? 8 : 1) >= 0x7FFFFFFFL) return false;
+  if ((long)(g.N / 64) * 27 * (g.Cin / 64) * C3_STAGE_BYTES >= 0xFFFFFF00L) return false;
+  return true;
+}
+size_t conv3d_tile_stream_halfs(int N, int Cin) { return (size_t)(N / 64) * 27 * (Cin / 64) * (C3_STAGE_BYTES / 2); }
+int conv3d_tile_pack(const half_t* w, int N, int Cin, int transposed, half_t* stream, hipStream_t s) {
+  if (!conv3d_tile_shape(N, Cin, transposed)) return mvd_fail("conv3d_tile_pack: unsupported shape");
+  const long nfrag = (long)(N / 64) * 27 * (Cin / 64) * 8;
+  hipLaunchKernelGGL(conv3d_tile_pack_kernel, dim3((unsigned)((nfrag * 64 + 255) / 256)), dim3(256), 0, s, w, N, Cin, transposed ? 1 : 0, stream, nfrag);
+  HIP_CHECK_RET(hipGetLastError());
+  return 0;
+}
+int launch_conv3d_tile(const IGemm& g, const half_t* stream, int transposed, hipStream_t s) {
+  if (!conv3d_tile_eligible(g, transposed)) return mvd_fail("conv3d_tile: shape not supported");
+  return transposed ? launch_c3<true, 2>(g, stream, s) : launch_c3<false, 1>(g, stream, s);
+}
diff --git a/morphablediffusion_amd/csrc/k_misc.hip b/morphablediffusion_amd/csrc/k_misc.hip
--- a/morphablediffusion_amd/csrc/k_misc.hip
+++ b/morphablediffusion_amd/csrc/k_misc.hip
@@ -245,6 +245,11 @@
 __global__ void f32_to_f16_kernel(const float* __restrict__ in, half_t* __restrict__ out, size_t n) {
   for (size_t i = (size_t)blockIdx.x * blockDim.x + threadIdx.x; i < n; i += (size_t)gridDim.x * blockDim.x)
     out[i] = (half_t)in[i];
+}
+
+__global__ void f16_to_f32_kernel(const half_t* __restrict__ in, float* __restrict__ out, size_t n) {
+  for (size_t i = (size_t)blockIdx.x * blockDim.x + threadIdx.x; i < n; i += (size_t)gridDim.x * blockDim.x)
+    out[i] = (float)in[i];
 }
 
 __global__ void rows_f32_to_f16_split_kernel(const float* __restrict__ in, int lda, long rows, int C, half_t* __restrict__ out) {
@@ -504,6 +509,12 @@
   return 0;
 }
 
+int launch_f16_to_f32(const half_t* in, float* out, size_t n, hipStream_t s) {
+  hipLaunchKernelGGL(f16_to_f32_kernel, dim3(grid_for(n)), dim3(256), 0, s, in, out, n);
+  HIP_CHECK_RET(hipGetLastError());
+  return 0;
+}
+
 int launch_rows_f32_to_f16(const float* in, int lda, long rows, int C, half_t* out, hipStream_t s) {
   if ((C & 3) || (lda & 3)) return mvd_fail("rows_f32_to_f16: C and lda must be multiples of 4");
   hipLaunchKernelGGL(rows_f32_to_f16_kernel, dim3(grid_for((size_t)rows * C / 4)), dim3(256), 0, s, in, lda, rows, C, out);
diff --git a/morphablediffusion_amd/engine.py b/morphablediffusion_amd/engine.py
--- a/morphablediffusion_amd/engine.py
+++ b/morphablediffusion_amd/engine.py
@@ -609,6 +609,20 @@
                                        1 if transposed else 0, L.ptr(r), L.ptr(out), _stream()))
         return out
 
+    def op_conv3d_form(self, x, w, bias=None, stride=1, transposed=False, resid=None, out_half=False, poison=False):
+        dev = self.device
+        x, w = _f32(x, dev), _f32(w, dev)
+        B, Cin, D, H, W = x.shape
+        Cout = w.shape[1] if transposed else w.shape[0]
+        od = (2 * D, 2 * H, 2 * W) if transposed else ((D - 1) // stride + 1, (H - 1) // stride + 1, (W - 1) // stride + 1)
+        out = torch.empty(B, Cout, *od, device=dev)
+        b = None if bias is None else _f32(bias, dev)
+        r = None if resid is None else _f32(resid, dev)
+        L.check(self.lib.mvd_op_conv3d_form(self._ctx, L.ptr(x), B, Cin, D, H, W, L.ptr(w), L.ptr(b), Cout, stride,
+                                            1 if transposed else 0, L.ptr(r), 1 if out_half else 0, 1 if poison else 0,
+                                            L.ptr(out), _stream()))
+        return out
+
     def op_linear(self, a, w, bias=None, geglu=False, resid=None, a_half=False, force_splitk=0):
         dev = self.device
         a, w = _f32(a, dev), _f32(w, dev)
diff --git a/morphablediffusion_amd/lib.py b/morphablediffusion_amd/lib.py
--- a/morphablediffusion_amd/lib.py
+++ b/morphablediffusion_amd/lib.py
@@ -13,7 +13,7 @@
     "mvd_comm_unique_id", "mvd_comm_init", "mvd_comm_destroy", "mvd_exchange_view_features", "mvd_comm_all_reduce", "mvd_train_sync_gradients",
     "mvd_stage_target_encoder", "mvd_stage_sparse_dense", "mvd_set_volume_ready_event", "mvd_volume_from_fused", "mvd_volume_from_fused_train", "mvd_mse_loss", "mvd_set_volume", "mvd_train_enable", "mvd_train_param_count", "mvd_train_param_info", "mvd_train_arena_size", "mvd_train_adopt_arena", "mvd_train_zero_grad", "mvd_train_unet_step", "mvd_train_get_grad", "mvd_train_get_tensor", "mvd_train_bn_calls", "mvd_train_cond_backward", "mvd_train_conditioner_backward", "mvd_train_conditioner_backward_batch", "mvd_train_adamw_step", "mvd_train_repack", "mvd_train_repack_async", "mvd_train_grad_bucket_count", "mvd_train_grad_bucket", "mvd_train_grad_bucket_wait", "mvd_train_set_bucket_snapshot",
     "mvd_frustum_volumes", "mvd_frustum_volumes_batch", "mvd_denoise_views", "mvd_denoise_views_batch", "mvd_denoise_views_ms", "mvd_op_cfg_ms", "mvd_op_conv", "mvd_op_linear", "mvd_op_group_norm",
-    "mvd_op_layer_norm", "mvd_op_attention", "mvd_op_attention_bwd", "mvd_op_group_norm_bwd", "mvd_op_layer_norm_bwd", "mvd_op_conv3d", "mvd_op_conv_bwd", "mvd_op_linear_bwd", "mvd_op_conv3d_bwd", "mvd_op_tgemm", "mvd_op_st_tail", "mvd_op_st_head", "mvd_bench_conv", "mvd_bench_linear", "mvd_bench_group_norm", "mvd_probe_config", "mvd_probe_report", "mvd_vae_decode", "mvd_vae_encode",
+    "mvd_op_layer_norm", "mvd_op_attention", "mvd_op_attention_bwd", "mvd_op_group_norm_bwd", "mvd_op_layer_norm_bwd", "mvd_op_conv3d", "mvd_op_conv3d_form", "mvd_op_conv_bwd", "mvd_op_linear_bwd", "mvd_op_conv3d_bwd", "mvd_op_tgemm", "mvd_op_st_tail", "mvd_op_st_head", "mvd_bench_conv", "mvd_bench_linear", "mvd_bench_group_norm", "mvd_probe_config", "mvd_probe_report", "mvd_vae_decode", "mvd_vae_encode",
     "mvd_clip_encode", "mvd_clip_embed_dim",
 ]
 
```

New measurement: 80.32 steps/s (median of 6 runs). +1.9%, better.
